# yangzhaojason/DualDiff

Measured on AMD Instinct MI355X. Metric: denoising-steps/sec, 6-view 224×400 fp16, 50-step DDIM @ 1/2/4/8 MI355X, higher is better.
Workload: dtype fp16; 1 GPU; BASELINE configs[1]: 6-view 224x400 (28x50 latents) multiview UNet + 2 ControlNet branches (ORS panorama + ORS-3D, SFA on), CFG 2.0 -> 12 view-instances/scene, DDIM-50 schedule, random-init weights; scenes_per_gpu=1, parallelism=scene-sharded x1 (no data-path collective), hip_graph=True, streams=3, invariant_conditioning=recomputed every step

## Files before the change

dualdiff_amd/_build.py:

```python
import os
import shutil
import subprocess
import sys
from concurrent.futures import ThreadPoolExecutor

HERE = os.path.dirname(os.path.abspath(__file__))
CSRC = os.path.join(HERE, "csrc")
LIBDIR = os.path.join(HERE, "lib")
OBJDIR = os.path.join(HERE, "lib", "obj")
LIBNAME = "libdualdiff_hip.so"
GEMM_SOURCES = ["gemm23.hip", "gemm2_conv.hip", "gemm1.hip", "conv3s.hip", "gemm2_geglu.hip", "gemm4.hip", "gemm.hip"]
SOURCES = ["gemm23.hip", "gemm2_conv.hip", "attention.hip", "gemm1.hip", "conv3s.hip", "gemm2_geglu.hip", "gemm4.hip",
           "norm.hip", "elementwise.hip", "tokens.hip", "xattn.hip", "clip.hip", "gemm8.hip", "vae.hip", "image.hip", "boxes.hip", "gemm.hip"]
EXTRA_FLAGS = {"attention.hip": ["-mllvm", "-amdgpu-mfma-vgpr-form=1", "-fno-honor-nans"],
               **{src: ["-mllvm", "-amdgpu-mfma-vgpr-form=1"] for src in GEMM_SOURCES},
               "clip.hip": ["-mllvm", "-amdgpu-mfma-vgpr-form=1"]}
ARCH = "gfx950"


def _hipcc():
    for cand in (os.environ.get("HIPCC"), "/opt/rocm/bin/hipcc", shutil.which("hipcc")):
        if cand and os.path.exists(cand):
            return cand
    raise RuntimeError("hipcc not found (set HIPCC or install ROCm under /opt/rocm)")


def lib_path():
    return os.environ.get("DD_HIP_LIB") or os.path.join(LIBDIR, LIBNAME)


def _deps():
    deps = [os.path.join(CSRC, f) for f in os.listdir(CSRC)]
    deps.append(os.path.join(HERE, "..", "include", "dualdiff_hip.h"))
    return deps


def needs_build():
    lib = lib_path()
    if not os.path.exists(lib):
        return True
    t = os.path.getmtime(lib)
    return any(os.path.getmtime(d) > t for d in _deps() if os.path.exists(d))


def build_native(force=False, verbose=True):
    if not force and not needs_build():
        return lib_path()
    hipcc = _hipcc()
    os.makedirs(OBJDIR, exist_ok=True)
    flags = ["--offload-arch=" + ARCH, "-O2", "-std=c++17", "-fPIC", "-Wno-unused-value",
             "-DNDEBUG"] + os.environ.get("DD_HIP_DEFINES", "").split()

    def compile_one(src):
        obj = os.path.join(OBJDIR, src.replace(".hip", ".o"))
        cmd = [hipcc] + flags + EXTRA_FLAGS.get(src, []) + ["-c", os.path.join(CSRC, src), "-o", obj]
        r = subprocess.run(cmd, capture_output=True, text=True)
        if r.returncode != 0:
            raise RuntimeError("hipcc failed for %s:\n%s\n%s" % (src, r.stdout, r.stderr))
        return obj

    with ThreadPoolExecutor(max_workers=4) as ex:
        objs = list(ex.map(compile_one, SOURCES))
    tmp = lib_path() + ".tmp"
    cmd = [hipcc, "--offload-arch=" + ARCH, "-shared", "-fPIC", "-o", tmp] + objs
    r = subprocess.run(cmd, capture_output=True, text=True)
    if r.returncode != 0:
        raise RuntimeError("link failed:\n%s\n%s" % (r.stdout, r.stderr))
    os.replace(tmp, lib_path())
    if verbose:
        print("[dualdiff_amd] built %s" % lib_path(), file=sys.stderr)
    return lib_path()


if __name__ == "__main__":
    build_native(force="--force" in sys.argv)
```

dualdiff_amd/_native.py:

```python
import ctypes
import os

import torch
from ctypes import (POINTER, Structure, c_char_p, c_float, c_int32, c_int64, c_uint32, c_void_p)

from . import _build

DD_F16, DD_BF16, DD_F32 = 0, 1, 2
DD_EPI_NONE, DD_EPI_GEGLU, DD_EPI_SILU = 0, 1, 2


class GemmDesc(Structure):
    _fields_ = [
        ("a", c_void_p), ("a2", c_void_p), ("lda", c_int64), ("lda2", c_int64), ("k1", c_int32),
        ("rows", c_int32), ("n", c_int32), ("k", c_int32),
        ("w", c_void_p), ("bias", c_void_p), ("rowvec", c_void_p),
        ("rows_per_inst", c_int32), ("ld_rowvec", c_int32),
        ("res", c_void_p), ("ldres", c_int64),
        ("out", c_void_p), ("ldc", c_int64),
        ("alpha", c_float), ("accumulate", c_int32), ("epilogue", c_int32),
        ("conv", c_int32), ("hin", c_int32), ("win", c_int32), ("cin", c_int32),
        ("hv", c_int32), ("wv", c_int32), ("hout", c_int32), ("wout", c_int32), ("stride", c_int32),
        ("dtype", c_int32), ("tile", c_int32), ("split_k", c_int32),
        ("ws", c_void_p), ("ws_bytes", c_int64),
        ("ln_colsum", c_void_p), ("ln_bias", c_void_p), ("ln_eps", c_float), ("out_f32", c_int32), ("ln_stats_out", c_void_p), ("ln_stats_in", c_void_p),
        ("out_headmajor_d", c_int32), ("hm_scaled_planes", c_int32), ("hm_scale", c_float),
        ("phase", c_int32),
        ("ln_out", c_void_p), ("ld_ln_out", c_int64), ("lno_gamma", c_void_p), ("lno_beta", c_void_p),
    ]


class AttnDesc(Structure):
    _fields_ = [
        ("q", c_void_p), ("k", c_void_p), ("v", c_void_p), ("o", c_void_p),
        ("ldq", c_int64), ("ldk", c_int64), ("ldv", c_int64), ("ldo", c_int64),
        ("q_batch_stride", c_int64), ("k_batch_stride", c_int64),
        ("v_batch_stride", c_int64), ("o_batch_stride", c_int64),
        ("batch", c_int32), ("heads", c_int32), ("head_dim", c_int32), ("lq", c_int32), ("lk", c_int32),
        ("scale", c_float),
        ("kv_batch_map", c_void_p),
        ("accumulate", c_int32), ("dtype", c_int32), ("variant", c_int32),
        ("q_head_stride", c_int64), ("k_head_stride", c_int64), ("v_head_stride", c_int64),
        ("q_prescaled", c_int32),
        ("kv_batch_map2", c_void_p),
        ("lk_dev", c_void_p),
    ]


class BoxTokensDesc(Structure):
    _fields_ = [
        ("points", c_void_p), ("classes", c_void_p), ("masks", c_void_p),
        ("class_tokens", c_void_p), ("null_pos", c_void_p), ("null_class", c_void_p),
        ("pos", c_void_p), ("cat", c_void_p), ("cls_out", c_void_p),
        ("rows", c_int32), ("points_per_box", c_int32), ("num_freqs", c_int32), ("include_input", c_int32),
        ("class_token_dim", c_int32), ("cls_offset", c_int32),
        ("ld_cat", c_int64),
        ("normalize", c_int32), ("points_dtype", c_int32), ("dtype", c_int32), ("n_classes", c_int32),
        ("freqs", c_float * 16), ("xyz_min", c_float * 3), ("xyz_range", c_float * 3),
    ]


class XAttnDesc(Structure):
    _fields_ = [
        ("x", c_void_p), ("ldx", c_int64), ("res", c_void_p), ("ldres", c_int64),
        ("wq", c_void_p), ("wo", c_void_p), ("bo", c_void_p),
        ("k", c_void_p), ("v", c_void_p), ("ldk", c_int64), ("ldv", c_int64),
        ("k_inst_stride", c_int64), ("k_head_stride", c_int64), ("v_inst_stride", c_int64), ("v_head_stride", c_int64),
        ("out", c_void_p), ("ldo", c_int64),
        ("instances", c_int32), ("rows_per_inst", c_int32), ("lk", c_int32),
        ("channels", c_int32), ("heads", c_int32), ("scale", c_float), ("dtype", c_int32),
        ("ln_out", c_void_p), ("ld_ln_out", c_int64), ("ln_gamma", c_void_p), ("ln_beta", c_void_p), ("ln_eps", c_float),
        ("lk_dev", c_void_p),
    ]


class Gemm8Desc(Structure):
    _fields_ = [
        ("a", c_void_p), ("a_scale", c_void_p), ("lda", c_int64),
        ("w", c_void_p), ("w_scale", c_void_p), ("ldw", c_int64),
        ("bias", c_void_p), ("res", c_void_p), ("ldres", c_int64),
        ("out", c_void_p), ("ldc", c_int64),
        ("rows", c_int32), ("n", c_int32), ("k_padded", c_int32), ("dtype", c_int32),
        ("out_headmajor_d", c_int32), ("hm_scaled_planes", c_int32), ("hm_scale", c_float), ("geglu", c_int32),
    ]


SIGNATURES = {
    "dd_abi_version": (c_int32, []),
    "dd_desc_size": (c_int64, [c_int32]),
    "dd_error_string": (c_char_p, [c_int32]),
    "dd_target_arch": (c_char_p, []),
    "dd_gemm": (c_int32, [POINTER(GemmDesc), c_void_p]),
    "dd_gemm_workspace_bytes": (c_int64, [POINTER(GemmDesc)]),
    "dd_gemm_num_tiles": (c_int32, []),
    "dd_gemm_tile_id": (c_int32, [c_int32]),
    "dd_gemm_kernel_name": (c_char_p, [POINTER(GemmDesc)]),
    "dd_gemm_conv_pad": (c_int32, [POINTER(GemmDesc), c_int32, c_void_p]),
    "dd_gemm_conv_pad_workspace_bytes": (c_int64, [POINTER(GemmDesc), c_int32]),
    "dd_gemm_conv_pad_kernel_name": (c_char_p, [POINTER(GemmDesc), c_int32]),
    "dd_groupnorm_nhwc": (c_int32, [c_void_p, c_int32, c_void_p, c_int32, c_void_p, c_void_p, c_void_p,
                                    c_int32, c_int32, c_int32, c_float, c_int32, c_int32,
                                    c_void_p, c_int64, c_void_p]),
    "dd_groupnorm_workspace_bytes": (c_int64, [c_int32, c_int32]),
    "dd_groupnorm_is_fused": (c_int32, [c_int32, c_int32, c_int32]),
    "dd_layernorm": (c_int32, [c_void_p, c_void_p, c_void_p, c_void_p, c_int64, c_int32, c_float,
                               c_int32, c_void_p]),
    "dd_attention": (c_int32, [POINTER(AttnDesc), c_void_p]),
    "dd_attention_kernel_name": (c_char_p, [POINTER(AttnDesc)]),
    "dd_add": (c_int32, [c_void_p, c_void_p, c_void_p, c_void_p, c_int64, c_int32, c_void_p]),
    "dd_scale": (c_int32, [c_void_p, c_void_p, c_float, c_int64, c_int32, c_void_p]),
    "dd_probe_spin": (c_int32, [c_void_p, c_uint32, c_void_p]),
    "dd_groupnorm_splitk": (c_int32, [c_void_p, c_int32, c_void_p, c_void_p, c_int32, c_void_p, c_int64, c_void_p,
                                      c_void_p, c_void_p, c_void_p, c_int32, c_int32, c_int32, c_int32, c_float, c_int32,
                                      c_int32, c_void_p]),
    "dd_xattn320": (c_int32, [POINTER(XAttnDesc), c_void_p]),
    "dd_nchw_to_nhwc_views": (c_int32, [c_void_p, c_void_p, c_int32, c_int32, c_int32, c_int32, c_int32, c_int32, c_int32,
                                        c_void_p]),
    "dd_fourier_embed_strided": (c_int32, [c_void_p, c_void_p, c_int64, c_int32, POINTER(c_float), c_int32, c_int32,
                                           c_int32, c_int32, c_int32, c_int64, c_int64, c_int64, c_int64, c_void_p]),
    "dd_box_tokens": (c_int32, [POINTER(BoxTokensDesc), c_void_p]),
    "dd_ctx_assemble": (c_int32, [c_void_p, c_void_p, c_void_p, c_void_p, c_void_p, c_int32, c_int32, c_int32, c_int32,
                                  c_int32, c_int32, c_int32, c_int32, c_void_p]),
    "dd_gemm8": (c_int32, [POINTER(Gemm8Desc), c_void_p]),
    "dd_rowquant_fp8": (c_int32, [c_void_p, c_void_p, c_void_p, c_void_p, c_void_p, c_int64, c_int32, c_int64, c_float,
                                  c_int32, c_void_p]),
    "dd_xattn_pack_weight": (c_int32, [c_void_p, c_void_p, c_int32, c_void_p]),
    "dd_silu": (c_int32, [c_void_p, c_void_p, c_int64, c_int32, c_void_p]),
    "dd_nchw_to_nhwc": (c_int32, [c_void_p, c_void_p, c_int32, c_int32, c_int32, c_int32, c_int32, c_void_p]),
    "dd_nhwc_to_nchw": (c_int32, [c_void_p, c_void_p, c_int32, c_int32, c_int32, c_int32, c_int32, c_void_p]),
    "dd_timestep_embedding": (c_int32, [c_void_p, c_void_p, c_int32, c_int32, c_int32, c_float,
                                        c_int32, c_void_p]),
    "dd_cfg_unipc_step": (c_int32, [c_void_p, c_void_p, c_void_p, c_void_p, c_void_p, c_void_p, c_void_p, c_void_p,
                                    c_float, c_int64, c_int32, c_void_p]),
    "dd_softmax_rows": (c_int32, [c_void_p, c_void_p, c_int64, c_int32, c_int64, c_int64, c_int32, c_void_p]),
    "dd_ors_project": (c_int32, [c_void_p, c_void_p, c_void_p, c_void_p, c_void_p, c_int32, c_int32, c_int32,
                                 c_float, c_int32, c_int32, c_int32, c_void_p]),
    "dd_fourier_embed": (c_int32, [c_void_p, c_void_p, c_int64, c_int32, POINTER(c_float), c_int32, c_int32,
                                   c_int32, c_int32, c_void_p]),
    "dd_conv3x3_small_cout": (c_int32, [c_void_p, c_void_p, c_void_p, c_void_p, c_int32, c_int32,
                                        c_int32, c_int32, c_int32, c_int32, c_void_p]),
    "dd_vae_posterior": (c_int32, [c_void_p, c_void_p, c_void_p, c_void_p, c_void_p, c_int32, c_int32, c_int32, c_float,
                                   c_int32, c_int32, c_void_p]),
    "dd_image_quantize_u8": (c_int32, [c_void_p, c_void_p, c_int32, c_int32, c_int32, c_int32, c_int32, c_void_p]),
    "dd_image_resample_u8": (c_int32, [c_void_p, c_void_p, c_int32, c_int32, c_int32, c_int32, c_int32, c_void_p, c_void_p,
                                       c_int32, c_void_p, c_void_p, c_int32, c_int32, c_int32, c_int32, c_int32, c_int32,
                                       c_int32, c_int32, c_void_p]),
    "dd_image_load_u8": (c_int32, [c_void_p, c_void_p, c_int32, c_int32, c_int32, c_int32, c_int32, c_void_p, c_void_p,
                                   c_int32, c_void_p, c_void_p, c_int32, c_void_p, c_int32, c_int32, c_void_p]),
    "dd_box_views": (c_int32, [c_void_p, c_void_p, c_void_p, c_void_p, c_void_p, c_int32, c_int32, c_int32, c_int32,
                               c_int32, c_int32, c_int32, c_int32, c_void_p, c_void_p, c_void_p, c_void_p, c_void_p,
                               c_void_p]),
    "dd_clip_embed": (c_int32, [c_void_p, c_void_p, c_void_p, c_void_p, c_void_p, c_int32, c_int32, c_int32, c_int32,
                                c_int32, c_int32, c_void_p]),
    "dd_causal_attention": (c_int32, [c_void_p, c_void_p, c_void_p, c_void_p, c_int64, c_int64, c_int64, c_int64,
                                      c_int64, c_int64, c_int64, c_int64, c_int32, c_int32, c_int32, c_int32, c_float,
                                      c_int32, c_void_p]),
    "dd_conv3x3_thin": (c_int32, [c_void_p, c_void_p, c_void_p, c_void_p, c_int32, c_int32, c_int32, c_int32, c_int32,
                                  c_int32, c_int32, c_int32, c_void_p]),
    "dd_cfg_ddim_step": (c_int32, [c_void_p, c_void_p, c_void_p, c_void_p, c_void_p, c_float,
                                   c_int64, c_int32, c_void_p]),
    "dd_cfg_ddim_step_given": (c_int32, [c_void_p, c_void_p, c_void_p, c_void_p, c_void_p, c_float, c_void_p, c_void_p,
                                         c_void_p, c_void_p, c_int32, c_int64, c_int64, c_int32, c_void_p]),
    "dd_cfg_unipc_step_given": (c_int32, [c_void_p, c_void_p, c_void_p, c_void_p, c_void_p, c_void_p, c_void_p,
                                          c_void_p, c_float, c_void_p, c_void_p, c_void_p, c_void_p, c_int32, c_int64,
                                          c_int64, c_int32, c_void_p]),
    "dd_given_views_noise": (c_int32, [c_void_p, c_void_p, c_void_p, c_void_p, c_void_p, c_float, c_float, c_int64,
                                       c_int64, c_int32, c_void_p]),
}

ABI_VERSION = 4
_LIB = None


def lib_path():
    return _build.lib_path()


def load(build_if_missing=True):
    global _LIB
    if _LIB is not None:
        return _LIB
    path = lib_path()
    if not os.path.exists(path):
        if not build_if_missing:
            raise RuntimeError("dualdiff_amd: %s is missing (run __graft_entry__.build())" % path)
        _build.build_native()
    try:
        lib = ctypes.CDLL(path)
    except OSError as e:
        raise RuntimeError("dualdiff_amd: cannot load HIP library %s: %s" % (path, e))
    for name, (res, args) in SIGNATURES.items():
        try:
            fn = getattr(lib, name)
        except AttributeError:
            raise RuntimeError("dualdiff_amd: %s does not export %s" % (path, name))
        fn.restype = res
        fn.argtypes = args
    if lib.dd_abi_version() != ABI_VERSION:
        raise RuntimeError("dualdiff_amd: %s has ABI version %d, this binding needs %d (rebuild: __graft_entry__.build())"
                           % (path, lib.dd_abi_version(), ABI_VERSION))
    for which, st in enumerate((GemmDesc, AttnDesc, XAttnDesc, Gemm8Desc, BoxTokensDesc)):
        if lib.dd_desc_size(which) != ctypes.sizeof(st):
            raise RuntimeError("dualdiff_amd: %s was built with a different %s (%d bytes, binding has %d)"
                               % (path, st.__name__, lib.dd_desc_size(which), ctypes.sizeof(st)))
    _LIB = lib
    return lib


class Unsupported(RuntimeError):
    """DD_ERR_UNSUPPORTED (-2): the library validated the call and launched NOTHING — the caller may take another form."""


def check(rc, what):
    if rc != 0:
        msg = load().dd_error_string(rc).decode()
        raise (Unsupported if rc == -2 else RuntimeError)("dualdiff_amd.%s failed: %s (%d)" % (what, msg, rc))
```

dualdiff_amd/csrc/gemm.hip:

```cpp
#include "gemm_device.h"
#include <algorithm>

namespace {

template <typename T>
__global__ __launch_bounds__(256)
void dd_splitk_reduce_kernel(const GemmParams p, int nsplit) {
  const int64_t groups_per_row = p.n / 8;
  const int64_t total = (int64_t)p.rows * groups_per_row;
  for (int64_t g = (int64_t)blockIdx.x * blockDim.x + threadIdx.x; g < total;
       g += (int64_t)gridDim.x * blockDim.x) {
    const int row = (int)(g / groups_per_row);
    const int col = (int)(g - (int64_t)row * groups_per_row) * 8;
    float v[8] = {0, 0, 0, 0, 0, 0, 0, 0};
    for (int z = 0; z < nsplit; ++z) {
      const float* src = p.partial + ((int64_t)z * p.rows + row) * p.n + col;
      const f32x4 a = *reinterpret_cast<const f32x4*>(src);
      const f32x4 b = *reinterpret_cast<const f32x4*>(src + 4);
      v[0] += a[0]; v[1] += a[1]; v[2] += a[2]; v[3] += a[3];
      v[4] += b[0]; v[5] += b[1]; v[6] += b[2]; v[7] += b[3];
    }
    epilogue_store8<T>(p, row, col, v);
  }
}

int ceil_div(int a, int b) { return (a + b - 1) / b; }

bool dma_ok(const dd_gemm_desc* d) {
  const int64_t lim = (int64_t)1 << 30;
  const int64_t nw = (d->epilogue == DD_EPI_GEGLU ? 2 : 1) * (int64_t)d->n;
  bool ok = (d->k % BK) == 0 && nw * d->k < lim;
  if (d->conv) {
    ok = ok && (d->cin % BK) == 0 && (int64_t)d->rows / (d->hout * d->wout) * d->hin * d->win * d->cin < lim;
  } else {
    ok = ok && (int64_t)d->rows * d->lda < lim;
    if (d->a2) ok = ok && (d->k1 % BK) == 0 && (int64_t)d->rows * d->lda2 < lim;
  }
  return ok;
}

bool env_is_zero(const char* name) { const char* v = getenv(name); return v && atoi(v) == 0; }
bool persist_off() { static const bool off = env_is_zero("DD_PERSIST"); return off; }
bool persist3_off() { static const bool off = env_is_zero("DD_PERSIST3"); return off; }

int64_t extent_bytes(const dd_gemm_desc* d, int64_t ld) { return (((int64_t)d->rows - 1) * ld + d->n) * 2; }
constexpr int64_t kExtentLimit = (int64_t)1 << 31;

int twin(const TileCfg& like, Family family) {
  for (int i = 0; i < kNumTiles; ++i)
    if (kTiles[i].family == family && kTiles[i].wm == like.wm && kTiles[i].wn == like.wn && kTiles[i].tm == like.tm &&
        kTiles[i].tn == like.tn) return i;
  return -1;
}

Plan unsupported() { Plan pl{}; pl.unsupported = true; return pl; }

Plan plan_direct(const dd_gemm_desc* d, int ti, unsigned form) {
  const TileCfg& t = kTiles[ti];
  const int hw = d->hout * d->wout, W = d->wout;
  const int arows = tile_bm(t) + 88;
  const int R = W > 0 ? std::min(tile_bm(t), arows - 16 - 2 * (W + 1)) / W : 0;
  const bool ok = form == F_CONV && d->stride == 1 && d->hv == d->hin && d->wv == d->win && d->hout == d->hin &&
                  d->wout == d->win && (d->cin % BK) == 0 && hw > 0 && d->rows % hw == 0 && dma_ok(d) &&
                  (t.band ? hw > tile_bm(t) && R >= 1 : hw <= tile_bm(t) && tile_bm(t) < 65535);
  if (!ok) return unsupported();
  const int m_inst = d->rows / hw;
  Plan pl{};
  pl.tile_idx = ti;
  if (t.band) {
    pl.band_rows = R * W;
    pl.bands = ceil_div(d->hout, R);
    pl.g_per_tile = 1;
    pl.tiles_m = m_inst * pl.bands;
  } else {
    pl.g_per_tile = std::min(tile_bm(t) / hw, m_inst);
    pl.tiles_m = ceil_div(m_inst, pl.g_per_tile);
  }
  const int nchunks = d->cin / BK;
  const int split = std::min(d->split_k > 0 ? d->split_k : 1, nchunks);
  pl.chunks_per_split = ceil_div(nchunks, split);
  pl.tiles_n = ceil_div(d->n, tile_bn(t));
  pl.split = ceil_div(nchunks, pl.chunks_per_split);
  pl.k_per_split = pl.chunks_per_split * BK;
  return pl;
}

unsigned form_of(const dd_gemm_desc* d, int pad_lo) {
  return pad_lo == 0 ? F_PAD0 : d->conv ? F_CONV : d->epilogue == DD_EPI_GEGLU ? F_GEGLU : F_DENSE;
}

Plan make_plan(const dd_gemm_desc* d, int pad_lo) {
  const bool geglu = d->epilogue == DD_EPI_GEGLU;
  const unsigned form = form_of(d, pad_lo);
  int ti = d->tile > 0 ? tile_index(d->tile) : -1;
  if (ti < 0) {
    for (int id : kAutoTiles) {
      const TileCfg& t = kTiles[tile_index(id)];
      if (!(t.forms & form)) continue;
      ti = tile_index(id);
      const int bn_out = geglu ? tile_bn(t) / 2 : tile_bn(t);
      if ((long)ceil_div(d->rows, tile_bm(t)) * ceil_div(d->n, bn_out) >= (long)kNumCU * 3 / 2) break;
    }
  }
  if (d->ln_colsum) {
    const int ring = twin(kTiles[ti], FAM_RING);
    if (d->tile <= 0 && ring >= 0) ti = ring;
    if (kTiles[ti].family != FAM_RING || !dma_ok(d)) return unsupported();
  }
  if (kTiles[ti].family == FAM_PIPE && d->conv) return unsupported();
  if (d->ln_out) {
    if (d->tile > 0 && !(kTiles[ti].forms & F_LN_OUT)) return unsupported();
    if (d->tile <= 0) {
      const int pipe = tile_index(kTileLnPipe);
      ti = (!persist3_off() || ceil_div(d->rows, tile_bm(kTiles[pipe])) <= kNumCU) ? pipe : tile_index(kTileLnRing);
    }
    if (d->n != 320 || !dma_ok(d)) return unsupported();
  }
  if (kTiles[ti].family == FAM_DIRECT) return plan_direct(d, ti, form);
  if (kTiles[ti].family != FAM_REG && !dma_ok(d)) {
    const int reg = twin(kTiles[ti], FAM_REG);
    ti = reg >= 0 ? reg : tile_index(geglu ? kTile128x128 : kTile64x64);
  }
  const TileCfg& t = kTiles[ti];
  if (!(t.forms & form)) return unsupported();
  Plan pl{};
  const int bn_out = geglu ? tile_bn(t) / 2 : tile_bn(t);
  pl.tile_idx = ti;
  pl.tiles_m = ceil_div(d->rows, tile_bm(t));
  pl.tiles_n = ceil_div(d->n, bn_out);
  int split = d->split_k;
  const int nkt = ceil_div(d->k, BK);
  if (split <= 0) {
    const long blocks = (long)pl.tiles_m * pl.tiles_n;
    const bool deep = !geglu && blocks < kNumCU && nkt >= 16;
    split = deep ? (int)std::max(1L, std::min({(2L * kNumCU + blocks - 1) / blocks, (long)nkt / 4, 32L})) : 1;
  }
  if (geglu || d->ln_colsum || d->ln_stats_out || d->out_headmajor_d || d->ln_out) split = 1;
  if (split > nkt) split = nkt;
  int kts = ceil_div(nkt, split);
  split = ceil_div(nkt, kts);
  pl.split = split;
  pl.k_per_split = kts * BK;
  const bool walk = (t.forms & F_PERSIST) && !d->conv && split == 1 && !d->ln_colsum && nkt >= t.depth;
  pl.persist_ok = walk && t.family == FAM_RING && !persist_off() && !d->ln_out;
  const bool ln_tile = (t.forms & F_LN_OUT) != 0;
  const bool pre_acc = !geglu && !ln_tile && t.tm * (t.tn / 2) <= 4;
  pl.persist3_ok = walk && t.family == FAM_PIPE && !persist3_off() && (d->k % BK) == 0 && !d->out_f32 && !d->ln_stats_out &&
                   !d->rowvec && (!d->accumulate || pre_acc) && ln_tile == (d->ln_out != nullptr) &&
                   extent_bytes(d, d->ldc) < kExtentLimit && (!d->res || extent_bytes(d, d->ldres) < kExtentLimit) &&
                   (!d->ln_out || extent_bytes(d, d->ld_ln_out) < kExtentLimit);
  return pl;
}

inline bool gemm4_takes(const Plan& pl) {
  return pl.persist3_ok && pl.tiles_m * pl.tiles_n > kNumCU * gemm4_resident(kTiles[pl.tile_idx]);
}

LaunchFn* launcher(const Plan& pl, unsigned form) {
  switch (kTiles[pl.tile_idx].family) {
    case FAM_REG: return launch_gemm1;
    case FAM_RING: return form == F_CONV ? launch_gemm2_conv : form == F_GEGLU ? launch_gemm2_geglu : launch_gemm2_dense;
    case FAM_PIPE: return gemm4_takes(pl) ? launch_gemm4 : launch_gemm3;
    default: return launch_conv3s;
  }
}

int validate(const dd_gemm_desc* d, int pad_lo = 1) {
  if (!d || !d->a || !d->w || !d->out) return DD_ERR_BAD_ARG;
  if (d->ln_colsum) {
    if (!d->ln_bias || d->conv || d->a2 || d->bias) return DD_ERR_BAD_ARG;
    if (d->k != 320 && d->k != 640 && d->k != 1280) return DD_ERR_UNSUPPORTED;
    if (!dd_aligned16(d->ln_colsum) || !dd_aligned16(d->ln_bias) || (d->lda & 7)) return DD_ERR_BAD_ARG;
  }
  if (d->ln_out) {
    if (!d->lno_gamma || !d->lno_beta || d->conv || d->epilogue != DD_EPI_NONE || d->rowvec || d->accumulate ||
        d->out_f32 || d->out_headmajor_d || d->ln_stats_out || d->ln_colsum)
      return DD_ERR_UNSUPPORTED;
    if (d->n != 320) return DD_ERR_UNSUPPORTED;
    if (!dd_aligned16(d->ln_out) || !dd_aligned16(d->lno_gamma) || !dd_aligned16(d->lno_beta) || (d->ld_ln_out & 7))
      return DD_ERR_BAD_ARG;
  }
  if (d->rows <= 0 || d->n <= 0 || d->k <= 0) return DD_ERR_BAD_ARG;
  if (d->rows >= (1 << 22)) return DD_ERR_UNSUPPORTED;
  if ((d->k & 7) || (d->n & 7) || (d->ldc & 7)) return DD_ERR_BAD_ARG;
  if (d->dtype != DD_F16 && d->dtype != DD_BF16) return DD_ERR_BAD_ARG;
  if (!dd_aligned16(d->a) || !dd_aligned16(d->w) || !dd_aligned16(d->out)) return DD_ERR_BAD_ARG;
  if (d->bias && !dd_aligned16(d->bias)) return DD_ERR_BAD_ARG;
  if (d->res && (!dd_aligned16(d->res) || (d->ldres & 7))) return DD_ERR_BAD_ARG;
  if (d->rowvec && (!dd_aligned16(d->rowvec) || (d->ld_rowvec & 7) || d->rows_per_inst <= 0)) return DD_ERR_BAD_ARG;
  if (d->conv) {
    if (d->a2) return DD_ERR_UNSUPPORTED;
    if (d->cin <= 0 || (d->cin & 7) || d->k != 9 * d->cin) return DD_ERR_BAD_ARG;
    if (d->hin <= 0 || d->win <= 0 || d->hout <= 0 || d->wout <= 0) return DD_ERR_BAD_ARG;
    if (d->stride != 1 && d->stride != 2) return DD_ERR_UNSUPPORTED;
    if (d->hv <= 0 || d->wv <= 0) return DD_ERR_BAD_ARG;
    if (d->rows % (d->hout * d->wout) != 0) return DD_ERR_BAD_ARG;
    if ((d->hv + pad_lo + 1 - 3) / d->stride + 1 != d->hout || (d->wv + pad_lo + 1 - 3) / d->stride + 1 != d->wout)
      return DD_ERR_BAD_ARG;
  } else {
    if (d->lda & 7) return DD_ERR_BAD_ARG;
    if (d->a2) {
      if (!dd_aligned16(d->a2) || (d->lda2 & 7) || (d->k1 & 7) || d->k1 <= 0 || d->k1 >= d->k) return DD_ERR_BAD_ARG;
    }
  }
  if (d->epilogue != DD_EPI_NONE && d->epilogue != DD_EPI_GEGLU && d->epilogue != DD_EPI_SILU) return DD_ERR_BAD_ARG;
  if (d->out_f32 && (d->epilogue == DD_EPI_GEGLU || d->accumulate)) return DD_ERR_UNSUPPORTED;
  if (d->ln_stats_out && ((d->n & 31) || d->epilogue == DD_EPI_GEGLU || d->out_f32 || !dd_aligned16(d->ln_stats_out)))
    return DD_ERR_UNSUPPORTED;
  if (d->ln_stats_in && (!d->ln_colsum || !dd_aligned16(d->ln_stats_in))) return DD_ERR_BAD_ARG;
  if (d->out_headmajor_d) {
    if (d->out_headmajor_d < 8 || (d->out_headmajor_d & 7) || d->n % d->out_headmajor_d) return DD_ERR_BAD_ARG;
    if (d->conv || d->epilogue == DD_EPI_GEGLU || d->accumulate || d->out_f32 || d->ln_stats_out) return DD_ERR_UNSUPPORTED;
  }
  if (d->epilogue == DD_EPI_GEGLU && (d->res || d->rowvec || d->accumulate || d->alpha != 1.0f)) return DD_ERR_UNSUPPORTED;
  if (d->epilogue == DD_EPI_GEGLU && d->conv) return DD_ERR_UNSUPPORTED;
  return DD_OK;
}

int validate_pad(const dd_gemm_desc* d, int pad_lo) {
  if (pad_lo != 0 && pad_lo != 1) return DD_ERR_BAD_ARG;
  if (pad_lo == 1) return validate(d);
  if (!d || !d->conv) return DD_ERR_BAD_ARG;
  if (d->stride != 2 || d->hv != d->hin || d->wv != d->win || d->epilogue == DD_EPI_GEGLU) return DD_ERR_UNSUPPORTED;
  if (d->hin < 2 || d->win < 2) return DD_ERR_BAD_ARG;
  return validate(d, 0);
}

thread_local char g_kname[160];

}

extern "C" int dd_gemm_num_tiles(void) { return kNumTiles; }
extern "C" int dd_gemm_tile_id(int index) { return (index >= 0 && index < kNumTiles) ? kTiles[index].id : -1; }

constexpr int64_t DD_COUNTER_BYTES = 65536;

namespace {

int64_t workspace_bytes(const dd_gemm_desc* d, int pad_lo) {
  if (validate_pad(d, pad_lo) != DD_OK) return 0;
  const Plan pl = make_plan(d, pad_lo);
  if (pl.unsupported || pl.split <= 1) return 0;
  return DD_COUNTER_BYTES + (int64_t)pl.split * d->rows * d->n * (int64_t)sizeof(float);
}

const char* kernel_name(const dd_gemm_desc* d, int pad_lo) {
  const int vc = validate_pad(d, pad_lo);
  if (vc != DD_OK) return (pad_lo == 0 && vc == DD_ERR_UNSUPPORTED) ? "unsupported" : "invalid";
  const Plan pl = make_plan(d, pad_lo);
  if (pl.unsupported) return "unsupported";
  const TileCfg& t = kTiles[pl.tile_idx];
  const char* conv = d->conv ? "true" : "false";
  const char* geglu = d->epilogue == DD_EPI_GEGLU ? "true" : "false";
  const char* kern = "dd_gemm_pad0_kernel";
  char args[48] = "";
  if (pad_lo == 0) {
  } else if (t.family == FAM_DIRECT) {
    kern = "dd_conv3s_kernel";
    snprintf(args, sizeof(args), ", %d, %d, %s", t.depth, t.grp, t.band ? "true" : "false");
  } else if (t.family == FAM_PIPE) {
    kern = gemm4_takes(pl) ? "dd_gemm4_kernel" : "dd_gemm3_kernel";
    snprintf(args, sizeof(args), ", %d, %s", t.depth, geglu);
  } else if (t.family == FAM_RING) {
    kern = "dd_gemm2_kernel";
    snprintf(args, sizeof(args), ", %d, %s, %s", t.depth, conv, geglu);
  } else {
    kern = "dd_gemm_kernel";
    snprintf(args, sizeof(args), ", %s, %s", conv, geglu);
  }
  snprintf(g_kname, sizeof(g_kname), "%s<%s, %d, %d, %d, %d%s> split=%d grid=%dx%d tile=%s", kern,
           d->dtype == DD_F16 ? "_Float16" : "__bf16", t.wm, t.wn, t.tm, t.tn, args, pl.split, pl.tiles_m, pl.tiles_n, t.name);
  return g_kname;
}

int gemm_run(const dd_gemm_desc* d, int pad_lo, dd_stream_t stream) {
  const int vc = validate_pad(d, pad_lo);
  if (vc != DD_OK) return vc;
  const Plan pl = make_plan(d, pad_lo);
  if (pl.unsupported) return DD_ERR_UNSUPPORTED;
  GemmParams p{};
  p.g_per_tile = pl.g_per_tile; p.chunks_per_split = pl.chunks_per_split;
  p.ln_colsum = reinterpret_cast<const float*>(d->ln_colsum);
  p.ln_bias = reinterpret_cast<const float*>(d->ln_bias);
  p.ln_eps = d->ln_eps;
  p.ln_out = d->ln_out; p.ld_ln_out = d->ld_ln_out; p.lno_gamma = d->lno_gamma; p.lno_beta = d->lno_beta;
  p.a = d->a; p.a2 = d->a2; p.lda = d->lda; p.lda2 = d->lda2;
  p.k1 = d->a2 ? d->k1 : d->k;
  p.rows = d->rows; p.n = d->n; p.k = d->k;
  p.w = d->w; p.bias = d->bias; p.rowvec = d->rowvec;
  p.rows_per_inst = d->rows_per_inst > 0 ? d->rows_per_inst : 1; p.ld_rowvec = d->ld_rowvec;
  p.res = d->res; p.ldres = d->ldres; p.out = d->out; p.ldc = d->ldc;
  p.alpha = d->alpha; p.accumulate = d->accumulate; p.out_f32 = d->out_f32;
  p.stat_out = reinterpret_cast<float*>(d->ln_stats_out);
  p.stat_in = reinterpret_cast<const float*>(d->ln_stats_in);
  p.hm_d = d->out_headmajor_d; p.hm_planes = d->hm_scaled_planes; p.hm_scale = d->hm_scale;
  p.act = d->epilogue == DD_EPI_SILU ? DD_EPI_SILU : DD_EPI_NONE;
  p.hin = d->hin; p.win = d->win; p.cin = d->cin; p.hv = d->hv; p.wv = d->wv;
  p.hout = d->hout; p.wout = d->wout; p.stride = d->stride;
  p.upsample = d->conv && (d->hv != d->hin || d->wv != d->win);
  p.scale_h = d->conv ? (float)d->hin / (float)d->hv : 1.f;
  p.scale_w = d->conv ? (float)d->win / (float)d->wv : 1.f;
  p.k_per_split = pl.k_per_split;
  p.tiles_m = pl.tiles_m; p.tiles_n = pl.tiles_n;
  p.band_rows = pl.band_rows; p.bands = pl.bands; p.inv_bands = pl.bands > 0 ? 1.0f / (float)pl.bands : 1.0f;
  p.inv_hw = d->conv ? 1.0f / (float)(d->hout * d->wout) : 1.0f;
  p.inv_wout = d->conv ? 1.0f / (float)d->wout : 1.0f;
  p.inv_rpi = 1.0f / (float)p.rows_per_inst;
  {
    const int64_t nw = (d->epilogue == DD_EPI_GEGLU ? 2 : 1) * (int64_t)d->n;
    p.w_bytes = (uint32_t)(nw * d->k * 2);
    if (d->conv) {
      p.a_bytes = (uint32_t)((int64_t)d->rows / (d->hout * d->wout) * d->hin * d->win * d->cin * 2);
      p.a2_bytes = 0;
    } else {
      p.a_bytes = (uint32_t)((((int64_t)d->rows - 1) * d->lda + p.k1) * 2);
      p.a2_bytes = d->a2 ? (uint32_t)((((int64_t)d->rows - 1) * d->lda2 + (d->k - d->k1)) * 2) : 0u;
    }
  }
  {
    const int64_t ob = extent_bytes(d, d->ldc), rb = extent_bytes(d, d->ldres);
    const bool fits = ob < kExtentLimit && (!d->res || rb < kExtentLimit);
    p.out_bytes = fits ? (uint32_t)ob : 0u;
    p.res_bytes = fits && d->res ? (uint32_t)rb : 0u;
  }
  p.persist = 0;
  p.inv_tiles_n = 1.0f / (float)(pl.tiles_n > 0 ? pl.tiles_n : 1);
  p.inv_hm_d = d->out_headmajor_d > 0 ? 1.0f / (float)d->out_headmajor_d : 1.0f;
  p.ln_out_bytes = d->ln_out ? (uint32_t)extent_bytes(d, d->ld_ln_out) : 0u;
  p.partial = nullptr;
  p.dbg_stamps = nullptr;
  DD_STAMP_HOST(p, d);
  if (pl.split > 1) {
    const int64_t need = DD_COUNTER_BYTES + (int64_t)pl.split * d->rows * d->n * (int64_t)sizeof(float);
    if (!d->ws || d->ws_bytes < need) return DD_ERR_WORKSPACE;
    p.partial = reinterpret_cast<float*>(reinterpret_cast<char*>(d->ws) + DD_COUNTER_BYTES);
  }
  hipStream_t s = reinterpret_cast<hipStream_t>(stream);
  dd_clear_error();
  if (d->phase != 2) {
    const int rc = launcher(pl, form_of(d, pad_lo))(d->dtype, form_of(d, pad_lo), p, pl, s);
    if (rc != DD_OK) return rc;
  }
  if (pl.split > 1 && d->phase != 1) {
    const int blocks = (int)std::min<int64_t>(((int64_t)p.rows * (p.n / 8) + 255) / 256, 2048);
    if (d->dtype == DD_F16) hipLaunchKernelGGL(dd_splitk_reduce_kernel<_Float16>, dim3(blocks), dim3(256), 0, s, p, pl.split);
    else hipLaunchKernelGGL(dd_splitk_reduce_kernel<__bf16>, dim3(blocks), dim3(256), 0, s, p, pl.split);
    return dd_check_launch();
  }
  return DD_OK;
}

}

extern "C" int64_t dd_gemm_workspace_bytes(const dd_gemm_desc* d) { return workspace_bytes(d, 1); }
extern "C" const char* dd_gemm_kernel_name(const dd_gemm_desc* d) { return kernel_name(d, 1); }
extern "C" int dd_gemm(const dd_gemm_desc* d, dd_stream_t stream) { return gemm_run(d, 1, stream); }

extern "C" int dd_gemm_conv_pad(const dd_gemm_desc* d, int32_t pad_lo, dd_stream_t stream) {
  return gemm_run(d, pad_lo, stream);
}
extern "C" int64_t dd_gemm_conv_pad_workspace_bytes(const dd_gemm_desc* d, int32_t pad_lo) {
  return workspace_bytes(d, pad_lo);
}
extern "C" const char* dd_gemm_conv_pad_kernel_name(const dd_gemm_desc* d, int32_t pad_lo) {
  return kernel_name(d, pad_lo);
}
```

dualdiff_amd/csrc/gemm2_kernel.h:

```cpp
#pragma once
#include "gemm_device.h"

namespace {

template <int NW, int TM, int TN, int NSTAGE, bool CONV>
constexpr int gemm2_min_blocks() {
  return (!CONV && NW == 4 && TM * TN <= 8 && NSTAGE <= 3) ? 2 : 1;
}

template <typename T, int WAVES_M, int WAVES_N, int TM, int TN, int NSTAGE, bool CONV, bool GEGLU>
__global__ __launch_bounds__(64 * WAVES_M * WAVES_N, (gemm2_min_blocks<WAVES_M * WAVES_N, TM, TN, NSTAGE, CONV>()))
void dd_gemm2_kernel(const GemmParams p) {
  using V8 = typename dd_vec<T>::v8;
  constexpr int NW = WAVES_M * WAVES_N;
  constexpr int BM = WAVES_M * TM * 16;
  constexpr int BN = WAVES_N * TN * 16;
  constexpr int BN_OUT = GEGLU ? BN / 2 : BN;
  constexpr int XI = BM / 8 / NW;
  constexpr int WI = BN / 8 / NW;
  constexpr int LPS = XI + WI;
  constexpr int STAGE = (BM + BN) * BK;
  static_assert(BM % (8 * NW) == 0 && BN % (8 * NW) == 0, "tile/waves mismatch");
  static_assert(NW % 2 == 0, "swizzle must not depend on the instruction index");
  static_assert(TN % 2 == 0 && (!GEGLU || TN % 4 == 0), "TN");
  static_assert(NSTAGE >= 2 && NSTAGE <= 8, "NSTAGE");
  static_assert((NSTAGE - 2) * LPS <= 63, "vmcnt is a 6-bit counter");

  DD_STAMP_DECL();
  DD_STAMP(0);
  extern __shared__ __attribute__((aligned(16))) unsigned char smem[];
  T* ring = reinterpret_cast<T*>(smem);

  const int tid = threadIdx.x;
  const int lane = tid & 63;
  const int wave = __builtin_amdgcn_readfirstlane(tid >> 6);
  const int wave_m = wave / WAVES_N;
  const int wave_n = wave % WAVES_N;

  const int ntiles = p.tiles_m * p.tiles_n;
  int lin = blockIdx.x;
  int tile = xcd_remap(lin, ntiles);
  int block_m0 = (tile / p.tiles_n) * BM;
  int block_n0 = (tile % p.tiles_n) * BN_OUT;

  const int kbeg = blockIdx.z * p.k_per_split;
  const int kend = min(p.k, kbeg + p.k_per_split);
  const int nk = (kend - kbeg + BK - 1) / BK;

  const int lrow = lane >> 3;
  const int lc = (lane & 7) ^ ((((wave & 1) << 2) + (lane >> 4)) & 7);
  const uint32_t lcb = (uint32_t)lc * 16u;

  uint32_t wv[WI];
  auto make_wv = [&](const int bn0) __attribute__((always_inline)) {
#pragma unroll
  for (int j = 0; j < WI; ++j) {
    const int R = (j * NW + wave) * 8 + lrow;
    const int wvi = R / (TN * 16);
    const int rho = R % (TN * 16);
    const int tn = rho >> 4, r = rho & 15;
    int n_glob;
    if (GEGLU) {
      constexpr int TH = TN / 2;
      const int t = tn % TH;
      const int loc = wvi * (TH * 16) + (r >> 2) * (4 * TH) + t * 4 + (r & 3);
      const int col = bn0 + loc;
      n_glob = (col < p.n) ? col + (tn >= TH ? p.n : 0) : -1;
    } else {
      const int loc = wvi * (TN * 16) + (r >> 2) * (4 * TN) + tn * 4 + (r & 3);
      const int col = bn0 + loc;
      n_glob = (col < p.n) ? col : -1;
    }
    wv[j] = n_glob >= 0 ? (uint32_t)n_glob * (uint32_t)p.k * 2u + lcb : DD_OOB;
  }
  };
  make_wv(block_n0);

  uint32_t xe[XI];
  uint32_t xe2[CONV ? 1 : XI];
  uint32_t syo[CONV ? XI : 1][3], sxo[CONV ? XI : 1][3], xbits[CONV ? XI : 1];
#pragma unroll
  for (int j = 0; j < XI; ++j) {
    const int r = block_m0 + (j * NW + wave) * 8 + lrow;
    const bool rv = r < p.rows;
    if (CONV) {
      const int hw = p.hout * p.wout;
      const int rr = rv ? r : 0;
      const int inst = dd_fdiv(rr, p.inv_hw);
      const int rem = rr - inst * hw;
      const int oy = dd_fdiv(rem, p.inv_wout);
      const int ox = rem - oy * p.wout;
      const int iy0 = oy * p.stride - 1, ix0 = ox * p.stride - 1;
      uint32_t bits = 0;
#pragma unroll
      for (int t = 0; t < 3; ++t) {
        const int iy = iy0 + t, ix = ix0 + t;
        const bool vy = iy >= 0 && iy < p.hv, vx = ix >= 0 && ix < p.wv;
        int sy = min(max(iy, 0), p.hv - 1), sx = min(max(ix, 0), p.wv - 1);
        if (p.upsample) {
          sy = min((int)floorf(sy * p.scale_h), p.hin - 1);
          sx = min((int)floorf(sx * p.scale_w), p.win - 1);
        }
        syo[j][t] = (uint32_t)((inst * p.hin + sy) * p.win) * (uint32_t)p.cin * 2u + lcb;
        sxo[j][t] = (uint32_t)(sx * p.cin) * 2u;
        if (vy) bits |= 1u << t;
        if (vx) bits |= 8u << t;
      }
      uint32_t m9 = 0;
#pragma unroll
      for (int t = 0; t < 9; ++t)
        if (rv && ((bits >> (t / 3)) & 1u) && ((bits >> (3 + t % 3)) & 1u)) m9 |= 1u << t;
      xbits[j] = m9;
      xe[j] = DD_OOB;
    } else {
      xe[j] = rv ? (uint32_t)r * (uint32_t)p.lda * 2u + lcb : DD_OOB;
      xe2[j] = rv ? (uint32_t)r * (uint32_t)p.lda2 * 2u + lcb : DD_OOB;
    }
  }
  auto make_xe = [&](const int bm0) __attribute__((always_inline)) {
#pragma unroll
    for (int j = 0; j < XI; ++j) {
      const int r = bm0 + (j * NW + wave) * 8 + lrow;
      const bool rv = r < p.rows;
      xe[j] = rv ? (uint32_t)r * (uint32_t)p.lda * 2u + lcb : DD_OOB;
      xe2[j] = rv ? (uint32_t)r * (uint32_t)p.lda2 * 2u + lcb : DD_OOB;
    }
  };
  auto set_tap = [&](int tap) __attribute__((always_inline)) {
    if (CONV) {
      const int ky = (tap * 11) >> 5;
      const int kx = tap - ky * 3;
      const uint32_t y0 = 0u - (uint32_t)(ky == 0), y1 = 0u - (uint32_t)(ky == 1), y2 = 0u - (uint32_t)(ky == 2);
      const uint32_t x0 = 0u - (uint32_t)(kx == 0), x1 = 0u - (uint32_t)(kx == 1), x2 = 0u - (uint32_t)(kx == 2);
#pragma unroll
      for (int j = 0; j < XI; ++j) {
        const uint32_t oy = (syo[j][0] & y0) | (syo[j][1] & y1) | (syo[j][2] & y2);
        const uint32_t ox = (sxo[j][0] & x0) | (sxo[j][1] & x1) | (sxo[j][2] & x2);
        const uint32_t m = 0u - ((xbits[j] >> tap) & 1u);
        xe[j] = ((oy + ox) & m) | (DD_OOB & ~m);
      }
    }
  };
  const __amdgpu_buffer_rsrc_t rs_w = __builtin_amdgcn_make_buffer_rsrc(const_cast<void*>(p.w), 0, p.w_bytes, 0x00020000);
  const __amdgpu_buffer_rsrc_t rs_a = __builtin_amdgcn_make_buffer_rsrc(const_cast<void*>(p.a), 0, p.a_bytes, 0x00020000);
  const __amdgpu_buffer_rsrc_t rs_a2 = __builtin_amdgcn_make_buffer_rsrc(
      const_cast<void*>(p.a2 ? p.a2 : p.a), 0, p.a2 ? p.a2_bytes : p.a_bytes, 0x00020000);

  int ik0 = kbeg;
  int itap = CONV ? kbeg / p.cin : 0;
  int ici0 = CONV ? kbeg - itap * p.cin : 0;
  set_tap(itap);
  auto issue_next = [&](int slot) __attribute__((always_inline)) {
    T* xs = ring + slot * STAGE;
    T* ws = xs + BM * BK;
    const uint32_t ksoff = dd_dbg::SAMEK ? 0u : (uint32_t)ik0 * 2u;
#pragma unroll
    for (int j = 0; j < WI; ++j) bdma16(rs_w, wv[j], ksoff, ws + (j * NW + wave) * 8 * BK);
    if (CONV) {
      const uint32_t csoff = (uint32_t)ici0 * 2u;
#pragma unroll
      for (int j = 0; j < XI; ++j) bdma16(rs_a, xe[j], csoff, xs + (j * NW + wave) * 8 * BK);
      ici0 += BK;
      if (ici0 >= p.cin) {
        ici0 = 0;
        ++itap;
        set_tap(itap);
      }
    } else if (ik0 >= p.k1) {
      const uint32_t k2 = (uint32_t)(ik0 - p.k1) * 2u;
#pragma unroll
      for (int j = 0; j < XI; ++j) bdma16(rs_a2, xe2[j], k2, xs + (j * NW + wave) * 8 * BK);
    } else {
#pragma unroll
      for (int j = 0; j < XI; ++j) bdma16(rs_a, xe[j], ksoff, xs + (j * NW + wave) * 8 * BK);
    }
    ik0 += BK;
  };

  f32x4 acc[TN][TM];
#pragma unroll
  for (int i = 0; i < TN; ++i)
#pragma unroll
    for (int j = 0; j < TM; ++j) acc[i][j] = f32x4{0.f, 0.f, 0.f, 0.f};

  const int frow = lane & 15;
  const int fswz = (lane >> 1) & 7;
  const int fchunk = lane >> 4;

  DD_STAMP(1);
#pragma unroll
  for (int s0 = 0; s0 < NSTAGE - 1; ++s0)
    if (s0 < nk) issue_next(s0);
  DD_STAMP(2);

  __shared__ float s_ln_mean[BM], s_ln_rstd[BM];
  if (!CONV && p.ln_colsum && p.stat_in) {
    const int parts = p.k >> 5;
    const float inv_k = 1.0f / (float)p.k;
    for (int r = tid; r < BM; r += NW * 64) {
      const float* src = p.stat_in + (int64_t)min(block_m0 + r, p.rows - 1) * parts * 2;
      float sum = 0.f, sq = 0.f;
      for (int i = 0; i < parts; i += 2) {
        const f32x4 v = *reinterpret_cast<const f32x4*>(src + i * 2);
        sum += v[0] + v[2];
        sq += v[1] + v[3];
      }
      const float mean = sum * inv_k;
      s_ln_mean[r] = mean;
      s_ln_rstd[r] = rsqrtf(fmaxf(sq * inv_k - mean * mean, 0.f) + p.ln_eps);
    }
    __syncthreads();
  } else if (!CONV && p.ln_colsum) {
    const int lpr = p.k / 40;
    const int rpw = 64 / lpr;
    const int sub = lane & (lpr - 1);
    const float inv_k = 1.0f / (float)p.k;
    for (int r0 = wave * rpw; r0 < BM; r0 += NW * rpw) {
      const int r = r0 + lane / lpr;
      const int64_t grow = min(block_m0 + r, p.rows - 1);
      float sum = 0.f, sq = 0.f;
      u32x4 raw[5];
#pragma unroll
      for (int i = 0; i < 5; ++i)
        raw[i] = dd_ld16(reinterpret_cast<const T*>(p.a) + grow * p.lda + (sub + i * lpr) * 8);
#pragma unroll
      for (int i = 0; i < 5; ++i) {
        float f[8];
        dd_unpack8<T>(raw[i], f);
#pragma unroll
        for (int e = 0; e < 8; ++e) { sum += f[e]; sq += f[e] * f[e]; }
      }
      for (int o = lpr >> 1; o > 0; o >>= 1) { sum += __shfl_xor(sum, o, 64); sq += __shfl_xor(sq, o, 64); }
      if (sub == 0) {
        const float mean = sum * inv_k;
        s_ln_mean[r] = mean;
        s_ln_rstd[r] = rsqrtf(fmaxf(sq * inv_k - mean * mean, 0.f) + p.ln_eps);
      }
    }
    __syncthreads();
  }

  V8 wf[2][TN], xf[2][TM];
  auto mfma_step = [&]() __attribute__((always_inline)) {
    __builtin_amdgcn_s_setprio(1);
#pragma unroll
    for (int ks = 0; ks < 2; ++ks) {
#pragma unroll
      for (int i = 0; i < TN; ++i)
#pragma unroll
        for (int j = 0; j < TM; ++j) acc[i][j] = dd_mfma16(wf[ks][i], xf[ks][j], acc[i][j]);
    }
    __builtin_amdgcn_s_setprio(0);
  };
  int sbase = 0;
  bool have_next = false;
  auto kstep = [&](const int kt) __attribute__((always_inline)) {
    if (NSTAGE == 2) {
      wait_vmcnt<0>();
    } else {
      const int ahead = have_next ? NSTAGE - 2 : min(nk - 1 - kt, NSTAGE - 2);
      if (ahead <= 0) wait_vmcnt<0>();
      else if (ahead == 1 || NSTAGE <= 3) wait_vmcnt<(NSTAGE > 2 ? 1 : 0) * LPS>();
      else if (ahead == 2 || NSTAGE <= 4) wait_vmcnt<(NSTAGE > 3 ? 2 : 0) * LPS>();
      else if (ahead == 3 || NSTAGE <= 5) wait_vmcnt<(NSTAGE > 4 ? 3 : 0) * LPS>();
      else if (ahead == 4 || NSTAGE <= 6) wait_vmcnt<(NSTAGE > 5 ? 4 : 0) * LPS>();
      else if (ahead == 5 || NSTAGE <= 7) wait_vmcnt<(NSTAGE > 6 ? 5 : 0) * LPS>();
      else wait_vmcnt<(NSTAGE > 7 ? 6 : 0) * LPS>();
    }
    __builtin_amdgcn_s_barrier();
    {
      const int a = kt + NSTAGE - 1;
      const int islot = (sbase + a) % NSTAGE;
      if (a < nk) {
        issue_next(islot);
      } else if (have_next) {
        if constexpr (!CONV) {
          if (a == nk) {
            const int nt = xcd_remap(lin + (int)gridDim.x, ntiles);
            make_wv((nt % p.tiles_n) * BN_OUT);
            make_xe((nt / p.tiles_n) * BM);
            ik0 = kbeg;
          }
          issue_next(islot);
        }
      }
    }
    const int slot = (sbase + kt) % NSTAGE;
    const T* xs = ring + slot * STAGE + (wave_m * TM * 16 + frow) * BK;
    const T* ws = ring + slot * STAGE + BM * BK + (wave_n * TN * 16 + frow) * BK;
#pragma unroll
    for (int ks = 0; ks < 2; ++ks) {
      const int cofs = ((fchunk + 4 * ks) ^ fswz) << 3;
#pragma unroll
      for (int i = 0; i < TN; ++i) wf[ks][i] = dd_as_v8<T>(dd_ld16(ws + i * 16 * BK + cofs));
#pragma unroll
      for (int j = 0; j < TM; ++j) xf[ks][j] = dd_as_v8<T>(dd_ld16(xs + j * 16 * BK + cofs));
    }
    __builtin_amdgcn_sched_barrier(0);
    mfma_step();
  };
  const bool persist = !CONV && p.persist != 0;
  for (;;) {
  have_next = persist && lin + (int)gridDim.x < ntiles;
  for (int kt = 0; kt < nk; kt += 2) {
    kstep(kt);
    DD_STAMP_IF(kt == 0, 3);
    if (kt + 1 < nk) kstep(kt + 1);
  }
  DD_STAMP(4);
  if constexpr (!CONV && !GEGLU && WAVES_M == 1 && WAVES_N == 10 && TM == 5 && TN == 2) {
    if (p.ln_out) {
      store_tile_ln<T>(p, acc, block_m0, wave_n, lane, reinterpret_cast<float*>(smem));
      return;
    }
  }
  const bool ln = !CONV && p.ln_colsum;
  store_tile<T, TM, TN, GEGLU>(p, acc, block_m0, block_n0, wave_m, wave_n, lane, p.rows,
                               ln ? s_ln_mean : nullptr, ln ? s_ln_rstd : nullptr);
  if (!have_next) break;
  lin += (int)gridDim.x;
  tile = xcd_remap(lin, ntiles);
  block_m0 = (tile / p.tiles_n) * BM;
  block_n0 = (tile % p.tiles_n) * BN_OUT;
  sbase = (sbase + nk) % NSTAGE;
#pragma unroll
  for (int i = 0; i < TN; ++i)
#pragma unroll
    for (int j = 0; j < TM; ++j) acc[i][j] = f32x4{0.f, 0.f, 0.f, 0.f};
  }
  DD_STAMP_FLUSH(p);
}

struct Gemm2 {
  static constexpr Family family = FAM_RING;
  static constexpr unsigned needs = 0;
  template <typename T, size_t I, unsigned FORM>
  static int run(const GemmParams& p, const Plan& pl, hipStream_t s) {
    constexpr const TileCfg& t = kTiles[I];
    constexpr size_t smem = (size_t)t.depth * (tile_bm(t) + tile_bn(t)) * BK * sizeof(T);
    static_assert(smem <= 160 * 1024, "LDS");
    constexpr auto kern = dd_gemm2_kernel<T, t.wm, t.wn, t.tm, t.tn, t.depth, FORM == F_CONV, FORM == F_GEGLU>;
    dim3 grid(pl.tiles_m * pl.tiles_n, 1, pl.split);
    GemmParams q = p;
    if (pl.persist_ok) {
      static std::atomic<int> resident{0};
      int per_cu = resident.load(std::memory_order_relaxed);
      if (per_cu == 0) {
        raise_lds_limit<kern>(smem);
        if (hipOccupancyMaxActiveBlocksPerMultiprocessor(&per_cu, kern, 64 * t.wm * t.wn, smem) != hipSuccess || per_cu < 1)
          per_cu = 1;
        resident.store(per_cu, std::memory_order_relaxed);
      }
      if ((int)grid.x > kNumCU * per_cu) {
        q.persist = 1;
        grid.x = kNumCU * per_cu;
      }
    }
    return launch_kernel<kern>(grid, 64 * t.wm * t.wn, smem, s, q);
  }
};

}
```

dualdiff_amd/csrc/gemm_device.h:

```cpp
#pragma once
#include "dd_common.h"
#include "dd_debug.h"
#include "gemm_tiles.h"
#include <type_traits>

using namespace ddg;

namespace {

__device__ __forceinline__ int dd_fdiv(int n, float inv) { return (int)(((float)n + 0.5f) * inv); }


template <typename T>
__device__ __forceinline__ void store8(const GemmParams& p, int64_t row, int col, float (&v)[8]) {
  if (p.hm_d) {
    const int plane = col / p.hm_d;
    if (plane < p.hm_planes) {
#pragma unroll
      for (int e = 0; e < 8; ++e) v[e] *= p.hm_scale;
    }
    dd_st16(reinterpret_cast<T*>(p.out) + ((int64_t)plane * p.rows + row) * p.hm_d + (col - plane * p.hm_d),
            dd_pack8<T>(v));
    return;
  }
  if (p.out_f32) {
    float* o = reinterpret_cast<float*>(p.out) + row * p.ldc + col;
    *reinterpret_cast<f32x4*>(o) = f32x4{v[0], v[1], v[2], v[3]};
    *reinterpret_cast<f32x4*>(o + 4) = f32x4{v[4], v[5], v[6], v[7]};
  } else {
    dd_st16(reinterpret_cast<T*>(p.out) + row * p.ldc + col, dd_pack8<T>(v));
  }
}

template <typename T>
__device__ __forceinline__ void epilogue_store8(const GemmParams& p, int row, int col, float (&v)[8]) {
  if (p.bias) {
    float b[8];
    dd_unpack8<T>(dd_ld16(reinterpret_cast<const T*>(p.bias) + col), b);
#pragma unroll
    for (int i = 0; i < 8; ++i) v[i] += b[i];
  }
  if (p.rowvec) {
    const int inst = dd_fdiv(row, p.inv_rpi);
    float b[8];
    dd_unpack8<T>(dd_ld16(reinterpret_cast<const T*>(p.rowvec) + (int64_t)inst * p.ld_rowvec + col), b);
#pragma unroll
    for (int i = 0; i < 8; ++i) v[i] += b[i];
  }
#pragma unroll
  for (int i = 0; i < 8; ++i) v[i] *= p.alpha;
  if (p.res) {
    float b[8];
    dd_unpack8<T>(dd_ld16(reinterpret_cast<const T*>(p.res) + (int64_t)row * p.ldres + col), b);
#pragma unroll
    for (int i = 0; i < 8; ++i) v[i] += b[i];
  }
  if (p.act == DD_EPI_SILU) {
#pragma unroll
    for (int i = 0; i < 8; ++i) v[i] = dd_silu_f(v[i]);
  }
  if (p.accumulate) {
    float b[8];
    dd_unpack8<T>(dd_ld16(reinterpret_cast<T*>(p.out) + (int64_t)row * p.ldc + col), b);
#pragma unroll
    for (int i = 0; i < 8; ++i) v[i] += b[i];
  }
  store8<T>(p, row, col, v);
}

__device__ __forceinline__ int xcd_remap(int bid, int nwg) {
  const int xcd = bid & 7;
  const int q = nwg >> 3, r = nwg & 7;
  const int base = (xcd < r) ? xcd * (q + 1) : r * (q + 1) + (xcd - r) * q;
  return base + (bid >> 3);
}

template <typename T, int TM, int TN, bool GEGLU>
__device__ __forceinline__ void store_tile(const GemmParams& p, f32x4 (&acc)[TN][TM], int block_m0,
                                           int block_n0, int wave_m, int wave_n, int lane, int row_end,
                                           const float* ln_mean = nullptr, const float* ln_rstd = nullptr) {
  const int q = lane >> 4;
  const int c = lane & 15;
  const int row0 = block_m0 + wave_m * (TM * 16) + c;
  if constexpr (GEGLU) {
    constexpr int TH = TN / 2;
    constexpr int NG = TH / 2;
    const int col0 = block_n0 + wave_n * (TH * 16) + q * (4 * TH);
    u32x4 bh[NG], bg[NG];
    f32x4 lsh[NG][2], lsg[NG][2], lbh[NG][2], lbg[NG][2];
    if (ln_mean) {
#pragma unroll
      for (int g8 = 0; g8 < NG; ++g8) {
        const int col = min(col0 + g8 * 8, p.n - 8);
#pragma unroll
        for (int h2 = 0; h2 < 2; ++h2) {
          lsh[g8][h2] = *reinterpret_cast<const f32x4*>(p.ln_colsum + col + 4 * h2);
          lsg[g8][h2] = *reinterpret_cast<const f32x4*>(p.ln_colsum + p.n + col + 4 * h2);
          lbh[g8][h2] = *reinterpret_cast<const f32x4*>(p.ln_bias + col + 4 * h2);
          lbg[g8][h2] = *reinterpret_cast<const f32x4*>(p.ln_bias + p.n + col + 4 * h2);
        }
      }
    }
    if (p.bias) {
#pragma unroll
      for (int g8 = 0; g8 < NG; ++g8) {
        const int col = min(col0 + g8 * 8, p.n - 8);
        bh[g8] = dd_ld16(reinterpret_cast<const T*>(p.bias) + col);
        bg[g8] = dd_ld16(reinterpret_cast<const T*>(p.bias) + p.n + col);
      }
    }
#pragma unroll
    for (int tm = 0; tm < TM; ++tm) {
      const int row = row0 + tm * 16;
      if (row >= row_end) continue;
#pragma unroll
      for (int g8 = 0; g8 < NG; ++g8) {
        const int col = col0 + g8 * 8;
        if (col >= p.n) continue;
        float h[8], g[8];
#pragma unroll
        for (int e = 0; e < 8; ++e) {
          h[e] = acc[g8 * 2 + (e >> 2)][tm][e & 3];
          g[e] = acc[TH + g8 * 2 + (e >> 2)][tm][e & 3];
        }
        if (ln_mean) {
          const int lr = wave_m * (TM * 16) + tm * 16 + c;
          const float mu = ln_mean[lr], rs = ln_rstd[lr];
#pragma unroll
          for (int e = 0; e < 8; ++e) {
            h[e] = rs * (h[e] - mu * lsh[g8][e >> 2][e & 3]) + lbh[g8][e >> 2][e & 3];
            g[e] = rs * (g[e] - mu * lsg[g8][e >> 2][e & 3]) + lbg[g8][e >> 2][e & 3];
          }
        }
        if (p.bias) {
          float b[8];
          dd_unpack8<T>(bh[g8], b);
#pragma unroll
          for (int e = 0; e < 8; ++e) h[e] += b[e];
          dd_unpack8<T>(bg[g8], b);
#pragma unroll
          for (int e = 0; e < 8; ++e) g[e] += b[e];
        }
        float v[8];
#pragma unroll
        for (int e = 0; e < 8; ++e) v[e] = dd_geglu_f(h[e], g[e]);
        dd_st16(reinterpret_cast<T*>(p.out) + (int64_t)row * p.ldc + col, dd_pack8<T>(v));
      }
    }
  } else {
    constexpr int NG = TN / 2;
    const int col0 = block_n0 + wave_n * (TN * 16) + q * (4 * TN);
    if (p.partial) {
#pragma unroll
      for (int tm = 0; tm < TM; ++tm) {
        const int row = row0 + tm * 16;
        if (row >= row_end) continue;
#pragma unroll
        for (int g8 = 0; g8 < NG; ++g8) {
          const int col = col0 + g8 * 8;
          if (col >= p.n) continue;
          float* dst = p.partial + ((int64_t)blockIdx.z * p.rows + row) * p.n + col;
          *reinterpret_cast<f32x4*>(dst) = acc[g8 * 2][tm];
          *reinterpret_cast<f32x4*>(dst + 4) = acc[g8 * 2 + 1][tm];
        }
      }
      return;
    }
    constexpr int TMB = (TM >= 4 && TM % 2 == 0) ? TM / 2 : TM;
    u32x4 rb[NG];
    int colc[NG];
#pragma unroll
    for (int g8 = 0; g8 < NG; ++g8) colc[g8] = min(col0 + g8 * 8, p.n - 8);
    if (p.bias) {
#pragma unroll
      for (int g8 = 0; g8 < NG; ++g8) rb[g8] = dd_ld16(reinterpret_cast<const T*>(p.bias) + colc[g8]);
    }
    f32x4 lcs[NG][2], lcb[NG][2];
    if (ln_mean) {
#pragma unroll
      for (int g8 = 0; g8 < NG; ++g8)
#pragma unroll
        for (int h2 = 0; h2 < 2; ++h2) {
          lcs[g8][h2] = *reinterpret_cast<const f32x4*>(p.ln_colsum + colc[g8] + 4 * h2);
          lcb[g8][h2] = *reinterpret_cast<const f32x4*>(p.ln_bias + colc[g8] + 4 * h2);
        }
    }
#pragma unroll
    for (int tb = 0; tb < TM; tb += TMB) {
      u32x4 rv[TMB][NG], rr[TMB][NG], ra[TMB][NG];
#pragma unroll
      for (int t2 = 0; t2 < TMB; ++t2) {
        const int rowc = min(row0 + (tb + t2) * 16, p.rows - 1);
        if (p.rowvec) {
          const int inst = dd_fdiv(rowc, p.inv_rpi);
#pragma unroll
          for (int g8 = 0; g8 < NG; ++g8)
            rv[t2][g8] = dd_ld16(reinterpret_cast<const T*>(p.rowvec) + (int64_t)inst * p.ld_rowvec + colc[g8]);
        }
        if (p.res) {
#pragma unroll
          for (int g8 = 0; g8 < NG; ++g8)
            rr[t2][g8] = dd_ld16(reinterpret_cast<const T*>(p.res) + (int64_t)rowc * p.ldres + colc[g8]);
        }
        if (p.accumulate) {
#pragma unroll
          for (int g8 = 0; g8 < NG; ++g8)
            ra[t2][g8] = dd_ld16(reinterpret_cast<const T*>(p.out) + (int64_t)rowc * p.ldc + colc[g8]);
        }
      }
#pragma unroll
      for (int t2 = 0; t2 < TMB; ++t2) {
        const int tm = tb + t2;
        const int row = row0 + tm * 16;
        float st_s = 0.f, st_q = 0.f;
        if (row < row_end) {
#pragma unroll
        for (int g8 = 0; g8 < NG; ++g8) {
          const int col = col0 + g8 * 8;
          if (col >= p.n) continue;
          float v[8], b[8];
#pragma unroll
          for (int e = 0; e < 8; ++e) v[e] = acc[g8 * 2 + (e >> 2)][tm][e & 3];
          if (ln_mean) {
            const int lr = wave_m * (TM * 16) + tm * 16 + c;
            const float mu = ln_mean[lr], rs = ln_rstd[lr];
#pragma unroll
            for (int e = 0; e < 8; ++e) v[e] = rs * (v[e] - mu * lcs[g8][e >> 2][e & 3]) + lcb[g8][e >> 2][e & 3];
          }
          if (p.bias) {
            dd_unpack8<T>(rb[g8], b);
#pragma unroll
            for (int e = 0; e < 8; ++e) v[e] += b[e];
          }
          if (p.rowvec) {
            dd_unpack8<T>(rv[t2][g8], b);
#pragma unroll
            for (int e = 0; e < 8; ++e) v[e] += b[e];
          }
#pragma unroll
          for (int e = 0; e < 8; ++e) v[e] *= p.alpha;
          if (p.res) {
            dd_unpack8<T>(rr[t2][g8], b);
#pragma unroll
            for (int e = 0; e < 8; ++e) v[e] += b[e];
          }
          if (p.act == DD_EPI_SILU) {
#pragma unroll
            for (int e = 0; e < 8; ++e) v[e] = dd_silu_f(v[e]);
          }
          if (p.accumulate) {
            dd_unpack8<T>(ra[t2][g8], b);
#pragma unroll
            for (int e = 0; e < 8; ++e) v[e] += b[e];
          }
          store8<T>(p, row, col, v);
          if (p.stat_out) {
#pragma unroll
            for (int e = 0; e < 8; ++e) { st_s += v[e]; st_q += v[e] * v[e]; }
          }
        }
        }
        if constexpr (TN == 2 || TN == 4) {
          if (p.stat_out) {
            st_s += __shfl_xor(st_s, 16, 64);  st_q += __shfl_xor(st_q, 16, 64);
            if (TN == 2) { st_s += __shfl_xor(st_s, 32, 64);  st_q += __shfl_xor(st_q, 32, 64); }
            const int gcol = block_n0 + wave_n * (TN * 16) + (TN == 2 ? 0 : (q >> 1) * 32);
            const bool writer = TN == 2 ? q == 0 : (q & 1) == 0;
            if (writer && row < row_end && gcol < p.n) {
              float* dst = p.stat_out + ((int64_t)row * (p.n >> 5) + (gcol >> 5)) * 2;
              dst[0] = st_s;
              dst[1] = st_q;
            }
          }
        }
      }
    }
  }
}

template <typename T>
__device__ __forceinline__ void store_tile_ln(const GemmParams& p, f32x4 (&acc)[2][5], int block_m0, int wave_n,
                                              int lane, float* scratch) {
  constexpr int TM = 5, NWV = 10, BM = 80, NCOL = 320;
  const int q = lane >> 4, c = lane & 15;
  const int col = wave_n * 32 + q * 8;
  float bias[8], ga[8], be[8];
  if (p.bias) dd_unpack8<T>(dd_ld16(reinterpret_cast<const T*>(p.bias) + col), bias);
  dd_unpack8<T>(dd_ld16(reinterpret_cast<const T*>(p.lno_gamma) + col), ga);
  dd_unpack8<T>(dd_ld16(reinterpret_cast<const T*>(p.lno_beta) + col), be);
  u32x4 rr[TM];
  if (p.res) {
#pragma unroll
    for (int tm = 0; tm < TM; ++tm) {
      const int64_t rowc = min(block_m0 + tm * 16 + c, p.rows - 1);
      rr[tm] = dd_ld16(reinterpret_cast<const T*>(p.res) + rowc * p.ldres + col);
    }
  }
  float v[TM][8], part[TM];
#pragma unroll
  for (int tm = 0; tm < TM; ++tm) {
    const int row = block_m0 + tm * 16 + c;
    float r[8];
    if (p.res) dd_unpack8<T>(rr[tm], r);
    float s = 0.f;
#pragma unroll
    for (int e = 0; e < 8; ++e) {
      float x = acc[e >> 2][tm][e & 3];
      if (p.bias) x += bias[e];
      x *= p.alpha;
      if (p.res) x += r[e];
      v[tm][e] = (float)(T)x;
      s += v[tm][e];
    }
    if (row < p.rows) dd_st16(reinterpret_cast<T*>(p.out) + (int64_t)row * p.ldc + col, dd_pack8<T>(v[tm]));
    s += __shfl_xor(s, 16, 64);
    s += __shfl_xor(s, 32, 64);
    part[tm] = s;
  }
  __syncthreads();
  if (q == 0) {
#pragma unroll
    for (int tm = 0; tm < TM; ++tm) scratch[wave_n * BM + tm * 16 + c] = part[tm];
  }
  __syncthreads();
  float mean[TM];
#pragma unroll
  for (int tm = 0; tm < TM; ++tm) {
    float s = 0.f;
#pragma unroll
    for (int w = 0; w < NWV; ++w) s += scratch[w * BM + tm * 16 + c];
    mean[tm] = s * (1.0f / (float)NCOL);
    float ss = 0.f;
#pragma unroll
    for (int e = 0; e < 8; ++e) { const float d = v[tm][e] - mean[tm]; ss += d * d; }
    ss += __shfl_xor(ss, 16, 64);
    ss += __shfl_xor(ss, 32, 64);
    part[tm] = ss;
  }
  __syncthreads();
  if (q == 0) {
#pragma unroll
    for (int tm = 0; tm < TM; ++tm) scratch[wave_n * BM + tm * 16 + c] = part[tm];
  }
  __syncthreads();
#pragma unroll
  for (int tm = 0; tm < TM; ++tm) {
    const int row = block_m0 + tm * 16 + c;
    float ss = 0.f;
#pragma unroll
    for (int w = 0; w < NWV; ++w) ss += scratch[w * BM + tm * 16 + c];
    const float rstd = rsqrtf(ss * (1.0f / (float)NCOL) + p.ln_eps);
    float o[8];
#pragma unroll
    for (int e = 0; e < 8; ++e) o[e] = (v[tm][e] - mean[tm]) * rstd * ga[e] + be[e];
    if (row < p.rows) dd_st16(reinterpret_cast<T*>(p.ln_out) + (int64_t)row * p.ld_ln_out + col, dd_pack8<T>(o));
  }
}

template <int N>
__device__ __forceinline__ void wait_vmcnt() { asm volatile("s_waitcnt vmcnt(%0)" ::"n"(N) : "memory"); }

__device__ __forceinline__ void bdma16(__amdgpu_buffer_rsrc_t rsrc, uint32_t voff, uint32_t soff, void* lds_wave_base) {
  if constexpr (!dd_dbg::NODMA)
    __builtin_amdgcn_raw_ptr_buffer_load_lds(rsrc, (__attribute__((address_space(3))) void*)lds_wave_base, 16,
                                             (int)voff, (int)soff, 0, 0);
}
constexpr uint32_t DD_OOB = 0x80000000u;


template <int WM, int WN>
constexpr int gemm3_min_waves() {
  return WM * WN == 4 ? 2 : 1;
}

}
```

dualdiff_amd/csrc/gemm_tiles.h:

```cpp
#pragma once
#include "dd_common.h"
#include <utility>

namespace ddg {

constexpr int BK = 64;
constexpr int kNumCU = 256;

struct GemmParams {
  const void* a; const void* a2; int64_t lda, lda2; int k1;
  int rows, n, k;
  const void* w; const void* bias; const void* rowvec; int rows_per_inst, ld_rowvec;
  const void* res; int64_t ldres;
  void* out; int64_t ldc;
  float alpha; int accumulate; int act;
  int hin, win, cin, hv, wv, hout, wout, stride, upsample;
  float scale_h, scale_w;
  int k_per_split;
  float* partial;
  int tiles_m, tiles_n;
  uint32_t a_bytes, a2_bytes, w_bytes;
  uint32_t out_bytes, res_bytes;
  int g_per_tile, chunks_per_split;
  int band_rows, bands; float inv_bands;
  const float* ln_colsum; const float* ln_bias; float ln_eps;
  int out_f32;
  float* stat_out;
  const float* stat_in;
  int hm_d, hm_planes; float hm_scale;
  int persist;
  uint64_t* dbg_stamps;
  float inv_hw, inv_wout, inv_rpi;
  void* ln_out; int64_t ld_ln_out;
  const void* lno_gamma; const void* lno_beta;
  float inv_tiles_n, inv_hm_d;
  uint32_t ln_out_bytes;
};

enum Family {
  FAM_REG,
  FAM_RING,
  FAM_PIPE,
  FAM_DIRECT,
};

enum Form : unsigned {
  F_DENSE = 1,
  F_CONV = 2,
  F_GEGLU = 4,
  F_PAD0 = 8,
  F_LN_OUT = 16,
  F_PERSIST = 32,
};

struct TileCfg {
  int id; const char* name; Family family;
  int wm, wn, tm, tn;
  unsigned forms;
  int depth = 0;
  int grp = 1;
  bool band = false;
};

constexpr unsigned REG_ALL = F_DENSE | F_CONV | F_GEGLU | F_PAD0, REG_TN2 = F_DENSE | F_CONV | F_PAD0;
constexpr unsigned RING_ALL = F_DENSE | F_CONV | F_GEGLU | F_PERSIST, RING_TN2 = F_DENSE | F_CONV | F_PERSIST;
constexpr unsigned RING_DENSE = F_DENSE | F_PERSIST;
constexpr unsigned PIPE = F_DENSE | F_PERSIST;

constexpr TileCfg kTiles[] = {
    {1, "128x128", FAM_REG, 2, 2, 4, 4, REG_ALL},
    {2, "128x64", FAM_REG, 2, 2, 4, 2, REG_TN2},
    {3, "64x128", FAM_REG, 2, 2, 2, 4, REG_ALL},
    {4, "64x64", FAM_REG, 2, 2, 2, 2, REG_TN2},
    {5, "256x128", FAM_REG, 4, 2, 4, 4, REG_ALL},
    {11, "128x128/dma2", FAM_RING, 2, 2, 4, 4, RING_ALL, 2},
    {12, "128x128/dma3", FAM_RING, 2, 2, 4, 4, RING_ALL, 3},
    {13, "128x64/dma3", FAM_RING, 2, 2, 4, 2, RING_TN2, 3},
    {14, "64x128/dma3", FAM_RING, 2, 2, 2, 4, RING_ALL, 3},
    {15, "64x64/dma3", FAM_RING, 2, 2, 2, 2, RING_TN2, 3},
    {16, "256x128/dma2", FAM_RING, 4, 2, 4, 4, RING_ALL, 2},
    {20, "256x128/dma3", FAM_RING, 4, 2, 4, 4, RING_ALL, 3},
    {23, "128x64/dma4", FAM_RING, 2, 2, 4, 2, RING_TN2, 4},
    {24, "64x128/dma4", FAM_RING, 2, 2, 2, 4, RING_ALL, 4},
    {27, "160x160/dma2", FAM_RING, 2, 5, 5, 2, RING_TN2, 2},
    {28, "160x160/dma3", FAM_RING, 2, 5, 5, 2, RING_TN2, 3},
    {40, "80x320/dma2", FAM_RING, 1, 10, 5, 2, RING_DENSE | F_LN_OUT, 2},
    {52, "96x64/dma3", FAM_RING, 2, 2, 3, 2, RING_TN2, 3},
    {59, "32x64/dma3", FAM_RING, 2, 2, 1, 2, RING_DENSE, 3},
    {60, "32x64/dma6", FAM_RING, 2, 2, 1, 2, RING_DENSE, 6},
    {44, "192x128/dma3", FAM_RING, 4, 2, 3, 4, RING_ALL, 3},
    {46, "192x128/dma2", FAM_RING, 4, 2, 3, 4, RING_ALL, 2},
    {50, "256x256/dma2", FAM_RING, 2, 4, 8, 4, RING_ALL, 2},
    {72, "96x64/p3", FAM_PIPE, 2, 2, 3, 2, PIPE, 3},
    {73, "96x64/p5", FAM_PIPE, 2, 2, 3, 2, PIPE, 5},
    {75, "192x128/p3", FAM_PIPE, 4, 2, 3, 4, PIPE | F_GEGLU, 3},
    {76, "32x64/p4", FAM_PIPE, 2, 2, 1, 2, F_DENSE, 4},
    {77, "32x64/p6", FAM_PIPE, 2, 2, 1, 2, F_DENSE, 6},
    {78, "160x160/p3", FAM_PIPE, 2, 5, 5, 2, PIPE, 3},
    {74, "80x320/p3", FAM_PIPE, 1, 10, 5, 2, PIPE | F_LN_OUT, 3},
    {31, "conv3s 384x64", FAM_DIRECT, 4, 2, 6, 2, F_CONV, 5},
    {39, "conv3s band 384x64", FAM_DIRECT, 4, 2, 6, 2, F_CONV, 5, 1, true},
    {34, "conv3s 192x64/w4", FAM_DIRECT, 2, 2, 6, 2, F_CONV, 4},
    {35, "conv3s 128x64/w3", FAM_DIRECT, 2, 2, 4, 2, F_CONV, 3},
    {37, "conv3s 192x64/g3", FAM_DIRECT, 2, 2, 6, 2, F_CONV, 6, 3},
};
constexpr int kNumTiles = sizeof(kTiles) / sizeof(kTiles[0]);

constexpr int kTile128x128 = 1, kTile128x64 = 2, kTile64x128 = 3, kTile64x64 = 4;
constexpr int kAutoTiles[] = {kTile128x128, kTile128x64, kTile64x128, kTile64x64};
constexpr int kTileLnRing = 40, kTileLnPipe = 74;

constexpr int tile_bm(const TileCfg& t) { return t.wm * t.tm * 16; }
constexpr int tile_bn(const TileCfg& t) { return t.wn * t.tn * 16; }
constexpr int tile_index(int id) {
  for (int i = 0; i < kNumTiles; ++i) if (kTiles[i].id == id) return i;
  return -1;
}

constexpr bool tiles_consistent() {
  for (const TileCfg& t : kTiles)
    if (((t.forms & F_PAD0) && t.family != FAM_REG) || ((t.forms & F_CONV) && t.family == FAM_PIPE) ||
        ((t.forms & F_LN_OUT) && tile_bn(t) != 320) || (t.family == FAM_DIRECT) != (t.forms == F_CONV)) return false;
  for (int id : kAutoTiles) if (tile_index(id) < 0 || kTiles[tile_index(id)].family != FAM_REG) return false;
  return tile_index(kTileLnRing) >= 0 && tile_index(kTileLnPipe) >= 0;
}
static_assert(tiles_consistent(), "kTiles");

constexpr int gemm4_resident(const TileCfg& t) {
  const int ring = t.depth * (tile_bm(t) + tile_bn(t)) * BK * 2;
  return (t.wm * t.wn == 4 && 2 * ring <= 160 * 1024) ? 2 : 1;
}

struct Plan { int tile_idx; int split; int tiles_m, tiles_n; int k_per_split; int g_per_tile, chunks_per_split; bool unsupported; bool persist_ok; int band_rows, bands; bool persist3_ok; };

using LaunchFn = int(int dtype, unsigned form, const GemmParams& p, const Plan& pl, hipStream_t s);
__attribute__((visibility("hidden"))) LaunchFn launch_gemm1, launch_gemm2_dense, launch_gemm2_geglu, launch_gemm2_conv, launch_gemm3,
    launch_gemm4, launch_conv3s;

template <auto KERN>
void raise_lds_limit(size_t smem) {
  static std::atomic<uint64_t> attr_done{0};
  dd_ensure_dyn_lds(reinterpret_cast<const void*>(KERN), smem, attr_done);
}
template <auto KERN>
int launch_kernel(dim3 grid, int threads, size_t smem, hipStream_t s, const GemmParams& p) {
  raise_lds_limit<KERN>(smem);
  hipLaunchKernelGGL(KERN, grid, dim3(threads), smem, s, p);
  return dd_check_launch();
}

template <typename L, typename T, unsigned FORM, size_t I>
int launch_row(const GemmParams& p, const Plan& pl, hipStream_t s) {
  if constexpr (kTiles[I].family == L::family && (kTiles[I].forms & (FORM | L::needs)) == (FORM | L::needs))
    return L::template run<T, I, FORM>(p, pl, s);
  else return DD_ERR_UNSUPPORTED;
}
template <typename L, typename T, unsigned FORM, size_t... I>
int launch_rows(const GemmParams& p, const Plan& pl, hipStream_t s, std::index_sequence<I...>) {
  int rc = DD_ERR_UNSUPPORTED;
  (void)((pl.tile_idx == (int)I && ((rc = launch_row<L, T, FORM, I>(p, pl, s)), true)) || ...);
  return rc;
}
template <typename L, unsigned... FORMS>
int dispatch(int dtype, unsigned form, const GemmParams& p, const Plan& pl, hipStream_t s) {
  constexpr auto rows = std::make_index_sequence<kNumTiles>{};
  int rc = DD_ERR_UNSUPPORTED;
  (void)((form == FORMS && ((rc = dtype == DD_F16 ? launch_rows<L, _Float16, FORMS>(p, pl, s, rows)
                                                  : launch_rows<L, __bf16, FORMS>(p, pl, s, rows)), true)) || ...);
  return rc;
}

}
```

dualdiff_amd/networks/layers.py:

```python
import math

import torch
import torch.nn as nn

from .. import ops as O


CACHE_EPOCH = [0]


class _Cached(nn.Module):

    def _drop_cache(self):
        CACHE_EPOCH[0] += 1
        for k in [k for k in self.__dict__ if k.startswith("_pk_")]:
            del self.__dict__[k]

    def _apply(self, fn, *a, **k):
        self._drop_cache()
        return super()._apply(fn, *a, **k)

    def _load_from_state_dict(self, *a, **k):
        self._drop_cache()
        return super()._load_from_state_dict(*a, **k)


CTX_BASE = 78
CTX_BUCKET = 32


def box_capacity(n_box):
    return max(CTX_BUCKET, -(-int(n_box) // CTX_BUCKET) * CTX_BUCKET)


def ctx_capacity(lc):
    return int(lc) if lc < CTX_BASE else CTX_BASE + box_capacity(lc - CTX_BASE)


_CTX_KEYS = __import__("threading").local()


class context_keys:

    def __init__(self, ctx, capacity, lk_dev):
        self.new = None if lk_dev is None else (ctx.data_ptr(), ctx.data_ptr() + ctx.numel() * ctx.element_size(),
                                                int(capacity), lk_dev)

    def __enter__(self):
        self.old = getattr(_CTX_KEYS, "cur", None)
        _CTX_KEYS.cur = self.new
        return self

    def __exit__(self, *exc):
        _CTX_KEYS.cur = self.old
        return False


def lk_dev_for(ctx2d, lk):
    cur = getattr(_CTX_KEYS, "cur", None)
    if cur is None or lk != cur[2] or not (cur[0] <= ctx2d.data_ptr() < cur[1]):
        return None
    return cur[3]


_LK_CONST = {}


def lk_const(value, device):
    key = (str(device), int(value))
    t = _LK_CONST.get(key)
    if t is None:
        if torch.cuda.is_current_stream_capturing():
            raise RuntimeError("lk_const(%d) first requested inside a stream capture" % value)
        t = _LK_CONST[key] = torch.tensor([int(value)], dtype=torch.int32, device=device)
    return t


def _pad_cols(w, mult=8):
    k = w.shape[1]
    kp = (k + mult - 1) // mult * mult
    if kp == k:
        return w.contiguous()
    out = w.new_zeros((w.shape[0], kp))
    out[:, :k] = w
    return out


def to_nhwc(x):
    m, c, h, w = x.shape
    p = x.permute(0, 2, 3, 1)
    if not p.is_contiguous():
        if not x.is_cuda or x.dtype not in (torch.float16, torch.bfloat16):
            p = p.contiguous()
        else:
            return O.nchw_to_nhwc(x), m, h, w
    return p.reshape(m * h * w, c), m, h, w


def as_nchw_view(x2d, m, h, w):
    return x2d.view(m, h, w, x2d.shape[1]).permute(0, 3, 1, 2)


class Linear(_Cached):

    def __init__(self, in_features, out_features, bias=True, conv=False):
        super().__init__()
        self.in_features, self.out_features, self.conv = in_features, out_features, conv
        shape = (out_features, in_features, 1, 1) if conv else (out_features, in_features)
        self.weight = nn.Parameter(torch.empty(shape))
        self.bias = nn.Parameter(torch.empty(out_features)) if bias else None

    @property
    def w2d(self):
        if "_pk_w" not in self.__dict__:
            self.__dict__["_pk_w"] = _pad_cols(self.weight.detach().reshape(self.out_features, -1))
        return self.__dict__["_pk_w"]

    @property
    def wx(self):
        ver = (self.weight.data_ptr(), self.weight._version)
        hit = self.__dict__.get("_pk_wx")
        if hit is None or (hit[1] != ver and not torch.cuda.is_current_stream_capturing()):
            hit = self.__dict__["_pk_wx"] = (O.xattn_pack_weight(self.w2d), ver)
        return hit[0]

    fp8_mfma = False

    @property
    def w8p(self):
        if "_pk_w8p" not in self.__dict__:
            self.__dict__["_pk_w8p"] = O.quantize_fp8_padded(self.w2d)
        return self.__dict__["_pk_w8p"]

    def run(self, x2d, ln_next=None, **kw):
        if ln_next is not None and ln_producer_ok(self, ln_next, kw):
            w = self.w2d
            out = O.gemm(x2d, w, self.bias, ln_out=(ln_next.weight, ln_next.bias, ln_next.eps), **kw)
            out._ln_cache = (ln_next, out._ln_out)
            return out
        w = self.w2d
        if w.shape[1] != self.in_features:
            x2d = torch.nn.functional.pad(x2d, (0, w.shape[1] - x2d.shape[1]))
        return O.gemm(x2d, w, self.bias, **kw)

    def run_ln(self, x2d, norm, **kw):
        if self.fp8_mfma and fp8_mfma_ok(norm, self.in_features, self.out_features, x2d) \
                and set(kw) <= {"epilogue"} and kw.get("epilogue", O.DD_EPI_NONE) in (O.DD_EPI_NONE, O.DD_EPI_GEGLU):
            a8, sa = O.rowquant_fp8(x2d, (norm.weight, norm.bias, norm.eps))
            w8, sw = self.w8p
            return O.gemm8(a8, sa, w8, sw, self.bias, dtype=x2d.dtype, geglu=kw.get("epilogue") == O.DD_EPI_GEGLU)
        if not ln_fold_ok(norm, self.in_features, self.out_features, x2d):
            return self.run(norm.run(x2d), **kw)
        w, ln = fold_layernorm(self.__dict__, "_pk_ln", norm, [self.weight], [self.bias])
        return O.gemm(x2d, w, None, ln=ln, **kw)

    def forward(self, x):
        if self.conv and x.dim() == 4:
            x2d, m, h, w = to_nhwc(x)
            return as_nchw_view(self.run(x2d), m, h, w)
        lead = x.shape[:-1]
        y = self.run(x.reshape(-1, x.shape[-1]) if x.is_contiguous() else x.contiguous().reshape(-1, x.shape[-1]))
        return y.reshape(*lead, self.out_features)


class Conv3x3(_Cached):

    def __init__(self, in_channels, out_channels, stride=1):
        super().__init__()
        self.in_channels, self.out_channels, self.stride = in_channels, out_channels, stride
        self.weight = nn.Parameter(torch.empty(out_channels, in_channels, 3, 3))
        self.bias = nn.Parameter(torch.empty(out_channels))

    @property
    def cin_pad(self):
        return (self.in_channels + 7) // 8 * 8

    @property
    def packed(self):
        if "_pk_w" not in self.__dict__:
            w = self.weight.detach().permute(0, 2, 3, 1)
            if self.cin_pad != self.in_channels:
                wp = w.new_zeros((self.out_channels, 3, 3, self.cin_pad))
                wp[..., :self.in_channels] = w
                w = wp
            self.__dict__["_pk_w"] = w.reshape(self.out_channels, 9 * self.cin_pad).contiguous()
        return self.__dict__["_pk_w"]

    def run(self, x2d, m, h, w, up_size=None, **kw):
        return O.conv3x3(x2d, self.packed, self.bias, m, h, w, stride=self.stride, up_size=up_size, **kw)

    def out_hw(self, h, w, up_size=None):
        hv, wv = (h, w) if up_size is None else up_size
        return (hv - 1) // self.stride + 1, (wv - 1) // self.stride + 1

    def forward(self, x):
        x2d, m, h, w = to_nhwc(x)
        if x2d.shape[1] != self.cin_pad:
            x2d = torch.nn.functional.pad(x2d, (0, self.cin_pad - x2d.shape[1]))
        ho, wo = self.out_hw(h, w)
        return as_nchw_view(self.run(x2d, m, h, w), m, ho, wo)


class GroupNorm(nn.Module):
    def __init__(self, num_groups, num_channels, eps=1e-5):
        super().__init__()
        self.num_groups, self.num_channels, self.eps = num_groups, num_channels, eps
        self.weight = nn.Parameter(torch.empty(num_channels))
        self.bias = nn.Parameter(torch.empty(num_channels))

    def run(self, x2d, m, hw, silu, x2=None):
        hit = getattr(x2d, "_gn_cache", None)
        if hit is not None:
            del x2d._gn_cache
            if hit[0] is self and hit[1] == bool(silu) and x2 is None:
                return hit[2]
        if getattr(x2d, "_unwritten", False):
            raise RuntimeError("this conv output was folded into its GroupNorm and never written")
        return O.groupnorm(x2d, self.weight, self.bias, m, hw, self.num_groups, self.eps, silu, x2=x2)


class LayerNorm(nn.Module):
    def __init__(self, dim, eps=1e-5):
        super().__init__()
        self.eps = eps
        self.weight = nn.Parameter(torch.empty(dim))
        self.bias = nn.Parameter(torch.empty(dim))

    def run(self, x2d):
        hit = getattr(x2d, "_ln_cache", None)
        if hit is not None:
            del x2d._ln_cache
            if hit[0] is self:
                return hit[1]
        return O.layernorm(x2d, self.weight, self.bias, self.eps)

    def forward(self, x):
        return self.run(x.reshape(-1, x.shape[-1])).reshape(x.shape)


LN_FOLD = __import__("os").environ.get("DD_LN_FOLD", "0")


def ln_fold_ok(norm, k, n=None, x=None):
    if LN_FOLD == "0" or not isinstance(norm, LayerNorm) or k not in (320, 640, 1280):
        return False
    if LN_FOLD == "stats":
        return x is not None and getattr(x, "_ln_stats", None) is not None
    return LN_FOLD == "all" or (n is not None and n <= k)


def want_ln_stats():
    return LN_FOLD == "stats"


LN_PRODUCER = __import__("os").environ.get("DD_LN_PRODUCER", "1") != "0"


def ln_producer_ok(lin, norm, kw):
    if not LN_PRODUCER or not isinstance(norm, LayerNorm) or lin.out_features != 320:
        return False
    if LN_FOLD != "0":
        return False
    if lin.w2d.shape[1] % 64 or kw.get("a2") is not None and kw["a2"].shape[1] % 64:
        return False
    bad = ("ln", "ln_stats", "head_major", "out_f32", "accumulate", "rowvec", "out", "tile", "split_k")
    return not any(kw.get(k) for k in bad) and kw.get("epilogue", O.DD_EPI_NONE) == O.DD_EPI_NONE \
        and kw.get("alpha", 1.0) == 1.0


def fp8_mfma_ok(norm, k, n, x2d):
    return isinstance(norm, LayerNorm) and k in (640, 1280) and n >= 3 * k and x2d.is_contiguous() \
        and getattr(x2d, "_ln_cache", None) is None


XATTN_FUSED = __import__("os").environ.get("DD_XATTN_FUSED", "1") != "0"


HEAD_MAJOR = __import__("os").environ.get("DD_ATTN_HEAD_MAJOR", "1") != "0"


def fold_layernorm(cache, key, norm, weights, biases):
    params = [norm.weight, norm.bias] + list(weights) + [b for b in biases if b is not None]
    ver = tuple((t._version, t.data_ptr()) for t in params)
    hit = cache.get(key)
    if hit is not None and hit[0] == ver:
        return hit[1], hit[2]
    with torch.no_grad():
        w = torch.cat([t.detach().reshape(t.shape[0], -1) for t in weights], dim=0).float()
        b = torch.cat([(bb.detach().float() if bb is not None else torch.zeros(t.shape[0], device=t.device))
                       for t, bb in zip(weights, biases)])
        wp = (w * norm.weight.detach().float()[None, :]).to(weights[0].dtype).contiguous()
        colsum = wp.float().sum(dim=1).contiguous()
        lnb = (w @ norm.bias.detach().float() + b).contiguous()
    cache[key] = (ver, wp, (colsum, lnb, norm.eps))
    return wp, (colsum, lnb, norm.eps)


class _Dropout(nn.Module):

    def forward(self, x):
        return x


class Timesteps(nn.Module):
    def __init__(self, num_channels, flip_sin_to_cos, downscale_freq_shift):
        super().__init__()
        self.num_channels, self.flip_sin_to_cos = num_channels, flip_sin_to_cos
        self.downscale_freq_shift = downscale_freq_shift

    def run(self, t_f32, dtype):
        return O.timestep_embedding(t_f32, self.num_channels, dtype, self.flip_sin_to_cos,
                                    float(self.downscale_freq_shift))


class TimestepEmbedding(nn.Module):
    def __init__(self, in_channels, time_embed_dim):
        super().__init__()
        self.linear_1 = Linear(in_channels, time_embed_dim)
        self.linear_2 = Linear(time_embed_dim, time_embed_dim)

    def run(self, t_emb):
        return self.linear_2.run(self.linear_1.run(t_emb, epilogue=O.DD_EPI_SILU))


class ResnetBlock2D(nn.Module):

    def __init__(self, in_channels, out_channels, temb_channels, groups=32, eps=1e-5):
        super().__init__()
        self.in_channels, self.out_channels = in_channels, out_channels
        self.norm1 = GroupNorm(groups, in_channels, eps)
        self.conv1 = Conv3x3(in_channels, out_channels)
        self.time_emb_proj = Linear(temb_channels, out_channels)
        self.norm2 = GroupNorm(groups, out_channels, eps)
        self.conv2 = Conv3x3(out_channels, out_channels)
        self.conv_shortcut = Linear(in_channels, out_channels, conv=True) if in_channels != out_channels else None

    def run(self, x, m, h, w, temb_vec, x2=None, extra_res=None, gn_next=None):
        hw = h * w
        a = self.norm1.run(x, m, hw, True, x2=x2)
        hid = self.conv1.run(a, m, h, w, rowvec=temb_vec, gn_next=(self.norm2, True, False))
        a = self.norm2.run(hid, m, hw, True)
        if self.conv_shortcut is not None:
            sc = self.conv_shortcut.run(x, a2=x2, res=extra_res)
        elif extra_res is not None:
            sc = O.add(x, extra_res)
        else:
            sc = x
        return self.conv2.run(a, m, h, w, res=sc, gn_next=None if gn_next is None else (gn_next, False, True))


class Downsample2D(nn.Module):
    def __init__(self, channels):
        super().__init__()
        self.conv = Conv3x3(channels, channels, stride=2)


class Upsample2D(nn.Module):
    def __init__(self, channels):
        super().__init__()
        self.conv = Conv3x3(channels, channels)


class HIPAttnProcessor:

    def __call__(self, attn, hidden_states, encoder_hidden_states=None, attention_mask=None, temb=None,
                 residual=None):
        if attention_mask is not None:
            raise NotImplementedError("attention_mask is None on the denoising path (blocks.py:166-187)")
        b, lq, c = hidden_states.shape
        x = hidden_states.reshape(b * lq, c)
        res2d = residual.reshape(b * lq, -1) if residual is not None else None
        if encoder_hidden_states is None:
            out = attn.run_self(x, b, lq, res=res2d)
        else:
            e = encoder_hidden_states
            out = attn.run_cross(x, b, lq, e.reshape(-1, e.shape[-1]), e.shape[1], res=res2d)
        return out.reshape(b, lq, -1)


class Attention(_Cached):

    def __init__(self, query_dim, cross_attention_dim=None, heads=8, dim_head=64, bias=False):
        super().__init__()
        inner = heads * dim_head
        self.inner_dim, self.heads, self.dim_head = inner, heads, dim_head
        self.scale = dim_head ** -0.5
        self.is_cross = cross_attention_dim is not None
        self.norm_cross = None
        self.group_norm = None
        self.spatial_norm = None
        self.residual_connection = False
        self.rescale_output_factor = 1.0
        self.to_q = Linear(query_dim, inner, bias=bias)
        self.to_k = Linear(cross_attention_dim or query_dim, inner, bias=bias)
        self.to_v = Linear(cross_attention_dim or query_dim, inner, bias=bias)
        self.to_out = nn.ModuleList([Linear(inner, query_dim), _Dropout()])
        self.processor = HIPAttnProcessor()

    def set_processor(self, processor):
        if isinstance(getattr(self, "processor", None), nn.Module) and not isinstance(processor, nn.Module):
            self._modules.pop("processor")
        self.processor = processor
        CACHE_EPOCH[0] += 1

    def prepare_attention_mask(self, attention_mask, target_length, batch_size=None, out_dim=3):
        if attention_mask is not None:
            raise NotImplementedError
        return None

    def head_to_batch_dim(self, t):
        b, l, c = t.shape
        return t.reshape(b, l, self.heads, c // self.heads).permute(0, 2, 1, 3).reshape(b * self.heads, l, -1)

    def batch_to_head_dim(self, t):
        bh, l, d = t.shape
        return t.reshape(bh // self.heads, self.heads, l, d).permute(0, 2, 1, 3).reshape(bh // self.heads, l, -1)

    def get_attention_scores(self, query, key, attention_mask=None):
        if attention_mask is not None:
            raise NotImplementedError("attention_mask is None on the denoising path")
        scores = torch.baddbmm(torch.empty((), dtype=query.dtype, device=query.device).expand(
            query.shape[0], query.shape[1], key.shape[1]), query, key.transpose(-1, -2), beta=0, alpha=self.scale)
        return scores.float().softmax(dim=-1).to(query.dtype)

    def _fused(self, names):
        key = "_pk_" + "".join(names)
        if key not in self.__dict__:
            self.__dict__[key] = torch.cat([getattr(self, n).weight.detach() for n in names], dim=0).contiguous()
        return self.__dict__[key]

    def _fused_bias(self, names):
        mods = [getattr(self, n) for n in names]
        if all(m.bias is None for m in mods):
            return None
        key = "_pk_b_" + "".join(names)
        if key not in self.__dict__:
            self.__dict__[key] = torch.cat([
                m.bias.detach() if m.bias is not None else m.weight.new_zeros(m.out_features) for m in mods]).contiguous()
        return self.__dict__[key]

    fp8_mfma = False

    def _hm(self, planes):
        return (self.dim_head, planes, self.scale * 1.4426950408889634)

    def project_qkv(self, x2d, norm=None, head_major=False):
        hm = self._hm(self.heads) if head_major else None
        names = ("to_q", "to_k", "to_v")
        if self.fp8_mfma and norm is not None and fp8_mfma_ok(norm, x2d.shape[1], 3 * self.inner_dim, x2d):
            key = "_pk_w8p_qkv"
            if key not in self.__dict__:
                self.__dict__[key] = O.quantize_fp8_padded(self._fused(names))
            w8, sw = self.__dict__[key]
            a8, sa = O.rowquant_fp8(x2d, (norm.weight, norm.bias, norm.eps))
            return O.gemm8(a8, sa, w8, sw, self._fused_bias(names), head_major=hm, dtype=x2d.dtype)
        if norm is not None:
            if not ln_fold_ok(norm, x2d.shape[1], 3 * self.inner_dim, x2d):
                return O.gemm(norm.run(x2d), self._fused(("to_q", "to_k", "to_v")),
                              self._fused_bias(("to_q", "to_k", "to_v")), head_major=hm)
            mods = (self.to_q, self.to_k, self.to_v)
            w, ln = fold_layernorm(self.__dict__, "_pk_ln_qkv", norm, [m.weight for m in mods], [m.bias for m in mods])
            return O.gemm(x2d, w, None, ln=ln, head_major=hm)
        return O.gemm(x2d, self._fused(("to_q", "to_k", "to_v")), self._fused_bias(("to_q", "to_k", "to_v")),
                      head_major=hm)

    def project_kv(self, ctx2d):
        return O.gemm(ctx2d, self._fused(("to_k", "to_v")), self._fused_bias(("to_k", "to_v")))

    def run_self(self, x2d, batch, lq, res=None, norm=None, ln_stats=False, ln_next=None):
        c, hd = self.inner_dim, self.heads
        if HEAD_MAJOR and self.to_q.bias is None:
            qkv = self.project_qkv(x2d, norm, head_major=True)
            o = O.attention(qkv[:hd], qkv[hd:2 * hd], qkv[2 * hd:], batch, lq, lq, hd, self.dim_head,
                            q_prescaled=True)
        else:
            qkv = self.project_qkv(x2d, norm)
            o = O.attention(qkv[:, :c], qkv[:, c:2 * c], qkv[:, 2 * c:], batch, lq, lq, hd,
                            self.dim_head, self.scale)
        return self.to_out[0].run(o, res=res, ln_stats=ln_stats, ln_next=ln_next)

    def run_cross(self, x2d, batch, lq, ctx2d, lk, res=None, kv=None, norm=None, ln_stats=False, ln_next=None):
        c = self.inner_dim
        pre = self.__dict__.pop("_kv_prefetched", None)
        if kv is None and pre is not None and pre[0] is ctx2d:
            kv, side = pre[1], pre[2]
            if side is not None:
                torch.cuda.current_stream().wait_stream(side)
                if not torch.cuda.is_current_stream_capturing():
                    kv.record_stream(torch.cuda.current_stream())
        if kv is None:
            kv = self.project_kv(ctx2d)
        lk_dev = lk_dev_for(ctx2d, lk)
# ... 351 lines not shown
```

dualdiff_amd/ops.py:

```python
import collections as _collections
import ctypes
import os as _os

import torch

from . import _native, _timer, _workspace, tuning
from ._native import DD_BF16, DD_EPI_GEGLU, DD_EPI_NONE, DD_EPI_SILU, DD_F16, AttnDesc, Gemm8Desc, GemmDesc, XAttnDesc
from ._timer import KernelTimer, _stream, set_timer
from ._workspace import workspace, workspace_owner
from .tuning import (CHALLENGE_TILES, TUNE_TABLE_PATH, forget_tuned, load_tuned, save_tuned,
                     tune_candidates, tuned_table)

_THIN_CONV = _os.environ.get("DD_THIN_CONV", "1") != "0"
GN_SPLITK = _os.environ.get("DD_GN_SPLITK", "0") == "1"
LN_OUT_TILE = int(_os.environ.get("DD_LN_OUT_TILE", "0"))
XATTN_MAX_WGS = int(_os.environ.get("DD_XATTN_MAX_WGS", "256"))
CAUSAL_ATTN_MAX_L = 128
_ZERO_BIAS = {}
_FDT = {torch.float16: 0, torch.bfloat16: 1, torch.float32: 2}


def _dtype_code(dtype):
    if dtype == torch.float16:
        return DD_F16
    if dtype == torch.bfloat16:
        return DD_BF16
    raise TypeError("dualdiff_amd ops take fp16 / bf16 tensors, got %s" % dtype)


def _dt(t):
    return _dtype_code(t.dtype)


def _tname(code):
    return "f16" if code == DD_F16 else "bf16"


def _need_gpu(*ts):
    for t in ts:
        if t is not None and not t.is_cuda:
            raise RuntimeError("dualdiff_amd ops run on the GPU only (got a %s tensor); "
                               "there is no CPU fallback" % t.device)


def _ptr(t):
    return ctypes.c_void_p(t.data_ptr()) if t is not None else None


def _forget_derived(t):
    for a in ("_ln_cache", "_ln_out", "_ln_stats", "_gn_cache", "_unwritten"):
        if hasattr(t, a):
            delattr(t, a)


def _out_or_new(out, shape, dtype, device, what):
    if out is None:
        return torch.empty_like(shape) if isinstance(shape, torch.Tensor) else torch.empty(shape, dtype=dtype, device=device)
    if out.dtype != dtype:
        raise TypeError("%s: out must be %s" % (what, dtype))
    _forget_derived(out)
    return out


def _rows2d(t):
    if t.dim() != 2 or t.stride(1) != 1:
        raise ValueError("expected a 2-D tensor with unit inner stride, got shape %s stride %s"
                         % (tuple(t.shape), t.stride()))
    return t


def _check_lk_dev(lk_dev):
    if lk_dev is not None and (lk_dev.dtype != torch.int32 or lk_dev.numel() < 1):
        raise TypeError("lk_dev must be an int32 device tensor")


def _epilogue_side(d, dtype, bias, rowvec, rows_per_inst, res, out, alpha, accumulate, epilogue, tile, split_k):
    d.bias = bias.data_ptr() if bias is not None else None
    if rowvec is not None:
        rowvec = _rows2d(rowvec)
        d.rowvec = rowvec.data_ptr(); d.ld_rowvec = rowvec.stride(0); d.rows_per_inst = rows_per_inst
    if res is not None:
        res = _rows2d(res)
        d.res = res.data_ptr(); d.ldres = res.stride(0)
    out = _rows2d(out)
    d.out = out.data_ptr(); d.ldc = out.stride(0)
    d.alpha = alpha; d.accumulate = int(accumulate); d.epilogue = epilogue
    d.dtype = dtype; d.tile = tile; d.split_k = split_k


def _tune(L, d, key, out_shape, dtype, device, warm):
    d.tile, d.split_k = tuning.tune(L, d, key, out_shape, dtype, device, warm, CHALLENGE_TILES)[:2]


def gemm(a, w, bias=None, *, a2=None, res=None, rowvec=None, rows_per_inst=1, alpha=1.0,
         out=None, accumulate=False, epilogue=DD_EPI_NONE, tile=0, split_k=0, ln=None, out_f32=False,
         ln_stats=False, head_major=None, ln_out=None):
    lib = _native.load()
    _need_gpu(a, w, bias, a2, res, rowvec, out)
    stats_in = getattr(a, "_ln_stats", None) if ln is not None else None
    a = _rows2d(a)
    w = _rows2d(w)
    rows = a.shape[0]
    k = a.shape[1] + (a2.shape[1] if a2 is not None else 0)
    n_w = w.shape[0]
    if w.shape[1] != k or not w.is_contiguous():
        raise ValueError("weight must be contiguous [N, K=%d], got %s" % (k, tuple(w.shape)))
    n = n_w // 2 if epilogue == DD_EPI_GEGLU else n_w
    odt = torch.float32 if out_f32 else a.dtype
    hm_out = None
    if head_major is not None:
        hd, hplanes, hscale = head_major
        if out is not None or n % hd or hd % 8 or out_f32 or epilogue != DD_EPI_NONE or accumulate or ln_stats:
            raise ValueError("head_major needs a plain epilogue, its own output and n % D == 0")
        hm_out = torch.empty((n // hd, rows, hd), dtype=a.dtype, device=a.device)
        out = hm_out.view(rows, n)
    out = _out_or_new(out, (rows, n), odt, a.device, "gemm")
    d = GemmDesc()
    d.out_f32 = int(bool(out_f32))
    if hm_out is not None:
        d.out_headmajor_d, d.hm_scaled_planes, d.hm_scale = int(hd), int(hplanes), float(hscale)
    d.a = a.data_ptr(); d.lda = a.stride(0); d.k1 = a.shape[1]
    if a2 is not None:
        a2 = _rows2d(a2)
        d.a2 = a2.data_ptr(); d.lda2 = a2.stride(0)
    d.rows, d.n, d.k = rows, n, k
    d.w = w.data_ptr()
    d.conv = 0
    _epilogue_side(d, _dt(a), bias, rowvec, rows_per_inst, res, out, alpha, accumulate, epilogue, tile, split_k)
    if ln is not None:
        if bias is not None or a2 is not None:
            raise ValueError("gemm(ln=...) folds the bias and takes a single source")
        colsum, lnb, eps = ln
        _need_gpu(colsum, lnb)
        if colsum.dtype != torch.float32 or lnb.dtype != torch.float32 or colsum.numel() != n_w or lnb.numel() != n_w:
            raise ValueError("ln fold vectors must be fp32 with %d entries" % n_w)
        d.ln_colsum, d.ln_bias, d.ln_eps = colsum.data_ptr(), lnb.data_ptr(), float(eps)
        if stats_in is not None:
            if tuple(stats_in.shape) != (rows, k // 32, 2) or stats_in.dtype != torch.float32:
                raise ValueError("stale LayerNorm statistics attached to the input")
            d.ln_stats_in = stats_in.data_ptr()
    if w.dtype != a.dtype:
        raise TypeError("gemm: weight dtype %s != activation dtype %s" % (w.dtype, a.dtype))
    ln_second = None
    if ln_out is not None:
        g_, b_, eps_ = ln_out
        _need_gpu(g_, b_)
        if n != 320 or g_.numel() != n or b_.numel() != n or g_.dtype != a.dtype or b_.dtype != a.dtype:
            raise ValueError("ln_out needs n == 320 and %s gamma / beta of 320 entries" % a.dtype)
        ln_second = torch.empty((rows, n), dtype=a.dtype, device=a.device)
        d.ln_out, d.ld_ln_out = ln_second.data_ptr(), n
        d.lno_gamma, d.lno_beta, d.ln_eps = g_.data_ptr(), b_.data_ptr(), float(eps_)
        if tile not in (40, 74):
            tile = LN_OUT_TILE
        d.tile, d.split_k = tile, 1
        tile = -1
    stats_out = None
    if ln_stats:
        if n % 32 or epilogue == DD_EPI_GEGLU or out_f32:
            raise ValueError("ln_stats needs a plain epilogue and n % 32 == 0")
        stats_out = torch.empty((rows, n // 32, 2), dtype=torch.float32, device=a.device)
        d.ln_stats_out = stats_out.data_ptr()
    L = tuning.launcher(lib)
    if tile == 0 and split_k == 0:
        key = tuning.gemm_key(rows, n, k, epilogue, d.dtype, a2 is not None, ln is not None, out_f32=out_f32,
                              stats_out=ln_stats, stats_in=stats_in is not None,
                              head_major=head_major[0] if head_major is not None else None, res=res is not None,
                              acc=accumulate)
        _tune(L, d, key, (rows, n), odt, a.device, (a, a2, res))
    _workspace.attach(d, a.device, lambda: L.ws_bytes(d))
    _timer.gemm_launch(L, d, "gemm", "gemm", n_w, rows * k)
    if stats_out is not None:
        out._ln_stats = stats_out
    if ln_second is not None:
        out._ln_out = ln_second
    return hm_out if hm_out is not None else out


def thin_conv_ok(cin, cout, stride, m):
    return _THIN_CONV and (cin, cout, stride) in ((8, 16, 1), (16, 16, 1), (16, 32, 2), (32, 32, 1), (8, 32, 1), (16, 32, 1),
                                                  (16, 16, 2), (8, 16, 2), (32, 16, 1)) and m <= 65535


def conv3x3(x, w, bias, m, hin, win, *, stride=1, up_size=None, rowvec=None, res=None,
            alpha=1.0, out=None, accumulate=False, epilogue=DD_EPI_NONE, tile=0, split_k=0, gn_next=None, pad=1):
    lib = _native.load()
    _need_gpu(x, w, bias, res, rowvec, out)
    x = _rows2d(x)
    cin = x.shape[1]
    if not x.is_contiguous() or x.shape[0] != m * hin * win:
        raise ValueError("conv input must be contiguous (m*h*w, cin)")
    hv, wv = (hin, win) if up_size is None else (int(up_size[0]), int(up_size[1]))
    if pad not in (0, 1):
        raise ValueError("conv3x3: pad is 1 (nn.Conv2d(padding=1)) or 0 (Downsample2D(padding=0))")
    if pad == 0 and (stride != 2 or up_size is not None or hin < 2 or win < 2):
        raise ValueError("conv3x3(pad=0) is the stride-2 downsample of an image of at least 2 x 2 pixels, without upsample")
    hout = (hv + pad + 1 - 3) // stride + 1
    wout = (wv + pad + 1 - 3) // stride + 1
    cout = w.shape[0]
    if w.shape[1] != 9 * cin or not w.is_contiguous():
        raise ValueError("conv weight must be contiguous [cout, 9*cin]")
    rows = m * hout * wout
    out = _out_or_new(out, (rows, cout), x.dtype, x.device, "conv3x3")
    if pad == 1 and thin_conv_ok(cin, cout, stride, m) and up_size is None and rowvec is None and res is None and alpha == 1.0 \
            and not accumulate and epilogue in (DD_EPI_NONE, DD_EPI_SILU) and tile == 0 and split_k == 0 \
            and out.is_contiguous():
        def book():
            suffix, flops, nbytes = _timer.mm_cost("conv", rows, cout, 9 * cin, x.numel(), cout)
            return "dd_conv3x3_thin_kernel" + suffix, flops, nbytes
        _timer.launch("conv3x3_thin", lib.dd_conv3x3_thin, _ptr(x), _ptr(w), _ptr(bias), _ptr(out), m, hin, win, cin, cout,
                      stride, int(epilogue == DD_EPI_SILU), _dt(x), _stream(), book=book)
        return out
    d = GemmDesc()
    d.a = x.data_ptr(); d.lda = cin; d.k1 = 9 * cin
    d.rows, d.n, d.k = rows, cout, 9 * cin
    d.w = w.data_ptr()
    d.conv = 1
    d.hin, d.win, d.cin, d.hv, d.wv = hin, win, cin, hv, wv
    d.hout, d.wout, d.stride = hout, wout, stride
    _epilogue_side(d, _dt(x), bias, rowvec, hout * wout, res, out, alpha, accumulate, epilogue, tile, split_k)
    L = tuning.launcher(lib, pad)
    what = "conv3x3" if pad == 1 else "conv3x3(pad=0)"
    if tile == 0 and split_k == 0:
        key = (tuning.conv_key if pad == 1 else tuning.conv_pad0_key)(m, hin, win, cin, cout, stride, hv, wv, d.dtype)
        _tune(L, d, key, (rows, cout), x.dtype, x.device, (x, res))
    need = _workspace.attach(d, x.device, lambda: L.ws_bytes(d))
    if pad == 1 and gn_next is not None and GN_SPLITK and need > 0 and alpha == 1.0 and not accumulate \
            and epilogue == DD_EPI_NONE:
        gmod, gsilu, want_x = gn_next
        split = _timer.plan_of(L, d)[1]
        if split > 1 and lib.dd_groupnorm_is_fused(hout * wout, cout, gmod.num_groups):
            y = torch.empty((rows, cout), dtype=x.dtype, device=x.device)
            _timer.gemm_launch(L, d, what, "conv", cout, x.numel(), reduce=False)
            _timer.launch("groupnorm_splitk", lib.dd_groupnorm_splitk, ctypes.c_void_p(d.ws + 65536), split, _ptr(bias),
                          _ptr(rowvec), rowvec.stride(0) if rowvec is not None else 0, _ptr(res),
                          res.stride(0) if res is not None else 0, _ptr(out) if want_x else None,
                          _ptr(gmod.weight), _ptr(gmod.bias), _ptr(y), m, hout * wout, cout,
                          gmod.num_groups, float(gmod.eps), int(gsilu), _dt(x), _stream(),
                          book=lambda: ("dd_gn_splitk_kernel", 0.0,
                                        4.0 * split * rows * cout + 2.0 * rows * cout * (2 if want_x else 1)))
            out._gn_cache = (gmod, bool(gsilu), y)
            if not want_x:
                out._unwritten = True
            return out
    _timer.gemm_launch(L, d, what, "conv", cout, x.numel())
    return out


def vae_posterior(moments, wq, bq, m, h, w, noise=None, scale=1.0, out_f32=False):
    lib = _native.load()
    _need_gpu(moments, wq, bq, noise)
    if moments.shape != (m * h * w, 8) or not moments.is_contiguous():
        raise ValueError("moments must be contiguous (m*h*w, 8), got %s" % (tuple(moments.shape),))
    if wq.dtype != torch.float32 or bq.dtype != torch.float32 or wq.numel() != 64 or bq.numel() != 8 \
            or not wq.is_contiguous() or not bq.is_contiguous():
        raise ValueError("quant_conv weight / bias must be contiguous fp32 (8, 8) / (8,)")
    if noise is not None and (noise.shape != (m, 4, h, w) or noise.dtype != moments.dtype or not noise.is_contiguous()):
        raise ValueError("noise must be a contiguous %s (%d, 4, %d, %d) tensor" % (moments.dtype, m, h, w))
    z = torch.empty((m, 4, h, w), dtype=torch.float32 if out_f32 else moments.dtype, device=moments.device)
    _native.check(lib.dd_vae_posterior(_ptr(moments), _ptr(wq), _ptr(bq), _ptr(noise), _ptr(z), m, h, w, float(scale),
                                       int(bool(out_f32)), _dt(moments), _stream()), "vae_posterior")
    return z


def _image_arg(x, what):
    if x.dim() != 4 or x.shape[1] != 3 or x.numel() == 0:
        raise ValueError("%s takes an (m, 3, h, w) image batch, got %s" % (what, tuple(x.shape)))
    if x.dtype not in _FDT:
        raise ValueError("%s takes fp16 / bf16 / fp32 images, got %s" % (what, x.dtype))
    if not x.is_contiguous():
        raise ValueError("%s takes a contiguous NCHW tensor" % what)
    return x.shape[0], x.shape[2], x.shape[3]


def _image_out(out, shape, device, what):
    if out is None:
        return torch.empty(shape, dtype=torch.uint8, device=device)
    if out.dtype != torch.uint8 or tuple(out.shape) != tuple(shape) or not out.is_contiguous():
        raise ValueError("%s: out must be a contiguous uint8 %s tensor" % (what, tuple(shape)))
    return out


def image_padding(padding):
    if isinstance(padding, int) and not isinstance(padding, bool):
        p = (padding,) * 4
    else:
        try:
            p = tuple(padding)
        except TypeError:
            raise ValueError("padding must be an int or a sequence of 2 or 4 ints, got %r" % (padding,))
        if len(p) == 1:
            p = p * 4
        elif len(p) == 2:
            p = (p[0], p[1], p[0], p[1])
    if len(p) != 4 or any(isinstance(v, bool) or not isinstance(v, int) or v < 0 for v in p):
        raise ValueError("padding must be an int or a sequence of 2 or 4 non-negative ints, got %r" % (padding,))
    return p


def image_quantize_u8(x, m11=False, out=None):
    m, h, w = _image_arg(x, "image_quantize_u8")
    out = _image_out(out, (m, h, w, 3), x.device, "image_quantize_u8")
    _need_gpu(x, out)
    lib = _native.load()
    _timer.launch("image_quantize_u8", lib.dd_image_quantize_u8, _ptr(x), _ptr(out), m, h, w, int(bool(m11)),
                  _FDT[x.dtype], _stream(),
                  book=lambda: ("dd_image_quantize_kernel", 0.0, float(x.numel() * x.element_size() + out.numel())))
    return out


def image_resample_u8(x, size, padding=(0, 0, 0, 0), fill=0, m11=False, out=None):
    m, h, w = _image_arg(x, "image_resample_u8")
    try:
        oh, ow = (int(v) for v in size)
    except (TypeError, ValueError):
        raise ValueError("size must be (h, w), got %r" % (size,))
    if oh <= 0 or ow <= 0:
        raise ValueError("size must be positive, got %r" % (size,))
    pl, pt, pr, pb = image_padding(padding)
    if isinstance(fill, bool) or not isinstance(fill, int) or not 0 <= fill <= 255:
        raise ValueError("fill must be a byte value, got %r" % (fill,))
    out = _image_out(out, (m, pt + oh + pb, pl + ow + pr, 3), x.device, "image_resample_u8")
    _need_gpu(x, out)
    lib = _native.load()
    from .pipeline.image_output import device_tables
    kx, bx = device_tables(w, ow, x.device)
    ky, by = device_tables(h, oh, x.device)
    _timer.launch("image_resample_u8", lib.dd_image_resample_u8, _ptr(x), _ptr(out), m, h, w, oh, ow, _ptr(kx), _ptr(bx),
                  kx.shape[1], _ptr(ky), _ptr(by), ky.shape[1], pl, pt, pr, pb, fill, int(bool(m11)), _FDT[x.dtype],
                  _stream(),
                  book=lambda: ("dd_image_resample_kernel", 0.0, float(x.numel() * x.element_size() + out.numel())))
    return out


_IMAGE_LUTS = {}
_IMAGE_LAYOUTS = {"nchw": 0, "nhwc8": 1}


def _image_mean_std(mean, std):
    try:
        mean, std = tuple(float(v) for v in mean), tuple(float(v) for v in std)
    except (TypeError, ValueError):
        raise ValueError("mean and std must be 3 numbers each, got %r / %r" % (mean, std))
    if len(mean) != 3 or len(std) != 3:
        raise ValueError("mean and std must be 3 numbers each, got %r / %r" % (mean, std))
    if any(v == 0 for v in std):
        raise ValueError("std must not be 0 (Normalize would divide by zero), got %r" % (std,))
    return mean, std


def image_norm_lut(mean, std):
    mean, std = _image_mean_std(mean, std)
    x = torch.arange(256).float().div(255)
    mean, std = torch.tensor(mean, dtype=torch.float32), torch.tensor(std, dtype=torch.float32)
    return x[None].sub(mean[:, None]).div(std[:, None]).contiguous()


def _image_lut(mean, std, device):
    key = (mean, std, device.type,
           device.index if device.index is not None else torch.cuda.current_device())
    if key not in _IMAGE_LUTS:
        _IMAGE_LUTS[key] = image_norm_lut(mean, std).to(device)
    return _IMAGE_LUTS[key]


def image_load_u8(frames, size, box=None, mean=(0.5, 0.5, 0.5), std=(0.5, 0.5, 0.5), dtype=torch.float32, layout="nchw",
                  out=None):
    what = "image_load_u8"
    if frames.dim() != 4 or frames.shape[3] != 3 or frames.numel() == 0:
        raise ValueError("%s takes an (m, h, w, 3) frame batch, got %s" % (what, tuple(frames.shape)))
    if frames.dtype != torch.uint8:
        raise ValueError("%s takes uint8 frames, got %s" % (what, frames.dtype))
    if not frames.is_contiguous():
        raise ValueError("%s takes a contiguous NHWC tensor" % what)
    m, h, w = frames.shape[0], frames.shape[1], frames.shape[2]
    try:
        nh, nw = (int(v) for v in size)
    except (TypeError, ValueError):
        raise ValueError("size must be (h, w), got %r" % (size,))
    if nh <= 0 or nw <= 0:
        raise ValueError("size must be positive, got %r" % (size,))
    if box is None:
        box = (0, 0, nw, nh)
    try:
        left, top, right, bottom = (int(v) for v in box)
    except (TypeError, ValueError):
        raise ValueError("box must be (left, top, right, bottom), got %r" % (box,))
    if not (0 <= left < right <= nw and 0 <= top < bottom <= nh):
        raise ValueError("box %r is empty or leaves the %d x %d (w x h) resized image" % (tuple(box), nw, nh))
    if layout not in _IMAGE_LAYOUTS:
        raise ValueError("layout must be one of %s, got %r" % (", ".join(sorted(_IMAGE_LAYOUTS)), layout))
    if dtype not in _FDT:
        raise ValueError("%s writes fp16 / bf16 / fp32, got %s" % (what, dtype))
    mean, std = _image_mean_std(mean, std)
    oh, ow = bottom - top, right - left
    shape = (m, 3, oh, ow) if layout == "nchw" else (m * oh * ow, 8)
    if out is None:
        _need_gpu(frames)
        out = torch.empty(shape, dtype=dtype, device=frames.device)
    elif out.dtype != dtype or tuple(out.shape) != shape or not out.is_contiguous():
        raise ValueError("%s: out must be a contiguous %s %s tensor" % (what, dtype, shape))
    _need_gpu(frames, out)
    _forget_derived(out)
    lib = _native.load()
    from .pipeline.image_output import device_tables
    kx, bx = device_tables(w, nw, frames.device)
    ky, by = device_tables(h, nh, frames.device)
    lut = _image_lut(mean, std, frames.device)
    _timer.launch(what, lib.dd_image_load_u8, _ptr(frames), _ptr(out), m, h, w, oh, ow, _ptr(kx[left:]), _ptr(bx[left:]),
                  kx.shape[1], _ptr(ky[top:]), _ptr(by[top:]), ky.shape[1], _ptr(lut), _FDT[dtype],
                  _IMAGE_LAYOUTS[layout], _stream(),
                  book=lambda: ("dd_image_load_kernel", 0.0, float(frames.numel() + out.numel() * out.element_size())))
    return out


BOX_POINT_MODES = {"all-xyz": 0, "cxyz": 1}
BOX_FILTERS = {"all": 0, "positive_z": 1, "canvas": 2}


def box_views(corners, labels, offsets, transforms, views, cap, points_mode="all-xyz", filter_mode="positive_z",
              canvas_size=None, filter_corners=None, out=None):
    what = "box_views"
    if points_mode not in BOX_POINT_MODES:
        raise ValueError("%s: points_mode must be one of %s, got %r" % (what, ", ".join(sorted(BOX_POINT_MODES)), points_mode))
    if filter_mode not in BOX_FILTERS:
        raise ValueError("%s: filter_mode must be one of %s, got %r" % (what, ", ".join(sorted(BOX_FILTERS)), filter_mode))
    if corners.dim() != 3 or tuple(corners.shape[1:]) != (8, 3) or corners.dtype != torch.float32:
        raise ValueError("%s takes fp32 corners (total, 8, 3), got %s %s" % (what, corners.dtype, tuple(corners.shape)))
    total = corners.shape[0]
    if labels.dtype != torch.int64 or tuple(labels.shape) != (total,):
        raise ValueError("%s takes int64 labels (%d,), got %s %s" % (what, total, labels.dtype, tuple(labels.shape)))
    if offsets.dtype != torch.int32 or offsets.dim() != 1 or offsets.shape[0] < 2:
        raise ValueError("%s takes int32 offsets (scenes + 1,), got %s %s" % (what, offsets.dtype, tuple(offsets.shape)))
    scenes, views, cap = offsets.shape[0] - 1, int(views), int(cap)
    if views <= 0 or cap <= 0:
        raise ValueError("%s: views and cap must be positive, got %d and %d" % (what, views, cap))
    fm = BOX_FILTERS[filter_mode]
    if fm == 0 and views != 1:
        raise ValueError("%s: filter \"all\" is the view-shared form and has one view, got %d" % (what, views))
    if fm != 0 and (transforms is None or transforms.dtype != torch.float32
                    or tuple(transforms.shape) != (scenes, views, 4, 4)):
        raise ValueError("%s: filter %r takes fp32 transforms (%d, %d, 4, 4)" % (what, filter_mode, scenes, views))
    ch = cw = 0
    if fm == 2:
        try:
            ch, cw = (int(v) for v in canvas_size)
        except (TypeError, ValueError):
            raise ValueError("%s: filter \"canvas\" takes canvas_size = (h, w), got %r" % (what, canvas_size))
        if ch <= 0 or cw <= 0:
            raise ValueError("%s: canvas_size must be positive, got %r" % (what, canvas_size))
    if filter_corners is not None and (filter_corners.dtype != torch.float32 or filter_corners.shape != corners.shape):
        raise ValueError("%s: filter_corners must match corners" % what)
    ins = (corners, labels, offsets, transforms, filter_corners)
    if any(t is not None and not t.is_contiguous() for t in ins):
        raise ValueError("%s takes contiguous tensors" % what)
    _need_gpu(*ins)
    pts = 8 if BOX_POINT_MODES[points_mode] == 0 else 4
    shapes = ((scenes, views, cap, pts, 3), (scenes, views, cap), (scenes, views, cap), (scenes, views), (1,))
    dtypes = (torch.float32, torch.int64, torch.bool, torch.int32, torch.int32)
    if out is None:
        out = tuple(torch.empty(s, dtype=d, device=corners.device) for s, d in zip(shapes, dtypes))
    else:
        out = tuple(out)
        if len(out) != 5 or any(tuple(t.shape) != s or t.dtype != d or not t.is_contiguous()
                                for t, s, d in zip(out, shapes, dtypes)):
            raise ValueError("%s: out must be contiguous tensors of %s" % (what, list(zip(shapes, dtypes))))
        _need_gpu(*out)
    lib = _native.load()
    _timer.launch(what, lib.dd_box_views, _ptr(corners), _ptr(filter_corners), _ptr(labels), _ptr(offsets),
                  _ptr(transforms) if fm != 0 else None, total, scenes, views, cap, BOX_POINT_MODES[points_mode], fm, ch, cw,
                  *(_ptr(t) for t in out), _stream(),
                  book=lambda: ("dd_box_views_kernel", 0.0,
                                float((1 if fm == 0 else views) * total * 96 + out[0].numel() * 4 + out[1].numel() * 9)))
    return out


def groupnorm(x, gamma, beta, m, hw, groups, eps, silu, x2=None, out=None):
    lib = _native.load()
    _need_gpu(x, gamma, beta, x2, out)
    c1 = x.shape[1]
    c2 = x2.shape[1] if x2 is not None else 0
    if not x.is_contiguous() or (x2 is not None and not x2.is_contiguous()):
        raise ValueError("groupnorm inputs must be contiguous")
    out = _out_or_new(out, (m * hw, c1 + c2), x.dtype, x.device, "groupnorm")
    need = lib.dd_groupnorm_workspace_bytes(m, groups)
    ws = workspace(need, x.device, "gn")

    def book():
        th = lib.dd_groupnorm_is_fused(hw, c1 + c2, groups)
        return ("dd_gn_fused_kernel<%s, %d, 8>" % (_tname(_dt(x)), th) if th
                else "dd_gn_stats_kernel + dd_gn_apply_kernel (2 launches)", 0.0, (4.0 if th else 6.0) * out.numel())
    _timer.launch("groupnorm", lib.dd_groupnorm_nhwc, _ptr(x), c1, _ptr(x2), c2, _ptr(gamma), _ptr(beta), _ptr(out),
                  m, hw, groups, eps, int(silu), _dt(x), _ptr(ws), ws.numel() * 4, _stream(), book=book)
    return out


def layernorm(x, gamma, beta, eps=1e-5, out=None):
    lib = _native.load()
    _need_gpu(x, gamma, beta, out)
    x = _rows2d(x)
    if not x.is_contiguous():
        raise ValueError("layernorm input must be contiguous")
    out = _out_or_new(out, x, x.dtype, x.device, "layernorm")
    _timer.launch("layernorm", lib.dd_layernorm, _ptr(x), _ptr(gamma), _ptr(beta), _ptr(out), x.shape[0], x.shape[1],
                  eps, _dt(x), _stream(), book=lambda: ("dd_layernorm", 0.0, 4.0 * out.numel()))
    return out


def attention(q, k, v, batch, lq, lk, heads, head_dim, scale=None, *, kv_batch_map=None,
              out=None, accumulate=False, variant=0, q_prescaled=False, seq_strides=None,
              out_seq_strides=None, kv_batch_map2=None, kv_seq_strides=None, lk_dev=None):
    lib = _native.load()
    _need_gpu(q, k, v, out, kv_batch_map, kv_batch_map2, lk_dev)
    _check_lk_dev(lk_dev)
    if kv_batch_map2 is not None and (kv_batch_map is None or seq_strides is not None):
        raise ValueError("kv_batch_map2 needs kv_batch_map and no seq_strides")
    if kv_seq_strides is not None and seq_strides is None:
        raise ValueError("kv_seq_strides needs seq_strides")
    d = AttnDesc()

    def operand(t, l):
        if t.dim() == 4:
            if t.shape[1] != heads or t.shape[2] != l or t.shape[3] != head_dim or t.stride(3) != 1 \
                    or t.stride(2) != head_dim:
                raise ValueError("batch-major operand must be (batches, heads, l, head_dim) with contiguous blocks")
            return t.data_ptr(), head_dim, t.stride(0), t.stride(1)
        if t.dim() == 3:
            if t.shape[0] != heads or t.shape[2] != head_dim or t.stride(2) != 1 or t.stride(1) != head_dim:
# ... 529 lines not shown
```

dualdiff_amd/tuning.py:

```python
import ast
import collections
import ctypes
import json
import os

import torch

from . import _workspace
from ._native import DD_EPI_GEGLU
from ._timer import _stream

_AUTOTUNE = os.environ.get("DD_AUTOTUNE", "1") != "0"
_COLD = os.environ.get("DD_AUTOTUNE_COLD", "1") != "0"
CHALLENGE_TILES = tuple(int(t) for t in os.environ.get("DD_TUNE_CHALLENGE", "").split(",") if t.strip())
TUNE_TABLE_PATH = os.path.join(os.path.dirname(os.path.abspath(__file__)), "tuned", "gfx950.json")
_TUNED = {}
_TABLE_LOADED = False
_CHALLENGED = set()
_FLUSH = {}
_TILES = None
_SPLITS = (1, 2, 3, 4, 5, 6, 8, 12, 16)


def gemm_key(rows, n, k, epilogue, dtype, a2=False, ln=False, *, out_f32=False, stats_out=False, stats_in=False,
             head_major=None, res=False, acc=False):
    return (("g", rows, n, k, epilogue, dtype, bool(a2), bool(ln))
            + (("f32",) if out_f32 else ()) + (("so",) if stats_out else ()) + (("si",) if stats_in else ())
            + (("hm", head_major) if head_major is not None else ())
            + (("res",) if res else ()) + (("acc",) if acc else ()))


def conv_key(m, hin, win, cin, cout, stride, hv, wv, dtype):
    return ("c", m, hin, win, cin, cout, stride, hv, wv, dtype)


def conv_pad0_key(m, hin, win, cin, cout, stride, hv, wv, dtype):
    return conv_key(m, hin, win, cin, cout, stride, hv, wv, dtype) + ("p0",)


def _entry(v):
    return (int(v[0]), int(v[1]), int(v[2]) if len(v) > 2 else 0)


def tuned_table():
    return dict(_TUNED)


def save_tuned(path, merge=True):
    entries = {}
    if merge and os.path.exists(path):
        with open(path) as f:
            for k, v in json.load(f).get("entries", []):
                entries[ast.literal_eval(k)] = _entry(v)
    entries.update(_TUNED)
    os.makedirs(os.path.dirname(os.path.abspath(path)), exist_ok=True)
    with open(path, "w") as f:
        json.dump({"arch": "gfx950", "entries": [[repr(k), list(v)] for k, v in sorted(entries.items(), key=repr)]}, f, indent=0)


def load_tuned(path):
    with open(path) as f:
        blob = json.load(f)
    if blob.get("arch") != "gfx950":
        raise RuntimeError("tune cache %s is not for gfx950" % path)
    n = 0
    for k, v in blob["entries"]:
        key = ast.literal_eval(k)
        if key not in _TUNED:
            _TUNED[key] = _entry(v)
            n += 1
    return n


def _load_default_table():
    global _TABLE_LOADED
    if _TABLE_LOADED:
        return
    _TABLE_LOADED = True
    path = os.environ.get("DD_TUNE_TABLE", TUNE_TABLE_PATH)
    if path != "0" and os.path.exists(path):
        load_tuned(path)


def forget_tuned():
    global _TABLE_LOADED
    _TUNED.clear()
    _TABLE_LOADED = True


class Launcher(collections.namedtuple("Launcher", "lib pad_lo launch ws_bytes kernel_name")):
    """How a GemmDesc is launched for a given top / left padding: launch(d, stream) -> rc, ws_bytes(d), kernel_name(d)
    -> plan string.  What the tuner times is what the caller launches afterwards."""


def launcher(lib, pad_lo=1):
    if pad_lo == 1:
        return Launcher(lib, 1, lambda d, st: lib.dd_gemm(ctypes.byref(d), st),
                        lambda d: lib.dd_gemm_workspace_bytes(ctypes.byref(d)),
                        lambda d: lib.dd_gemm_kernel_name(ctypes.byref(d)).decode())
    return Launcher(lib, pad_lo, lambda d, st: lib.dd_gemm_conv_pad(ctypes.byref(d), pad_lo, st),
                    lambda d: lib.dd_gemm_conv_pad_workspace_bytes(ctypes.byref(d), pad_lo),
                    lambda d: lib.dd_gemm_conv_pad_kernel_name(ctypes.byref(d), pad_lo).decode())


def tune_candidates(lib, d):
    global _TILES
    if _TILES is None:
        _TILES = tuple(lib.dd_gemm_tile_id(i) for i in range(lib.dd_gemm_num_tiles()))
    kt = (d.k + 63) // 64
    blocks128 = ((d.rows + 127) // 128) * ((d.n + 127) // 128)
    return [(tile, split) for tile in _TILES for split in _SPLITS
            if split == 1 or not (d.epilogue == DD_EPI_GEGLU or kt < 4 * split or blocks128 * split > 4096)]


def _capturing():
    return torch.cuda.is_current_stream_capturing()


def _flush_and_warm(device, warm):
    buf = _FLUSH.get(device)
    if buf is None:
        buf = _FLUSH[device] = torch.empty(320 << 20, dtype=torch.uint8, device=device)
    buf.zero_()
    for t in warm:
        if t is not None:
            t.sum()


def _time_launch(L, d, device, warm, tile, split, iters):
    d.tile, d.split_k = tile, split
    _workspace.attach(d, device, lambda: L.ws_bytes(d))
    stream = _stream()
    if L.launch(d, stream) != 0:
        return None
    e0, e1 = torch.cuda.Event(enable_timing=True), torch.cuda.Event(enable_timing=True)
    if not _COLD:
        e0.record()
        for _ in range(iters):
            L.launch(d, stream)
        e1.record()
        e1.synchronize()
        return e0.elapsed_time(e1) / iters
    samples = []
    for _ in range(iters):
        _flush_and_warm(device, warm)
        e0.record()
        L.launch(d, stream)
        e1.record()
        e1.synchronize()
        samples.append(e0.elapsed_time(e1))
    samples.sort()
    return samples[len(samples) // 2]


def tune(L, d, key, out_shape, dtype, device, warm=(), challenge_tiles=()):
    _load_default_table()
    hit = _TUNED.get(key)
    if hit is not None and (not challenge_tiles or key in _CHALLENGED or _capturing()):
        return hit
    if hit is None and (not _AUTOTUNE or _capturing()):
        return 0, 0, 0
    saved = (d.out, d.ldc, d.accumulate, d.tile, d.split_k, d.ws, d.ws_bytes)
    scratch = torch.empty(out_shape, dtype=dtype, device=device)
    d.out, d.ldc, d.accumulate = scratch.data_ptr(), scratch.stride(0), 0
    try:
        best = _challenge(L, d, key, hit, device, warm, challenge_tiles) if hit is not None else _sweep(L, d, device, warm)
    finally:
        (d.out, d.ldc, d.accumulate, d.tile, d.split_k, d.ws, d.ws_bytes) = saved
    if best[0] != 0:
        _TUNED[key] = best
    return best


def _sweep(L, d, device, warm):
    best, best_t = (0, 0, 0), float("inf")
    cands = []
    excl = {int(t) for t in os.environ.get("DD_TUNE_EXCLUDE", "").split(",") if t.strip()}
    for tile, split in tune_candidates(L.lib, d):
        if tile in excl:
            continue
        t = _time_launch(L, d, device, warm, tile, split, 3)
        if t is not None:
            cands.append((t, tile, split))
    cands.sort()
    for t, tile, split in cands[:8]:
        t2 = _time_launch(L, d, device, warm, tile, split, 15 if _COLD else 12)
        if t2 is not None and t2 < best_t:
            best, best_t = (tile, split, 0), t2
    return best


def _challenge(L, d, key, hit, device, warm, challenge_tiles):
    _CHALLENGED.add(key)
    t_inc = _time_launch(L, d, device, warm, hit[0], hit[1], 21)
    best, best_t = tuple(hit), (t_inc if t_inc is not None else float("inf"))
    for tile in challenge_tiles:
        for split in sorted({1, max(1, int(hit[1]))}):
            if (tile, split) == tuple(hit[:2]):
                continue
            t = _time_launch(L, d, device, warm, tile, split, 5)
            if t is None or t > 1.1 * best_t:
                continue
            t = _time_launch(L, d, device, warm, tile, split, 21)
            if t is not None and t < 0.97 * best_t:
                best, best_t = (tile, split, 0), t
    if best != tuple(hit):
        print("[tune] %s: %s -> %s (%.1f -> %.1f us)" % (key, tuple(hit), best, t_inc * 1e3, best_t * 1e3), flush=True)
    return best
```

include/dualdiff_hip.h:

```cpp
#ifndef DUALDIFF_HIP_H
#define DUALDIFF_HIP_H

#include <stdint.h>

#ifdef __cplusplus
extern "C" {
#endif

#define DD_ABI_VERSION 4

enum { DD_F16 = 0, DD_BF16 = 1 };

enum {
  DD_OK = 0,
  DD_ERR_BAD_ARG = -1,
  DD_ERR_UNSUPPORTED = -2,
  DD_ERR_LAUNCH = -3,
  DD_ERR_WORKSPACE = -4
};

typedef void* dd_stream_t;

int dd_abi_version(void);
int64_t dd_desc_size(int which);
const char* dd_error_string(int code);
const char* dd_target_arch(void);

enum { DD_EPI_NONE = 0, DD_EPI_GEGLU = 1, DD_EPI_SILU = 2 };

typedef struct dd_gemm_desc {
  const void* a;
  const void* a2;
  int64_t lda, lda2;
  int32_t k1;
  int32_t rows, n, k;
  const void* w;
  const void* bias;
  const void* rowvec;
  int32_t rows_per_inst, ld_rowvec;
  const void* res;
  int64_t ldres;
  void* out;
  int64_t ldc;
  float alpha;
  int32_t accumulate;
  int32_t epilogue;
  int32_t conv;
  int32_t hin, win, cin;
  int32_t hv, wv;
  int32_t hout, wout, stride;
  int32_t dtype;
  int32_t tile;
  int32_t split_k;
  void* ws;
  int64_t ws_bytes;
  const void* ln_colsum;
  const void* ln_bias;
  float ln_eps;
  int32_t out_f32;
  void* ln_stats_out;
  const void* ln_stats_in;
  int32_t out_headmajor_d;
  int32_t hm_scaled_planes;
  float hm_scale;
  int32_t phase;
  void* ln_out;
  int64_t ld_ln_out;
  const void* lno_gamma;
  const void* lno_beta;
} dd_gemm_desc;

int dd_gemm(const dd_gemm_desc* d, dd_stream_t stream);
int64_t dd_gemm_workspace_bytes(const dd_gemm_desc* d);
int dd_gemm_num_tiles(void);
int dd_gemm_tile_id(int index);
const char* dd_gemm_kernel_name(const dd_gemm_desc* d);

int dd_gemm_conv_pad(const dd_gemm_desc* d, int32_t pad_lo, dd_stream_t stream);
int64_t dd_gemm_conv_pad_workspace_bytes(const dd_gemm_desc* d, int32_t pad_lo);
const char* dd_gemm_conv_pad_kernel_name(const dd_gemm_desc* d, int32_t pad_lo);

int dd_groupnorm_nhwc(const void* x1, int32_t c1, const void* x2, int32_t c2,
                      const void* gamma, const void* beta, void* y,
                      int32_t m, int32_t hw, int32_t groups, float eps,
                      int32_t apply_silu, int32_t dtype, void* ws, int64_t ws_bytes,
                      dd_stream_t stream);
int64_t dd_groupnorm_workspace_bytes(int32_t m, int32_t groups);
int dd_groupnorm_is_fused(int32_t hw, int32_t c, int32_t groups);
int dd_groupnorm_splitk(const float* partial, int32_t nsplit, const void* bias, const void* rowvec, int32_t ld_rowvec,
                        const void* res, int64_t ldres, void* x_out, const void* gamma, const void* beta, void* y,
                        int32_t m, int32_t hw, int32_t c, int32_t groups, float eps, int32_t apply_silu, int32_t dtype,
                        dd_stream_t stream);

int dd_layernorm(const void* x, const void* gamma, const void* beta, void* y,
                 int64_t rows, int32_t c, float eps, int32_t dtype, dd_stream_t stream);

typedef struct dd_attn_desc {
  const void* q; const void* k; const void* v; void* o;
  int64_t ldq, ldk, ldv, ldo;
  int64_t q_batch_stride, k_batch_stride, v_batch_stride, o_batch_stride;
  int32_t batch, heads, head_dim, lq, lk;
  float scale;
  const int32_t* kv_batch_map;
  int32_t accumulate;
  int32_t dtype;
  int32_t variant;
  int64_t q_head_stride, k_head_stride, v_head_stride;
  int32_t q_prescaled;
  const int32_t* kv_batch_map2;
  const int32_t* lk_dev;
} dd_attn_desc;

int dd_attention(const dd_attn_desc* d, dd_stream_t stream);
const char* dd_attention_kernel_name(const dd_attn_desc* d);

typedef struct dd_xattn_desc {
  const void* x; int64_t ldx;
  const void* res; int64_t ldres;
  const void* wq; const void* wo; const void* bo;
  const void* k; const void* v; int64_t ldk, ldv;
  int64_t k_inst_stride, k_head_stride, v_inst_stride, v_head_stride;
  void* out; int64_t ldo;
  int32_t instances, rows_per_inst, lk;
  int32_t channels, heads;
  float scale;
  int32_t dtype;
  void* ln_out; int64_t ld_ln_out;
  const void* ln_gamma; const void* ln_beta; float ln_eps;
  const int32_t* lk_dev;
} dd_xattn_desc;

int dd_xattn320(const dd_xattn_desc* d, dd_stream_t stream);
int dd_xattn_pack_weight(const void* w, void* packed, int32_t dtype, dd_stream_t stream);

int dd_add(const void* a, const void* b, const void* c, void* y, int64_t n,
           int32_t dtype, dd_stream_t stream);
int dd_scale(const void* x, void* y, float s, int64_t n, int32_t dtype, dd_stream_t stream);
int dd_silu(const void* x, void* y, int64_t n, int32_t dtype, dd_stream_t stream);

int dd_nchw_to_nhwc(const void* x, void* y, int32_t m, int32_t c, int32_t hw,
                    int32_t c_pad, int32_t dtype, dd_stream_t stream);
int dd_nhwc_to_nchw(const void* x, void* y, int32_t m, int32_t c, int32_t hw,
                    int32_t ldx, int32_t dtype, dd_stream_t stream);

int dd_timestep_embedding(const float* t, void* out, int32_t n, int32_t dim,
                          int32_t flip_sin_to_cos, float freq_shift,
                          int32_t dtype, dd_stream_t stream);

#define DD_F32 2
int dd_fourier_embed(const void* x, void* out, int64_t rows, int32_t dims, const float* freqs,
                     int32_t num_freqs, int32_t include_input, int32_t in_dtype, int32_t out_dtype,
                     dd_stream_t stream);

int dd_nchw_to_nhwc_views(const void* x, void* y, int32_t m, int32_t c, int32_t h, int32_t w, int32_t views,
                          int32_t c_pad, int32_t dtype, dd_stream_t stream);
int dd_fourier_embed_strided(const void* x, void* out, int64_t rows, int32_t dims, const float* freqs,
                             int32_t num_freqs, int32_t include_input, int32_t in_dtype, int32_t out_dtype,
                             int32_t inner, int64_t stride_outer, int64_t stride_inner, int64_t stride_dim,
                             int64_t out_ld, dd_stream_t stream);
typedef struct dd_box_tokens_desc {
  const void* points; const int64_t* classes; const uint8_t* masks;
  const void* class_tokens; const void* null_pos; const void* null_class;
  void* pos; void* cat; void* cls_out;
  int32_t rows, points_per_box, num_freqs, include_input, class_token_dim, cls_offset;
  int64_t ld_cat;
  int32_t normalize, points_dtype, dtype;
  int32_t n_classes;
  float freqs[16]; float xyz_min[3]; float xyz_range[3];
} dd_box_tokens_desc;
int dd_box_tokens(const dd_box_tokens_desc* d, dd_stream_t stream);
int dd_ctx_assemble(const void* cam, const void* text, const void* box, void* full, void* txt, int32_t m,
                    int32_t n_cam, int32_t lt, int32_t nbox, int32_t dim, int32_t text_per_view, int32_t box_views,
                    int32_t dtype, dd_stream_t stream);

int dd_ors_project(const uint8_t* occ, const float* origin, const float* dir, uint8_t* labels, void* cond,
                   int32_t n_cam, int32_t hw, int32_t samples, float step, int32_t keep_fg, int32_t keep_bg,
                   int32_t dtype, dd_stream_t stream);

int dd_softmax_rows(const float* s, void* p, int64_t rows, int32_t cols, int64_t lds, int64_t ldp,
                    int32_t dtype, dd_stream_t stream);

int dd_conv3x3_small_cout(const void* x, const void* w, const void* bias, void* y_nchw,
                          int32_t m, int32_t h, int32_t wd, int32_t cin, int32_t cout,
                          int32_t dtype, dd_stream_t stream);

int dd_vae_posterior(const void* moments, const float* wq, const float* bq, const void* noise, void* z,
                     int32_t m, int32_t h, int32_t w, float scale, int32_t out_f32, int32_t dtype, dd_stream_t stream);

int dd_image_quantize_u8(const void* x, uint8_t* out, int32_t m, int32_t h, int32_t w, int32_t m11, int32_t dtype,
                         dd_stream_t stream);

#define DD_IMAGE_MAX_KSIZE 33
int dd_image_resample_u8(const void* x, uint8_t* out, int32_t m, int32_t h, int32_t w, int32_t oh, int32_t ow,
                         const int32_t* kx, const int32_t* bx, int32_t ksx, const int32_t* ky, const int32_t* by,
                         int32_t ksy, int32_t pad_l, int32_t pad_t, int32_t pad_r, int32_t pad_b, int32_t fill,
                         int32_t m11, int32_t dtype, dd_stream_t stream);

int dd_image_load_u8(const uint8_t* in, void* out, int32_t m, int32_t h, int32_t w, int32_t oh, int32_t ow,
                     const int32_t* kx, const int32_t* bx, int32_t ksx, const int32_t* ky, const int32_t* by,
                     int32_t ksy, const float* lut, int32_t dtype, int32_t layout, dd_stream_t stream);

int dd_box_views(const float* corners, const float* filter_corners, const int64_t* labels, const int32_t* offsets,
                 const float* transforms, int32_t total, int32_t scenes, int32_t views, int32_t cap,
                 int32_t points_mode, int32_t filter_mode, int32_t canvas_h, int32_t canvas_w, float* bboxes,
                 int64_t* classes, uint8_t* masks, int32_t* counts, int32_t* max_len, dd_stream_t stream);

int dd_clip_embed(const int64_t* ids, const void* tok, const void* pos, void* out, int32_t* pool_index,
                  int32_t batch, int32_t l, int32_t c, int32_t vocab, int32_t eos_token_id, int32_t dtype,
                  dd_stream_t stream);

#define DD_CAUSAL_ATTN_MAX_L 128
int dd_causal_attention(const void* q, const void* k, const void* v, void* o, int64_t ldq, int64_t ldk, int64_t ldv,
                        int64_t ldo, int64_t q_batch_stride, int64_t k_batch_stride, int64_t v_batch_stride,
                        int64_t o_batch_stride, int32_t batch, int32_t l, int32_t heads, int32_t head_dim, float scale,
                        int32_t dtype, dd_stream_t stream);

int dd_conv3x3_thin(const void* x, const void* w, const void* bias, void* y, int32_t m, int32_t hin, int32_t win,
                    int32_t cin, int32_t cout, int32_t stride, int32_t silu, int32_t dtype, dd_stream_t stream);

int dd_cfg_ddim_step(const void* eps, const void* x, void* x_out, void* x_dup,
                     const float* coef, float guidance, int64_t n,
                     int32_t dtype, dd_stream_t stream);

int dd_cfg_unipc_step(const void* eps, const void* x, void* x_out, void* x_dup, float* last, float* m1,
                      float* m2, const float* coef, float guidance, int64_t n, int32_t dtype,
                      dd_stream_t stream);

int dd_cfg_ddim_step_given(const void* eps, const void* x, void* x_out, void* x_dup, const float* coef,
                           float guidance, const uint8_t* given, const float* clean, const void* noise0,
                           const float* gcoef, int32_t mode, int64_t n, int64_t view_elems, int32_t dtype,
                           dd_stream_t stream);
int dd_cfg_unipc_step_given(const void* eps, const void* x, void* x_out, void* x_dup, float* last, float* m1,
                            float* m2, const float* coef, float guidance, const uint8_t* given, const float* clean,
                            const void* noise0, const float* gcoef, int32_t mode, int64_t n, int64_t view_elems,
                            int32_t dtype, dd_stream_t stream);

int dd_given_views_noise(void* x, void* x_dup, const uint8_t* given, const float* clean, const void* noise0,
                         float sqrt_acp, float sqrt_1m_acp, int64_t n, int64_t view_elems, int32_t dtype,
                         dd_stream_t stream);

int dd_rowquant_fp8(const void* x, const void* gamma, const void* beta, void* q, float* scale, int64_t rows, int32_t c,
                    int64_t ldq, float eps, int32_t dtype, dd_stream_t stream);

typedef struct dd_gemm8_desc {
  const void* a; const float* a_scale; int64_t lda;
  const void* w; const float* w_scale; int64_t ldw;
  const void* bias; const void* res; int64_t ldres;
  void* out; int64_t ldc;
  int32_t rows, n, k_padded;
  int32_t dtype;
  int32_t out_headmajor_d, hm_scaled_planes; float hm_scale;
  int32_t geglu;
} dd_gemm8_desc;

int dd_gemm8(const dd_gemm8_desc* d, dd_stream_t stream);

int dd_probe_spin(uint64_t* stamps, uint32_t ticks_100mhz, dd_stream_t stream);

#ifdef __cplusplus
}
#endif
#endif
```

Before: 90.52 steps/s.

## Fold nearest-upsample into 3x3 conv as per-parity 2x2 convs

Adds a folded form for a 3x3 conv that follows a nearest-neighbour upsample. Output pixels are grouped into up to nine phase classes, and for each class the 3x3 weights are summed into a 2x2 kernel. A new ring-GEMM kernel variant then gathers only 4 input taps instead of 9, with class-ordered tiles and a row-mapped store. This cuts the K dimension of the up-block convs by more than half, at the cost of extra folded weight memory, more index math and more complex scattered output writes. Fp32-summed weights may differ slightly numerically from the unfolded conv.

```diff
diff --git a/dualdiff_amd/_build.py b/dualdiff_amd/_build.py
--- a/dualdiff_amd/_build.py
+++ b/dualdiff_amd/_build.py
@@ -9,8 +9,8 @@
 LIBDIR = os.path.join(HERE, "lib")
 OBJDIR = os.path.join(HERE, "lib", "obj")
 LIBNAME = "libdualdiff_hip.so"
-GEMM_SOURCES = ["gemm23.hip", "gemm2_conv.hip", "gemm1.hip", "conv3s.hip", "gemm2_geglu.hip", "gemm4.hip", "gemm.hip"]
-SOURCES = ["gemm23.hip", "gemm2_conv.hip", "attention.hip", "gemm1.hip", "conv3s.hip", "gemm2_geglu.hip", "gemm4.hip",
+GEMM_SOURCES = ["gemm23.hip", "gemm2_conv.hip", "gemm2_upfold.hip", "gemm1.hip", "conv3s.hip", "gemm2_geglu.hip", "gemm4.hip", "gemm.hip"]
+SOURCES = ["gemm23.hip", "gemm2_conv.hip", "attention.hip", "gemm1.hip", "conv3s.hip", "gemm2_upfold.hip", "gemm2_geglu.hip", "gemm4.hip",
            "norm.hip", "elementwise.hip", "tokens.hip", "xattn.hip", "clip.hip", "gemm8.hip", "vae.hip", "image.hip", "boxes.hip", "gemm.hip"]
 EXTRA_FLAGS = {"attention.hip": ["-mllvm", "-amdgpu-mfma-vgpr-form=1", "-fno-honor-nans"],
                **{src: ["-mllvm", "-amdgpu-mfma-vgpr-form=1"] for src in GEMM_SOURCES},
diff --git a/dualdiff_amd/_native.py b/dualdiff_amd/_native.py
--- a/dualdiff_amd/_native.py
+++ b/dualdiff_amd/_native.py
@@ -27,6 +27,7 @@
         ("out_headmajor_d", c_int32), ("hm_scaled_planes", c_int32), ("hm_scale", c_float),
         ("phase", c_int32),
         ("ln_out", c_void_p), ("ld_ln_out", c_int64), ("lno_gamma", c_void_p), ("lno_beta", c_void_p),
+        ("upfold", c_int32),
     ]
 
 
diff --git a/dualdiff_amd/csrc/gemm.hip b/dualdiff_amd/csrc/gemm.hip
--- a/dualdiff_amd/csrc/gemm.hip
+++ b/dualdiff_amd/csrc/gemm.hip
@@ -1,5 +1,6 @@
 #include "gemm_device.h"
 #include <algorithm>
+#include <cmath>
 
 namespace {
 
@@ -37,6 +38,61 @@
     if (d->a2) ok = ok && (d->k1 % BK) == 0 && (int64_t)d->rows * d->lda2 < lim;
   }
   return ok;
+}
+
+int upfold_src(int o, int in, int out) { return std::min((int)floorf((float)o * ((float)in / (float)out)), in - 1); }
+
+int upfold_class(int o, int in, int out) {
+  const int s = upfold_src(o, in, out);
+  for (int c = 0; c < 3; ++c) {
+    bool ok = true;
+    for (int t = -1; t <= 1 && ok; ++t) {
+      const bool tap_in = o + t >= 0 && o + t < out;
+      if (c == 2 && t == 1) { ok = !tap_in; continue; }
+      const int src = (c == 1 ? s : s - 1) + (c == 1 ? t == 1 : t >= 0);
+      const bool src_in = src >= 0 && src < in;
+      ok = tap_in ? src_in && upfold_src(o + t, in, out) == src : !src_in;
+    }
+    if (ok) return c;
+  }
+  return -1;
+}
+
+bool upfold_axis(int in, int out, uint8_t* list, uint8_t* n, uint8_t* start) {
+  if (in <= 0 || out <= in || out > kUpfoldMax) return false;
+  int pos = 0;
+  for (int c = 0; c < 3; ++c) {
+    start[c] = (uint8_t)pos;
+    for (int o = 0; o < out; ++o) {
+      const int k = upfold_class(o, in, out);
+      if (k < 0) return false;
+      if (k == c) list[pos++] = (uint8_t)o;
+    }
+    n[c] = (uint8_t)(pos - start[c]);
+  }
+  return true;
+}
+
+bool upfold_tab(const dd_gemm_desc* d, int bm, UpfoldTab* t, int* tiles_m, int* ncls) {
+  *t = UpfoldTab{};
+  if (!d->conv || d->stride != 1 || d->hout != d->hv || d->wout != d->wv || d->hout <= 0 || d->wout <= 0) return false;
+  if (!upfold_axis(d->hin, d->hv, t->y, t->ny, t->y0) || !upfold_axis(d->win, d->wv, t->x, t->nx, t->x0)) return false;
+  t->m = d->rows / (d->hout * d->wout);
+  int tiles = 0, w = 0;
+  for (int c = 0; c < 9; ++c) {
+    const int plane = t->ny[c / 3] * t->nx[c % 3];
+    t->tile0[c] = (uint16_t)tiles;
+    t->widx[c] = (uint8_t)w;
+    t->inv_plane[c] = plane ? 1.0f / (float)plane : 1.0f;
+    if (plane) ++w;
+    tiles += (t->m * plane + bm - 1) / bm;
+    if (tiles > 65535) return false;
+  }
+  t->tile0[9] = (uint16_t)tiles;
+  for (int c = 0; c < 3; ++c) t->inv_nx[c] = t->nx[c] ? 1.0f / (float)t->nx[c] : 1.0f;
+  *tiles_m = tiles;
+  *ncls = w;
+  return true;
 }
 
 bool env_is_zero(const char* name) { const char* v = getenv(name); return v && atoi(v) == 0; }
@@ -86,7 +142,7 @@
 }
 
 unsigned form_of(const dd_gemm_desc* d, int pad_lo) {
-  return pad_lo == 0 ? F_PAD0 : d->conv ? F_CONV : d->epilogue == DD_EPI_GEGLU ? F_GEGLU : F_DENSE;
+  return pad_lo == 0 ? F_PAD0 : d->conv && d->upfold ? F_UPFOLD : d->conv ? F_CONV : d->epilogue == DD_EPI_GEGLU ? F_GEGLU : F_DENSE;
 }
 
 Plan make_plan(const dd_gemm_desc* d, int pad_lo) {
@@ -102,6 +158,10 @@
       if ((long)ceil_div(d->rows, tile_bm(t)) * ceil_div(d->n, bn_out) >= (long)kNumCU * 3 / 2) break;
     }
   }
+  if (ti < 0) {
+    if (form != F_UPFOLD) return unsupported();
+    ti = tile_index(d->rows >= 8192 ? 28 : 52);
+  }
   if (d->ln_colsum) {
     const int ring = twin(kTiles[ti], FAM_RING);
     if (d->tile <= 0 && ring >= 0) ti = ring;
@@ -117,6 +177,7 @@
     if (d->n != 320 || !dma_ok(d)) return unsupported();
   }
   if (kTiles[ti].family == FAM_DIRECT) return plan_direct(d, ti, form);
+  if (form == F_UPFOLD && (kTiles[ti].family != FAM_RING || !dma_ok(d) || d->ln_stats_out || d->out_f32)) return unsupported();
   if (kTiles[ti].family != FAM_REG && !dma_ok(d)) {
     const int reg = twin(kTiles[ti], FAM_REG);
     ti = reg >= 0 ? reg : tile_index(geglu ? kTile128x128 : kTile64x64);
@@ -128,6 +189,11 @@
   pl.tile_idx = ti;
   pl.tiles_m = ceil_div(d->rows, tile_bm(t));
   pl.tiles_n = ceil_div(d->n, bn_out);
+  if (form == F_UPFOLD) {
+    int ncls = 0;
+    if (!upfold_tab(d, tile_bm(t), &pl.upf, &pl.tiles_m, &ncls) || (int64_t)ncls * d->n * d->k >= ((int64_t)1 << 30))
+      return unsupported();
+  }
   int split = d->split_k;
   const int nkt = ceil_div(d->k, BK);
   if (split <= 0) {
@@ -159,7 +225,7 @@
 LaunchFn* launcher(const Plan& pl, unsigned form) {
   switch (kTiles[pl.tile_idx].family) {
     case FAM_REG: return launch_gemm1;
-    case FAM_RING: return form == F_CONV ? launch_gemm2_conv : form == F_GEGLU ? launch_gemm2_geglu : launch_gemm2_dense;
+    case FAM_RING: return form == F_UPFOLD ? launch_gemm2_upfold : form == F_CONV ? launch_gemm2_conv : form == F_GEGLU ? launch_gemm2_geglu : launch_gemm2_dense;
     case FAM_PIPE: return gemm4_takes(pl) ? launch_gemm4 : launch_gemm3;
     default: return launch_conv3s;
   }
@@ -190,7 +256,7 @@
   if (d->rowvec && (!dd_aligned16(d->rowvec) || (d->ld_rowvec & 7) || d->rows_per_inst <= 0)) return DD_ERR_BAD_ARG;
   if (d->conv) {
     if (d->a2) return DD_ERR_UNSUPPORTED;
-    if (d->cin <= 0 || (d->cin & 7) || d->k != 9 * d->cin) return DD_ERR_BAD_ARG;
+    if (d->cin <= 0 || (d->cin & 7) || d->k != (d->upfold ? 4 : 9) * d->cin) return DD_ERR_BAD_ARG;
     if (d->hin <= 0 || d->win <= 0 || d->hout <= 0 || d->wout <= 0) return DD_ERR_BAD_ARG;
     if (d->stride != 1 && d->stride != 2) return DD_ERR_UNSUPPORTED;
     if (d->hv <= 0 || d->wv <= 0) return DD_ERR_BAD_ARG;
@@ -214,6 +280,7 @@
   }
   if (d->epilogue == DD_EPI_GEGLU && (d->res || d->rowvec || d->accumulate || d->alpha != 1.0f)) return DD_ERR_UNSUPPORTED;
   if (d->epilogue == DD_EPI_GEGLU && d->conv) return DD_ERR_UNSUPPORTED;
+  if (d->upfold && (!d->conv || pad_lo != 1)) return DD_ERR_BAD_ARG;
   return DD_OK;
 }
 
@@ -261,6 +328,9 @@
   } else if (t.family == FAM_PIPE) {
     kern = gemm4_takes(pl) ? "dd_gemm4_kernel" : "dd_gemm3_kernel";
     snprintf(args, sizeof(args), ", %d, %s", t.depth, geglu);
+  } else if (t.family == FAM_RING && d->upfold) {
+    kern = "dd_gemm2u_kernel";
+    snprintf(args, sizeof(args), ", %d", t.depth);
   } else if (t.family == FAM_RING) {
     kern = "dd_gemm2_kernel";
     snprintf(args, sizeof(args), ", %d, %s, %s", t.depth, conv, geglu);
@@ -309,6 +379,11 @@
   {
     const int64_t nw = (d->epilogue == DD_EPI_GEGLU ? 2 : 1) * (int64_t)d->n;
     p.w_bytes = (uint32_t)(nw * d->k * 2);
+    if (d->upfold) {
+      int ncls = 0;
+      for (int c = 0; c < 9; ++c) ncls += pl.upf.tile0[c + 1] > pl.upf.tile0[c];
+      p.w_bytes = (uint32_t)(ncls * nw * d->k * 2);
+    }
     if (d->conv) {
       p.a_bytes = (uint32_t)((int64_t)d->rows / (d->hout * d->wout) * d->hin * d->win * d->cin * 2);
       p.a2_bytes = 0;
diff --git a/dualdiff_amd/csrc/gemm2_kernel.h b/dualdiff_amd/csrc/gemm2_kernel.h
--- a/dualdiff_amd/csrc/gemm2_kernel.h
+++ b/dualdiff_amd/csrc/gemm2_kernel.h
@@ -8,9 +8,9 @@
   return (!CONV && NW == 4 && TM * TN <= 8 && NSTAGE <= 3) ? 2 : 1;
 }
 
-template <typename T, int WAVES_M, int WAVES_N, int TM, int TN, int NSTAGE, bool CONV, bool GEGLU>
-__global__ __launch_bounds__(64 * WAVES_M * WAVES_N, (gemm2_min_blocks<WAVES_M * WAVES_N, TM, TN, NSTAGE, CONV>()))
-void dd_gemm2_kernel(const GemmParams p) {
+template <typename T, int WAVES_M, int WAVES_N, int TM, int TN, int NSTAGE, bool CONV, bool GEGLU, bool UPF>
+__device__ __forceinline__ void dd_gemm2_body(const GemmParams& p, const UpfoldTab* u) {
+  static_assert(!UPF || (CONV && !GEGLU), "the folded upsample is a conv form");
   using V8 = typename dd_vec<T>::v8;
   constexpr int NW = WAVES_M * WAVES_N;
   constexpr int BM = WAVES_M * TM * 16;
@@ -42,6 +42,37 @@
   int tile = xcd_remap(lin, ntiles);
   int block_m0 = (tile / p.tiles_n) * BM;
   int block_n0 = (tile % p.tiles_n) * BN_OUT;
+  int u_rc = 0, u_cc = 0, u_widx = 0, u_ny = 1, u_nx = 1, u_y0 = 0, u_x0 = 0, u_rows = 0;
+  float u_inv_plane = 1.f, u_inv_nx = 1.f;
+  if constexpr (UPF) {
+    const int tmi = tile / p.tiles_n;
+    int cls = 0;
+#pragma unroll
+    for (int c = 1; c < 9; ++c) if (tmi >= (int)u->tile0[c]) cls = c;
+    int t0 = 0;
+#pragma unroll
+    for (int c = 0; c < 9; ++c)
+      if (c == cls) { t0 = u->tile0[c]; u_widx = u->widx[c]; u_inv_plane = u->inv_plane[c]; }
+    u_rc = (cls * 11) >> 5;
+    u_cc = cls - u_rc * 3;
+#pragma unroll
+    for (int c = 0; c < 3; ++c) {
+      if (c == u_rc) { u_ny = u->ny[c]; u_y0 = u->y0[c]; }
+      if (c == u_cc) { u_nx = u->nx[c]; u_x0 = u->x0[c]; u_inv_nx = u->inv_nx[c]; }
+    }
+    u_rows = u->m * u_ny * u_nx;
+    block_m0 = (tmi - t0) * BM;
+  }
+  auto u_pixel = [&](const int r, int& inst, int& oy, int& ox) __attribute__((always_inline)) {
+    const bool rv = r < u_rows;
+    const int rr = rv ? r : 0;
+    inst = dd_fdiv(rr, u_inv_plane);
+    const int rem = rr - inst * (u_ny * u_nx);
+    const int iy = dd_fdiv(rem, u_inv_nx);
+    oy = u->y[u_y0 + iy];
+    ox = u->x[u_x0 + rem - iy * u_nx];
+    return rv;
+  };
 
   const int kbeg = blockIdx.z * p.k_per_split;
   const int kend = min(p.k, kbeg + p.k_per_split);
@@ -71,7 +102,7 @@
       const int col = bn0 + loc;
       n_glob = (col < p.n) ? col : -1;
     }
-    wv[j] = n_glob >= 0 ? (uint32_t)n_glob * (uint32_t)p.k * 2u + lcb : DD_OOB;
+    wv[j] = n_glob >= 0 ? (uint32_t)(UPF ? u_widx * p.n + n_glob : n_glob) * (uint32_t)p.k * 2u + lcb : DD_OOB;
   }
   };
   make_wv(block_n0);
@@ -82,8 +113,31 @@
 #pragma unroll
   for (int j = 0; j < XI; ++j) {
     const int r = block_m0 + (j * NW + wave) * 8 + lrow;
-    const bool rv = r < p.rows;
-    if (CONV) {
+    [[maybe_unused]] const bool rv = r < p.rows;
+    if constexpr (UPF) {
+      int inst, oy, ox;
+      const bool uv = u_pixel(r, inst, oy, ox);
+      const int sy0 = min((int)floorf(oy * p.scale_h), p.hin - 1) - (u_rc != 1);
+      const int sx0 = min((int)floorf(ox * p.scale_w), p.win - 1) - (u_cc != 1);
+      uint32_t bits = 0;
+#pragma unroll
+      for (int t = 0; t < 2; ++t) {
+        const int iy = sy0 + t, ix = sx0 + t;
+        const bool vy = iy >= 0 && iy < p.hin, vx = ix >= 0 && ix < p.win;
+        const int sy = min(max(iy, 0), p.hin - 1), sx = min(max(ix, 0), p.win - 1);
+        syo[j][t] = (uint32_t)((inst * p.hin + sy) * p.win) * (uint32_t)p.cin * 2u + lcb;
+        sxo[j][t] = (uint32_t)(sx * p.cin) * 2u;
+        if (vy) bits |= 1u << t;
+        if (vx) bits |= 4u << t;
+      }
+      syo[j][2] = sxo[j][2] = 0;
+      uint32_t m4 = 0;
+#pragma unroll
+      for (int t = 0; t < 4; ++t)
+        if (uv && ((bits >> (t >> 1)) & 1u) && ((bits >> (2 + (t & 1))) & 1u)) m4 |= 1u << t;
+      xbits[j] = m4;
+      xe[j] = DD_OOB;
+    } else if (CONV) {
       const int hw = p.hout * p.wout;
       const int rr = rv ? r : 0;
       const int inst = dd_fdiv(rr, p.inv_hw);
@@ -128,8 +182,8 @@
   };
   auto set_tap = [&](int tap) __attribute__((always_inline)) {
     if (CONV) {
-      const int ky = (tap * 11) >> 5;
-      const int kx = tap - ky * 3;
+      const int ky = UPF ? tap >> 1 : (tap * 11) >> 5;
+      const int kx = UPF ? tap & 1 : tap - ky * 3;
       const uint32_t y0 = 0u - (uint32_t)(ky == 0), y1 = 0u - (uint32_t)(ky == 1), y2 = 0u - (uint32_t)(ky == 2);
       const uint32_t x0 = 0u - (uint32_t)(kx == 0), x1 = 0u - (uint32_t)(kx == 1), x2 = 0u - (uint32_t)(kx == 2);
 #pragma unroll
@@ -315,6 +369,17 @@
     }
   }
   const bool ln = !CONV && p.ln_colsum;
+  if constexpr (UPF) {
+    int rowmap[TM];
+#pragma unroll
+    for (int tm = 0; tm < TM; ++tm) {
+      int inst, oy, ox;
+      const bool uv = u_pixel(block_m0 + wave_m * (TM * 16) + tm * 16 + (lane & 15), inst, oy, ox);
+      rowmap[tm] = uv ? (inst * p.hout + oy) * p.wout + ox : p.rows;
+    }
+    store_tile<T, TM, TN, false, true>(p, acc, block_m0, block_n0, wave_m, wave_n, lane, p.rows, nullptr, nullptr, rowmap);
+    break;
+  }
   store_tile<T, TM, TN, GEGLU>(p, acc, block_m0, block_n0, wave_m, wave_n, lane, p.rows,
                                ln ? s_ln_mean : nullptr, ln ? s_ln_rstd : nullptr);
   if (!have_next) break;
@@ -329,6 +394,18 @@
     for (int j = 0; j < TM; ++j) acc[i][j] = f32x4{0.f, 0.f, 0.f, 0.f};
   }
   DD_STAMP_FLUSH(p);
+}
+
+template <typename T, int WAVES_M, int WAVES_N, int TM, int TN, int NSTAGE, bool CONV, bool GEGLU>
+__global__ __launch_bounds__(64 * WAVES_M * WAVES_N, (gemm2_min_blocks<WAVES_M * WAVES_N, TM, TN, NSTAGE, CONV>()))
+void dd_gemm2_kernel(const GemmParams p) {
+  dd_gemm2_body<T, WAVES_M, WAVES_N, TM, TN, NSTAGE, CONV, GEGLU, false>(p, nullptr);
+}
+
+template <typename T, int WAVES_M, int WAVES_N, int TM, int TN, int NSTAGE>
+__global__ __launch_bounds__(64 * WAVES_M * WAVES_N, (gemm2_min_blocks<WAVES_M * WAVES_N, TM, TN, NSTAGE, true>()))
+void dd_gemm2u_kernel(const GemmParams p, const UpfoldTab u) {
+  dd_gemm2_body<T, WAVES_M, WAVES_N, TM, TN, NSTAGE, true, false, true>(p, &u);
 }
 
 struct Gemm2 {
@@ -360,4 +437,20 @@
   }
 };
 
+
+struct Gemm2U {
+  static constexpr Family family = FAM_RING;
+  static constexpr unsigned needs = 0;
+  template <typename T, size_t I, unsigned FORM>
+  static int run(const GemmParams& p, const Plan& pl, hipStream_t s) {
+    constexpr const TileCfg& t = kTiles[I];
+    constexpr size_t smem = (size_t)t.depth * (tile_bm(t) + tile_bn(t)) * BK * sizeof(T);
+    static_assert(smem <= 160 * 1024, "LDS");
+    constexpr auto kern = dd_gemm2u_kernel<T, t.wm, t.wn, t.tm, t.tn, t.depth>;
+    raise_lds_limit<kern>(smem);
+    hipLaunchKernelGGL(kern, dim3(pl.tiles_m * pl.tiles_n, 1, pl.split), dim3(64 * t.wm * t.wn), smem, s, p, pl.upf);
+    return dd_check_launch();
+  }
+};
+
 }
diff --git a/dualdiff_amd/csrc/gemm2_upfold.hip b/dualdiff_amd/csrc/gemm2_upfold.hip
--- /dev/null
+++ b/dualdiff_amd/csrc/gemm2_upfold.hip
@@ -0,0 +1,5 @@
+#include "gemm2_kernel.h"
+
+int ddg::launch_gemm2_upfold(int dtype, unsigned form, const GemmParams& p, const Plan& pl, hipStream_t s) {
+  return dispatch<Gemm2U, F_UPFOLD>(dtype, form, p, pl, s);
+}
diff --git a/dualdiff_amd/csrc/gemm_device.h b/dualdiff_amd/csrc/gemm_device.h
--- a/dualdiff_amd/csrc/gemm_device.h
+++ b/dualdiff_amd/csrc/gemm_device.h
@@ -75,10 +75,12 @@
   return base + (bid >> 3);
 }
 
-template <typename T, int TM, int TN, bool GEGLU>
+template <typename T, int TM, int TN, bool GEGLU, bool MAPPED = false>
 __device__ __forceinline__ void store_tile(const GemmParams& p, f32x4 (&acc)[TN][TM], int block_m0,
                                            int block_n0, int wave_m, int wave_n, int lane, int row_end,
-                                           const float* ln_mean = nullptr, const float* ln_rstd = nullptr) {
+                                           const float* ln_mean = nullptr, const float* ln_rstd = nullptr,
+                                           const int* rowmap = nullptr) {
+  static_assert(!(MAPPED && GEGLU), "no mapped GEGLU epilogue");
   const int q = lane >> 4;
   const int c = lane & 15;
   const int row0 = block_m0 + wave_m * (TM * 16) + c;
@@ -153,7 +155,7 @@
     if (p.partial) {
 #pragma unroll
       for (int tm = 0; tm < TM; ++tm) {
-        const int row = row0 + tm * 16;
+        const int row = MAPPED ? rowmap[tm] : row0 + tm * 16;
         if (row >= row_end) continue;
 #pragma unroll
         for (int g8 = 0; g8 < NG; ++g8) {
@@ -190,7 +192,7 @@
       u32x4 rv[TMB][NG], rr[TMB][NG], ra[TMB][NG];
 #pragma unroll
       for (int t2 = 0; t2 < TMB; ++t2) {
-        const int rowc = min(row0 + (tb + t2) * 16, p.rows - 1);
+        const int rowc = min(MAPPED ? rowmap[tb + t2] : row0 + (tb + t2) * 16, p.rows - 1);
         if (p.rowvec) {
           const int inst = dd_fdiv(rowc, p.inv_rpi);
 #pragma unroll
@@ -211,7 +213,7 @@
 #pragma unroll
       for (int t2 = 0; t2 < TMB; ++t2) {
         const int tm = tb + t2;
-        const int row = row0 + tm * 16;
+        const int row = MAPPED ? rowmap[tm] : row0 + tm * 16;
         float st_s = 0.f, st_q = 0.f;
         if (row < row_end) {
 #pragma unroll
diff --git a/dualdiff_amd/csrc/gemm_tiles.h b/dualdiff_amd/csrc/gemm_tiles.h
--- a/dualdiff_amd/csrc/gemm_tiles.h
+++ b/dualdiff_amd/csrc/gemm_tiles.h
@@ -37,6 +37,16 @@
   uint32_t ln_out_bytes;
 };
 
+constexpr int kUpfoldMax = 64;
+struct UpfoldTab {
+  uint16_t tile0[10];
+  uint8_t widx[9];
+  uint8_t ny[3], nx[3], y0[3], x0[3];
+  float inv_plane[9], inv_nx[3];
+  int m;
+  uint8_t y[kUpfoldMax], x[kUpfoldMax];
+};
+
 enum Family {
   FAM_REG,
   FAM_RING,
@@ -51,6 +61,7 @@
   F_PAD0 = 8,
   F_LN_OUT = 16,
   F_PERSIST = 32,
+  F_UPFOLD = 64,
 };
 
 struct TileCfg {
@@ -65,6 +76,7 @@
 constexpr unsigned REG_ALL = F_DENSE | F_CONV | F_GEGLU | F_PAD0, REG_TN2 = F_DENSE | F_CONV | F_PAD0;
 constexpr unsigned RING_ALL = F_DENSE | F_CONV | F_GEGLU | F_PERSIST, RING_TN2 = F_DENSE | F_CONV | F_PERSIST;
 constexpr unsigned RING_DENSE = F_DENSE | F_PERSIST;
+constexpr unsigned UPF = F_UPFOLD;
 constexpr unsigned PIPE = F_DENSE | F_PERSIST;
 
 constexpr TileCfg kTiles[] = {
@@ -74,21 +86,21 @@
     {4, "64x64", FAM_REG, 2, 2, 2, 2, REG_TN2},
     {5, "256x128", FAM_REG, 4, 2, 4, 4, REG_ALL},
     {11, "128x128/dma2", FAM_RING, 2, 2, 4, 4, RING_ALL, 2},
-    {12, "128x128/dma3", FAM_RING, 2, 2, 4, 4, RING_ALL, 3},
-    {13, "128x64/dma3", FAM_RING, 2, 2, 4, 2, RING_TN2, 3},
-    {14, "64x128/dma3", FAM_RING, 2, 2, 2, 4, RING_ALL, 3},
-    {15, "64x64/dma3", FAM_RING, 2, 2, 2, 2, RING_TN2, 3},
+    {12, "128x128/dma3", FAM_RING, 2, 2, 4, 4, RING_ALL | UPF, 3},
+    {13, "128x64/dma3", FAM_RING, 2, 2, 4, 2, RING_TN2 | UPF, 3},
+    {14, "64x128/dma3", FAM_RING, 2, 2, 2, 4, RING_ALL | UPF, 3},
+    {15, "64x64/dma3", FAM_RING, 2, 2, 2, 2, RING_TN2 | UPF, 3},
     {16, "256x128/dma2", FAM_RING, 4, 2, 4, 4, RING_ALL, 2},
-    {20, "256x128/dma3", FAM_RING, 4, 2, 4, 4, RING_ALL, 3},
+    {20, "256x128/dma3", FAM_RING, 4, 2, 4, 4, RING_ALL | UPF, 3},
     {23, "128x64/dma4", FAM_RING, 2, 2, 4, 2, RING_TN2, 4},
     {24, "64x128/dma4", FAM_RING, 2, 2, 2, 4, RING_ALL, 4},
     {27, "160x160/dma2", FAM_RING, 2, 5, 5, 2, RING_TN2, 2},
-    {28, "160x160/dma3", FAM_RING, 2, 5, 5, 2, RING_TN2, 3},
+    {28, "160x160/dma3", FAM_RING, 2, 5, 5, 2, RING_TN2 | UPF, 3},
     {40, "80x320/dma2", FAM_RING, 1, 10, 5, 2, RING_DENSE | F_LN_OUT, 2},
-    {52, "96x64/dma3", FAM_RING, 2, 2, 3, 2, RING_TN2, 3},
+    {52, "96x64/dma3", FAM_RING, 2, 2, 3, 2, RING_TN2 | UPF, 3},
     {59, "32x64/dma3", FAM_RING, 2, 2, 1, 2, RING_DENSE, 3},
     {60, "32x64/dma6", FAM_RING, 2, 2, 1, 2, RING_DENSE, 6},
-    {44, "192x128/dma3", FAM_RING, 4, 2, 3, 4, RING_ALL, 3},
+    {44, "192x128/dma3", FAM_RING, 4, 2, 3, 4, RING_ALL | UPF, 3},
     {46, "192x128/dma2", FAM_RING, 4, 2, 3, 4, RING_ALL, 2},
     {50, "256x256/dma2", FAM_RING, 2, 4, 8, 4, RING_ALL, 2},
     {72, "96x64/p3", FAM_PIPE, 2, 2, 3, 2, PIPE, 3},
@@ -120,7 +132,7 @@
 constexpr bool tiles_consistent() {
   for (const TileCfg& t : kTiles)
     if (((t.forms & F_PAD0) && t.family != FAM_REG) || ((t.forms & F_CONV) && t.family == FAM_PIPE) ||
-        ((t.forms & F_LN_OUT) && tile_bn(t) != 320) || (t.family == FAM_DIRECT) != (t.forms == F_CONV)) return false;
+        ((t.forms & F_LN_OUT) && tile_bn(t) != 320) || ((t.forms & F_UPFOLD) && (t.family != FAM_RING || !(t.forms & F_CONV))) || (t.family == FAM_DIRECT) != (t.forms == F_CONV)) return false;
   for (int id : kAutoTiles) if (tile_index(id) < 0 || kTiles[tile_index(id)].family != FAM_REG) return false;
   return tile_index(kTileLnRing) >= 0 && tile_index(kTileLnPipe) >= 0;
 }
@@ -131,10 +143,10 @@
   return (t.wm * t.wn == 4 && 2 * ring <= 160 * 1024) ? 2 : 1;
 }
 
-struct Plan { int tile_idx; int split; int tiles_m, tiles_n; int k_per_split; int g_per_tile, chunks_per_split; bool unsupported; bool persist_ok; int band_rows, bands; bool persist3_ok; };
+struct Plan { int tile_idx; int split; int tiles_m, tiles_n; int k_per_split; int g_per_tile, chunks_per_split; bool unsupported; bool persist_ok; int band_rows, bands; bool persist3_ok; UpfoldTab upf; };
 
 using LaunchFn = int(int dtype, unsigned form, const GemmParams& p, const Plan& pl, hipStream_t s);
-__attribute__((visibility("hidden"))) LaunchFn launch_gemm1, launch_gemm2_dense, launch_gemm2_geglu, launch_gemm2_conv, launch_gemm3,
+__attribute__((visibility("hidden"))) LaunchFn launch_gemm1, launch_gemm2_dense, launch_gemm2_geglu, launch_gemm2_conv, launch_gemm2_upfold, launch_gemm3,
     launch_gemm4, launch_conv3s;
 
 template <auto KERN>
diff --git a/dualdiff_amd/networks/layers.py b/dualdiff_amd/networks/layers.py
--- a/dualdiff_amd/networks/layers.py
+++ b/dualdiff_amd/networks/layers.py
@@ -1,9 +1,11 @@
 import math
+import os
 
 import torch
 import torch.nn as nn
 
 from .. import ops as O
+from .. import upfold
 
 
 CACHE_EPOCH = [0]
@@ -186,8 +188,30 @@
             self.__dict__["_pk_w"] = w.reshape(self.out_channels, 9 * self.cin_pad).contiguous()
         return self.__dict__["_pk_w"]
 
+    fold_upsample = os.environ.get("DD_UPFOLD", "1") != "0"
+
+    def folded_up(self, h, w, up_size, m=None):
+        if not self.fold_upsample or up_size is None:
+            return None
+        size = (h, w, int(up_size[0]), int(up_size[1]))
+        if m is not None:
+            row = O.tuning.upfold_tuned(O.tuning.conv_upfold_key(m, h, w, self.cin_pad, self.out_channels, size[2], size[3],
+                                                                O._dtype_code(self.weight.dtype)))
+            if row is None or row[0] == 0:
+                return None
+        key = (self.weight.data_ptr(), self.weight._version) + size
+        cache = self.__dict__.setdefault("_pk_upfold", {})
+        hit = cache.get(size)
+        if hit is None or (hit[0] != key and not torch.cuda.is_current_stream_capturing()):
+            if not upfold.ok(*size, self.cin_pad, self.stride):
+                return None
+            with torch.no_grad():
+                hit = cache[size] = (key, upfold.fold_weight(self.packed, *size))
+        return hit[1]
+
     def run(self, x2d, m, h, w, up_size=None, **kw):
-        return O.conv3x3(x2d, self.packed, self.bias, m, h, w, stride=self.stride, up_size=up_size, **kw)
+        return O.conv3x3(x2d, self.packed, self.bias, m, h, w, stride=self.stride, up_size=up_size,
+                         upfold=self.folded_up(h, w, up_size, m), **kw)
 
     def out_hw(self, h, w, up_size=None):
         hv, wv = (h, w) if up_size is None else up_size
diff --git a/dualdiff_amd/ops.py b/dualdiff_amd/ops.py
--- a/dualdiff_amd/ops.py
+++ b/dualdiff_amd/ops.py
@@ -4,7 +4,7 @@
 
 import torch
 
-from . import _native, _timer, _workspace, tuning
+from . import _native, _timer, _workspace, tuning, upfold as _upfold
 from ._native import DD_BF16, DD_EPI_GEGLU, DD_EPI_NONE, DD_EPI_SILU, DD_F16, AttnDesc, Gemm8Desc, GemmDesc, XAttnDesc
 from ._timer import KernelTimer, _stream, set_timer
 from ._workspace import workspace, workspace_owner
@@ -182,7 +182,8 @@
 
 
 def conv3x3(x, w, bias, m, hin, win, *, stride=1, up_size=None, rowvec=None, res=None,
-            alpha=1.0, out=None, accumulate=False, epilogue=DD_EPI_NONE, tile=0, split_k=0, gn_next=None, pad=1):
+            alpha=1.0, out=None, accumulate=False, epilogue=DD_EPI_NONE, tile=0, split_k=0, gn_next=None, pad=1,
+            upfold=None):
     lib = _native.load()
     _need_gpu(x, w, bias, res, rowvec, out)
     x = _rows2d(x)
@@ -200,6 +201,13 @@
     if w.shape[1] != 9 * cin or not w.is_contiguous():
         raise ValueError("conv weight must be contiguous [cout, 9*cin]")
     rows = m * hout * wout
+    if upfold is not None:
+        _need_gpu(upfold)
+        ncls = _upfold.num_classes(hin, win, hv, wv) if pad == 1 and stride == 1 and up_size is not None and cin % 64 == 0 else 0
+        if ncls == 0:
+            raise ValueError("conv3x3(upfold=...): no folded form for %dx%d -> %dx%d, stride %d, cin %d" % (hin, win, hv, wv, stride, cin))
+        if tuple(upfold.shape) != (ncls * cout, 4 * cin) or not upfold.is_contiguous() or upfold.dtype != x.dtype:
+            raise ValueError("folded conv weight must be contiguous %s [%d * cout, 4 * cin]" % (x.dtype, ncls))
     out = _out_or_new(out, (rows, cout), x.dtype, x.device, "conv3x3")
     if pad == 1 and thin_conv_ok(cin, cout, stride, m) and up_size is None and rowvec is None and res is None and alpha == 1.0 \
             and not accumulate and epilogue in (DD_EPI_NONE, DD_EPI_SILU) and tile == 0 and split_k == 0 \
@@ -217,12 +225,21 @@
     d.conv = 1
     d.hin, d.win, d.cin, d.hv, d.wv = hin, win, cin, hv, wv
     d.hout, d.wout, d.stride = hout, wout, stride
+    if upfold is not None:
+        d.w, d.k, d.k1, d.upfold = upfold.data_ptr(), 4 * cin, 4 * cin, 1
     _epilogue_side(d, _dt(x), bias, rowvec, hout * wout, res, out, alpha, accumulate, epilogue, tile, split_k)
     L = tuning.launcher(lib, pad)
     what = "conv3x3" if pad == 1 else "conv3x3(pad=0)"
     if tile == 0 and split_k == 0:
         key = (tuning.conv_key if pad == 1 else tuning.conv_pad0_key)(m, hin, win, cin, cout, stride, hv, wv, d.dtype)
-        _tune(L, d, key, (rows, cout), x.dtype, x.device, (x, res))
+        hit = None
+        if upfold is not None:
+            key = tuning.conv_upfold_key(m, hin, win, cin, cout, hv, wv, d.dtype)
+            hit = tuning.upfold_tuned(key)
+        if hit is not None and hit[0] != 0:
+            d.tile, d.split_k = hit[:2]
+        else:
+            _tune(L, d, key, (rows, cout), x.dtype, x.device, (x, res))
     need = _workspace.attach(d, x.device, lambda: L.ws_bytes(d))
     if pad == 1 and gn_next is not None and GN_SPLITK and need > 0 and alpha == 1.0 and not accumulate \
             and epilogue == DD_EPI_NONE:
diff --git a/dualdiff_amd/tuning.py b/dualdiff_amd/tuning.py
--- a/dualdiff_amd/tuning.py
+++ b/dualdiff_amd/tuning.py
@@ -14,6 +14,8 @@
 _COLD = os.environ.get("DD_AUTOTUNE_COLD", "1") != "0"
 CHALLENGE_TILES = tuple(int(t) for t in os.environ.get("DD_TUNE_CHALLENGE", "").split(",") if t.strip())
 TUNE_TABLE_PATH = os.path.join(os.path.dirname(os.path.abspath(__file__)), "tuned", "gfx950.json")
+UPFOLD_TABLE_PATH = os.path.join(os.path.dirname(os.path.abspath(__file__)), "tuned", "gfx950_upfold.json")
+_UPFOLD = None
 _TUNED = {}
 _TABLE_LOADED = False
 _CHALLENGED = set()
@@ -36,6 +38,23 @@
 
 def conv_pad0_key(m, hin, win, cin, cout, stride, hv, wv, dtype):
     return conv_key(m, hin, win, cin, cout, stride, hv, wv, dtype) + ("p0",)
+
+
+def conv_upfold_key(m, hin, win, cin, cout, hv, wv, dtype):
+    return conv_key(m, hin, win, cin, cout, 1, hv, wv, dtype) + ("uf",)
+
+
+def upfold_tuned(key):
+    global _UPFOLD
+    if _UPFOLD is None:
+        _UPFOLD = {}
+        if os.environ.get("DD_TUNE_TABLE") != "0" and os.path.exists(UPFOLD_TABLE_PATH):
+            with open(UPFOLD_TABLE_PATH) as f:
+                blob = json.load(f)
+            if blob.get("arch") != "gfx950":
+                raise RuntimeError("tune cache %s is not for gfx950" % UPFOLD_TABLE_PATH)
+            _UPFOLD = {ast.literal_eval(k): _entry(v) for k, v in blob["entries"]}
+    return _UPFOLD.get(key)
 
 
 def _entry(v):
diff --git a/dualdiff_amd/upfold.py b/dualdiff_amd/upfold.py
--- /dev/null
+++ b/dualdiff_amd/upfold.py
@@ -0,0 +1,84 @@
+import functools
+
+import numpy as np
+import torch
+
+MAX_OUT = 64
+SLOT_TAPS = (((0,), (1, 2)), ((0, 1), (2,)), ((0,), (1,)))
+
+
+def src(o, n_in, n_out):
+    scale = np.float32(n_in) / np.float32(n_out)
+    return min(int(np.floor(np.float32(o) * scale)), n_in - 1)
+
+
+def axis_class(o, n_in, n_out):
+    s = src(o, n_in, n_out)
+    for c in range(3):
+        ok = True
+        for t in (-1, 0, 1):
+            tap_in = 0 <= o + t < n_out
+            if c == 2 and t == 1:
+                ok = not tap_in
+            else:
+                pos = (s if c == 1 else s - 1) + ((t == 1) if c == 1 else (t >= 0))
+                src_in = 0 <= pos < n_in
+                ok = (src_in and src(o + t, n_in, n_out) == pos) if tap_in else not src_in
+            if not ok:
+                break
+        if ok:
+            return c
+    return None
+
+
+@functools.lru_cache(maxsize=None)
+def _axis_classes(n_in, n_out):
+    if n_in <= 0 or n_out <= n_in or n_out > MAX_OUT:
+        return None
+    cls = tuple(axis_class(o, n_in, n_out) for o in range(n_out))
+    return None if None in cls else cls
+
+
+def axis_classes(n_in, n_out):
+    cls = _axis_classes(int(n_in), int(n_out))
+    return None if cls is None else list(cls)
+
+
+@functools.lru_cache(maxsize=None)
+def _classes(hin, win, hv, wv):
+    ycls, xcls = _axis_classes(hin, hv), _axis_classes(win, wv)
+    if ycls is None or xcls is None:
+        return None
+    return ycls, xcls, tuple((rc, cc) for rc in range(3) for cc in range(3) if rc in ycls and cc in xcls)
+
+
+def classes(hin, win, hv, wv):
+    c = _classes(int(hin), int(win), int(hv), int(wv))
+    return None if c is None else (list(c[0]), list(c[1]), list(c[2]))
+
+
+def num_classes(hin, win, hv, wv):
+    c = _classes(int(hin), int(win), int(hv), int(wv))
+    return 0 if c is None else len(c[2])
+
+
+def ok(hin, win, hv, wv, cin=64, stride=1):
+    return stride == 1 and cin % 64 == 0 and num_classes(hin, win, hv, wv) > 0
+
+
+def fold_weight(w, hin, win, hv, wv, sum_dtype=torch.float32, out_dtype=None):
+    cl = classes(hin, win, hv, wv)
+    if cl is None:
+        raise ValueError("no folded form for the nearest map %dx%d -> %dx%d" % (hin, win, hv, wv))
+    cout = w.shape[0]
+    w9 = w.detach().reshape(cout, 3, 3, -1).to(sum_dtype)
+    mats = []
+    for rc, cc in cl[2]:
+        f = w9.new_zeros((cout, 2, 2, w9.shape[3]))
+        for sy in range(2):
+            for sx in range(2):
+                for ky in SLOT_TAPS[rc][sy]:
+                    for kx in SLOT_TAPS[cc][sx]:
+                        f[:, sy, sx] += w9[:, ky, kx]
+        mats.append(f.reshape(cout, -1))
+    return torch.cat(mats, 0).to(out_dtype or w.dtype).contiguous()
diff --git a/include/dualdiff_hip.h b/include/dualdiff_hip.h
--- a/include/dualdiff_hip.h
+++ b/include/dualdiff_hip.h
@@ -68,6 +68,7 @@
   int64_t ld_ln_out;
   const void* lno_gamma;
   const void* lno_beta;
+  int32_t upfold;
 } dd_gemm_desc;
 
 int dd_gemm(const dd_gemm_desc* d, dd_stream_t stream);
```

Measured after the change: 91.71 steps/s (median of 6 runs). 1.01x the previous value.
